# ereiss123/LDPCsimulation

Measured on AMD Instinct MI355X. Metric: decoded Mbit/s + FER match vs CPU, N=1944 rate-1/2 min-sum @ 1/2/4/8 MI355X, higher is better.
Workload: dtype f64

## Files before the change

include/ldpc_hip.h:

```cpp
#ifndef LDPC_HIP_H
#define LDPC_HIP_H

#include <stdint.h>

#ifdef __cplusplus
extern "C" {
#endif

#define LDPC_ABI_VERSION 11

typedef enum {
    LDPC_OK = 0,
    LDPC_ERR_INVALID = -1,
    LDPC_ERR_NOMEM = -2,
    LDPC_ERR_DEVICE = -3,
    LDPC_ERR_UNSUPPORTED = -4,
    LDPC_ERR_IO = -5,
    LDPC_ERR_GRAPH = -6
} ldpc_status;

typedef enum { LDPC_MS = 0, LDPC_NMS = 1, LDPC_OMS = 2, LDPC_BP = 3, LDPC_DDBMP = 4 } ldpc_variant;

typedef enum { LDPC_F32 = 0, LDPC_F64 = 1 } ldpc_precision;

typedef enum { LDPC_FLOODING = 0, LDPC_LAYERED = 1 } ldpc_schedule;

typedef struct ldpc_graph ldpc_graph;
typedef struct ldpc_ctx ldpc_ctx;

typedef struct {
    int64_t bit_err;
    int64_t frame_err;
    int64_t uncoded_bit_err;
    int64_t frames;
    int64_t iters;
    int64_t syndrome_fail;
} ldpc_counts;

typedef struct {
    int32_t bit_err;
    int32_t uncoded_bit_err;
    int32_t syndrome_fail;
    int32_t iters;
} ldpc_frame_result;

typedef struct {
    int32_t variant;
    int32_t precision;
    int32_t T;
    int32_t quantize;
    int32_t saturate;
    int32_t qbits;
    double  ymax;
    double  alpha;
    double  delta;
    int32_t schedule;
    int32_t early_stop;
    double  n0;
    double  max_llr;
} ldpc_decoder_cfg;

int         ldpc_abi_version(void);
const char *ldpc_last_error(void);
int         ldpc_f64_nms_fast_division(double alpha);
int         ldpc_bp_math_probe(int device, const double *x, int n, double *tanh_out, double *log_out);
int         ldpc_check_selftest(int device);

int  ldpc_graph_create(int N, int M, const int *num_nlist, const int *const *nlist,
                       const int *num_mlist, const int *const *mlist, ldpc_graph **out);
int  ldpc_graph_load_alist(const char *path, ldpc_graph **out);
int  ldpc_graph_info(const ldpc_graph *g, int *N, int *M, int *E, int *maxdv, int *maxdc);
void ldpc_graph_destroy(ldpc_graph *g);
int  ldpc_graph_layers(const ldpc_graph *g, int32_t *row_order, int32_t *layer_ptr, int *nlayers);

int  ldpc_device_count(int *n);
int  ldpc_ctx_create(int device, const ldpc_graph *g, int max_batch, ldpc_ctx **out);
int  ldpc_ctx_set_stream(ldpc_ctx *ctx, void *hip_stream);
int  ldpc_ctx_synchronize(ldpc_ctx *ctx);
void ldpc_ctx_destroy(ldpc_ctx *ctx);

int  ldpc_decode_batch(ldpc_ctx *ctx, const void *y, int batch, const ldpc_decoder_cfg *cfg,
                       const int8_t *c, int8_t *d_out, ldpc_frame_result *frames,
                       ldpc_counts *counts);

int  ldpc_sim_set_codewords(ldpc_ctx *ctx, const uint8_t *bits, int rows);

int  ldpc_sim_launch(ldpc_ctx *ctx, double ebn0_db, double R, const ldpc_decoder_cfg *cfg,
                     uint64_t seed, uint32_t stream_id, uint64_t first_cw, int batch,
                     ldpc_frame_result *frames_dev);
int  ldpc_ctx_read_counts(ldpc_ctx *ctx, ldpc_counts *out, int reset);
int  ldpc_ctx_read_histogram(ldpc_ctx *ctx, int64_t *out, int reset);
int  ldpc_sim_batch(ldpc_ctx *ctx, double ebn0_db, double R, const ldpc_decoder_cfg *cfg,
                    uint64_t seed, uint32_t stream_id, uint64_t first_cw, int batch,
                    ldpc_frame_result *frames, ldpc_counts *accum);

int  ldpc_sim_trace(ldpc_ctx *ctx, double ebn0_db, double R, const ldpc_decoder_cfg *cfg,
                    uint64_t seed, uint32_t stream_id, uint64_t first_cw, int batch,
                    void *y_out, int8_t *d_out, ldpc_frame_result *frames, ldpc_counts *accum);

int  ldpc_ctx_last_kernel_ms(ldpc_ctx *ctx, float *ms);
int  ldpc_ctx_kernel_info(ldpc_ctx *ctx, const ldpc_decoder_cfg *cfg, char *name, int name_len,
                          int *lds_bytes, int *blocks_per_cu);
int  ldpc_ctx_redo_count(ldpc_ctx *ctx, int64_t *n);
int  ldpc_ctx_redo_list(ldpc_ctx *ctx, uint32_t *list, int64_t cap, int64_t *n);
int  ldpc_ctx_row_sched_info(ldpc_ctx *ctx, const ldpc_decoder_cfg *cfg, int32_t *info);
int  ldpc_ctx_pp_inreg_info(ldpc_ctx *ctx, const ldpc_decoder_cfg *cfg, int32_t *info);
int  ldpc_ctx_pp_row_slots(ldpc_ctx *ctx, const ldpc_decoder_cfg *cfg, uint16_t *cols, uint8_t *deg, int cap,
                           int *nslots);

typedef enum {
    LDPC_OPT_ROWS64 = 1,
    LDPC_OPT_ROWS32 = 2,
    LDPC_OPT_PP_SLOTS = 3,
    LDPC_OPT_KERNEL = 4,
    LDPC_OPT_FLOOD_MODE = 5,
    LDPC_OPT_FLOOD_MSG = 6,
    LDPC_OPT_FLOOD_SPS_CHECK = 7,
    LDPC_OPT_FLOOD_SPS_BIT = 8,
    LDPC_OPT_FLOOD_RESIDENT = 9,
    LDPC_OPT_FLOOD_STREAMS = 10,
    LDPC_OPT_FLOOD_BPC = 11,
    LDPC_OPT_LAYERED_BPC = 12,
    LDPC_OPT_LAYERED_LDS_POS = 13,
    LDPC_OPT_LAYERED_ROWS64 = 14,
    LDPC_OPT_LAYERED_THREADS = 15,
    LDPC_OPT_ROWS_BPC = 16,
    LDPC_OPT_FAST_BPC = 17,
    LDPC_OPT_BP_KERNEL = 18,
    LDPC_OPT_GDBF_KERNEL = 19,
    LDPC_OPT_EMS_THREADS = 20,
    LDPC_OPT_EMS_SWIZZLE = 21,
    LDPC_OPT_DDBMP_KERNEL = 22
} ldpc_option;
#define LDPC_OPT_COUNT 23
int  ldpc_ctx_set_option(ldpc_ctx *ctx, int option, int value);
int  ldpc_ctx_get_option(const ldpc_ctx *ctx, int option, int *value);

typedef enum {
    LDPC_GDBF_NOISE = 1,
    LDPC_GDBF_ADAPT = 2,
    LDPC_GDBF_WEIGHT = 4,
    LDPC_GDBF_SMOOTH = 8,
    LDPC_GDBF_SATURATE = 16,
    LDPC_GDBF_QUANTIZE = 32,
    LDPC_GDBF_SEQUENTIAL = 64,
    LDPC_GDBF_MODESWITCH = 128,
    LDPC_GDBF_QPROB = 256
} ldpc_gdbf_flag;

typedef struct {
    int32_t flags;
    int32_t precision;
    int32_t T;
    int32_t windowsize;
    int32_t nq;
    int32_t tswitch;
    double  theta;
    double  lambda;
    double  alpha;
    double  noise_scale;
    double  ymax;
    double  qsigma;
} ldpc_gdbf_cfg;

int  ldpc_gdbf_decode_batch(ldpc_ctx *ctx, const void *y, const void *pert, int batch, const ldpc_gdbf_cfg *cfg,
                            const int8_t *c, int8_t *d_out, ldpc_frame_result *frames, ldpc_counts *counts);
int  ldpc_gdbf_sim_launch(ldpc_ctx *ctx, double ebn0_db, double R, const ldpc_gdbf_cfg *cfg, uint64_t seed,
                          uint32_t stream_id, uint64_t first_cw, int batch, ldpc_frame_result *frames_dev);
int  ldpc_gdbf_sim_batch(ldpc_ctx *ctx, double ebn0_db, double R, const ldpc_gdbf_cfg *cfg, uint64_t seed,
                         uint32_t stream_id, uint64_t first_cw, int batch, ldpc_frame_result *frames,
                         ldpc_counts *accum);
int  ldpc_gdbf_kernel_info(ldpc_ctx *ctx, const ldpc_gdbf_cfg *cfg, char *name, int name_len, int *lds_bytes);

typedef struct {
    int32_t flags;
    int32_t precision;
    int32_t T;
    int32_t maxphase;
    int32_t windowsize;
    int32_t reserved;
    double  theta;
    double  lambda;
    double  alpha;
    double  noise_scale;
    double  ymax;
} ldpc_rgdbf_cfg;

int  ldpc_rgdbf_decode_batch(ldpc_ctx *ctx, const void *y, const void *pert, int batch, const ldpc_rgdbf_cfg *cfg,
                             const int8_t *c, int8_t *d_out, ldpc_frame_result *frames, ldpc_counts *counts);
int  ldpc_rgdbf_sim_launch(ldpc_ctx *ctx, double ebn0_db, double R, const ldpc_rgdbf_cfg *cfg, uint64_t seed,
                           uint32_t stream_id, uint64_t first_cw, int batch, ldpc_frame_result *frames_dev);
int  ldpc_rgdbf_sim_batch(ldpc_ctx *ctx, double ebn0_db, double R, const ldpc_rgdbf_cfg *cfg, uint64_t seed,
                          uint32_t stream_id, uint64_t first_cw, int batch, ldpc_frame_result *frames,
                          ldpc_counts *accum);
int  ldpc_rgdbf_kernel_info(ldpc_ctx *ctx, const ldpc_rgdbf_cfg *cfg, char *name, int name_len, int *lds_bytes);

typedef struct {
    int32_t flags, precision, T, attempts, windowsize, first_attempt;
    double  theta, lambda, alpha, noise_scale, ymax;
} ldpc_rstat_cfg;
typedef struct { int32_t bit_err, iters, syndrome_fail, smoothing_used; } ldpc_attempt_result;
typedef struct {
    int32_t *err_trace;
    int32_t *unsat_trace;
    int8_t  *d_trace;
    int8_t  *s_trace;
} ldpc_rstat_trace;

int  ldpc_rstat_decode_batch(ldpc_ctx *ctx, const void *y, const void *pert, int batch, const ldpc_rstat_cfg *cfg,
                             const int8_t *c, ldpc_attempt_result *attempts_out, const ldpc_rstat_trace *trace,
                             int8_t *d_out, ldpc_frame_result *frames, ldpc_counts *counts);
int  ldpc_rstat_sim_launch(ldpc_ctx *ctx, double ebn0_db, double R, const ldpc_rstat_cfg *cfg, uint64_t seed,
                           uint32_t stream_id, uint64_t first_cw, int batch, ldpc_attempt_result *attempts_dev,
                           const ldpc_rstat_trace *trace_dev, ldpc_frame_result *frames_dev);
int  ldpc_rstat_sim_batch(ldpc_ctx *ctx, double ebn0_db, double R, const ldpc_rstat_cfg *cfg, uint64_t seed,
                          uint32_t stream_id, uint64_t first_cw, int batch, ldpc_attempt_result *attempts_out,
                          const ldpc_rstat_trace *trace, ldpc_frame_result *frames, ldpc_counts *accum);
int  ldpc_rstat_sim_trace(ldpc_ctx *ctx, double ebn0_db, double R, const ldpc_rstat_cfg *cfg, uint64_t seed,
                          uint32_t stream_id, uint64_t first_cw, int batch, void *y_out, void *pert_out,
                          ldpc_attempt_result *attempts_out, const ldpc_rstat_trace *trace, int8_t *d_out,
                          ldpc_frame_result *frames, ldpc_counts *accum);
int  ldpc_rstat_kernel_info(ldpc_ctx *ctx, const ldpc_rstat_cfg *cfg, int with_trace, char *name, int name_len,
                            int *lds_bytes);

typedef struct {
    int32_t precision;
    int32_t T;
    int32_t maxphase;
    int32_t nq;
    int32_t qlen;
    int32_t reserved;
    double  w, ymax, noise_scale, theta0;
} ldpc_hwgdbf_cfg;

int  ldpc_hwgdbf_decode_batch(ldpc_ctx *ctx, const void *y, const void *q, const int32_t *qptr0, int batch,
                              const ldpc_hwgdbf_cfg *cfg, const int8_t *c, int8_t *d_out, ldpc_frame_result *frames,
                              int32_t *iters_run, ldpc_counts *counts);
int  ldpc_hwgdbf_sim_launch(ldpc_ctx *ctx, double ebn0_db, double R, const ldpc_hwgdbf_cfg *cfg, uint64_t seed,
                            uint32_t stream_id, uint64_t first_cw, int batch, ldpc_frame_result *frames_dev);
int  ldpc_hwgdbf_sim_batch(ldpc_ctx *ctx, double ebn0_db, double R, const ldpc_hwgdbf_cfg *cfg, uint64_t seed,
                           uint32_t stream_id, uint64_t first_cw, int batch, ldpc_frame_result *frames,
                           ldpc_counts *accum);
int  ldpc_hwgdbf_sim_trace(ldpc_ctx *ctx, double ebn0_db, double R, const ldpc_hwgdbf_cfg *cfg, uint64_t seed,
                           uint32_t stream_id, uint64_t first_cw, int batch, void *y_out, void *q_out,
                           int8_t *d_out, ldpc_frame_result *frames, ldpc_counts *accum);
int  ldpc_hwgdbf_kernel_info(ldpc_ctx *ctx, const ldpc_hwgdbf_cfg *cfg, char *name, int name_len, int *lds_bytes);

typedef struct {
    int32_t variant;
    int32_t precision;
    int32_t T;
    int32_t qbits;
    int32_t msg_bits;
    int32_t nms_num;
    int32_t nms_shift;
    int32_t beta;
    int32_t early_stop;
    int32_t reserved;
    double  ymax;
} ldpc_fxms_cfg;

// ... 84 lines not shown
```

ldpcsimulation_amd/csrc/api.cpp:

```cpp
#include "ldpc_hip.h"
#include "gdbf.h"
#include "rgdbf.h"
#include "rstat.h"
#include "hwgdbf.h"
#include "fxms.h"
#include "fxlms.h"
#include "bp.h"
#include "ddbmp.h"
#include "nb.h"

#include <hip/hip_runtime.h>

#include <cmath>
#include <cstdlib>
#include <cstdio>
#include <cstring>
#include <algorithm>
#include <new>
#include <string>
#include <vector>

#include "graph.h"
#include "kernels.h"
#include "host_rt.h"

using namespace ldpc;

static thread_local std::string g_last_error;

#ifdef LDPC_CHECK
namespace ldpc {
static const char *check_site_name(unsigned s)
{
    static const char *const names[CHK_SITES] = {
        "?", "rows_pp gather (app entry)", "rows_pp scatter (c2v slot)", "rows_pp bit read (c2v slot)",
        "rows_pp app write", "rows_fast gather (app entry)", "rows_fast scatter (c2v slot)",
        "rows_fast bit read (c2v slot)", "rows_fast app write", "flood/layered bit position",
        "flood c2v / eref slot", "flood packed-state row", "gdbf_rows bit", "gdbf_rows check term slot",
        "EMS message slot", "bp_rows bit", "bp_rows message slot", "ddbmp edge flag slot", "ddbmp check parity",
        "rgdbf_rows bit flag", "rgdbf_rows check parity", "hwgdbf decision byte", "hwgdbf check parity",
        "hwgdbf noise sample", "rstat decision byte", "rstat check parity", "rows_es gather (app entry)",
        "rows_es scatter (c2v slot)", "rows_es bit read (c2v slot)", "rows_es app write", "fxms message slot",
        "fxms decision byte", "fxlms schedule entry", "fxlms APP", "fxlms row state"};
    return s < CHK_SITES ? names[s] : "?";
}
long check_collect(hipStream_t s, char *msg, size_t msg_len)
{
    hipError_t e = hipStreamSynchronize(s);
    if (e != hipSuccess) return -(long)e;
    hipError_t (*const take[])(CheckRec *) = {check_take_rows_pp, check_take_rows_fast, check_take_flood, check_take_layered,
                                              check_take_gdbf, check_take_nb, check_take_bp, check_take_ddbmp,
                                              check_take_rgdbf, check_take_hwgdbf, check_take_rstat, check_take_rows_es,
                                              check_take_fxms, check_take_fxlms};
    long total = 0;
    for (auto fn : take) {
        CheckRec r{};
        if ((e = fn(&r)) != hipSuccess) return -(long)e;
        if (r.count && !total)
            std::snprintf(msg, msg_len, "LDPC_CHECK: %s index %u >= bound %u (block %u, thread %u)",
                          check_site_name(r.site), r.idx, r.bound, r.block, r.thread);
        total += r.count;
    }
    return total;
}
}
#endif

struct ldpc_ctx : CtxCore {
    const ldpc_graph *g = nullptr;
    ldpc::DevGraph dg{};
    DevBuf graph, hist, y_stage, c_stage, d_stage, fw_stage, cw_table, gscratch, p_stage;
    DevBuf rs_att_stage, rs_unc, rs_tr_stage[4];
    DevBuf hw_ptr_stage, hw_it_stage;
    DevBuf fx_code_stage;
    bool has_fxl = false;
    ldpc::FxlmsSched fxl{};
    DevBuf fxl_sched;
    int cw_rows = 0;
    ldpc::AuxStream aux;
    bool has_rs = false;
    ldpc::RowSched rs{};
    DevBuf sched;
    bool has_rs_pp = false;
    ldpc::RowSched rs_pp{};
    DevBuf sched_pp;
    bool has_rs_ppi = false;
    ldpc::RowSched rs_ppi{};
    DevBuf sched_ppi;
    bool has_fs = false;
    ldpc::FloodSched fs{};
    DevBuf fsched;
    bool has_ls = false;
    ldpc::LayerSched ls{};
    DevBuf lsched;
    DevBuf divcheck;
    DevBuf redo;
    bool last_fast = false;
    std::vector<std::pair<float, bool>> div_ok;
};

namespace ldpc {
int set_last_error(int code, const std::string &msg)
{
    g_last_error = msg;
    return code;
}

static const Options kNoOptions{};
static thread_local const Options *t_opts = nullptr;
const Options &cur_opts() { return t_opts ? *t_opts : kNoOptions; }
OptScope::OptScope(const Options &o) : prev_(t_opts) { t_opts = &o; }
OptScope::~OptScope() { t_opts = prev_; }

bool option_value_ok(int option, int v)
{
    switch (option) {
    case LDPC_OPT_ROWS64:
    case LDPC_OPT_ROWS32: return v >= 0 && v <= 2;
    case LDPC_OPT_PP_SLOTS: return v >= 0 && v <= 2;
    case LDPC_OPT_FLOOD_MODE:
    case LDPC_OPT_FLOOD_MSG:
    case LDPC_OPT_BP_KERNEL:
    case LDPC_OPT_GDBF_KERNEL:
    case LDPC_OPT_DDBMP_KERNEL:
    case LDPC_OPT_EMS_SWIZZLE: return v == 0 || v == 1;
    case LDPC_OPT_KERNEL: return v >= 0 && v <= 3;
    case LDPC_OPT_FLOOD_SPS_CHECK:
    case LDPC_OPT_FLOOD_SPS_BIT: return v >= 0 && v <= 4;
    case LDPC_OPT_FLOOD_RESIDENT: return v >= 0 && v <= 4096;
    case LDPC_OPT_FLOOD_STREAMS: return v >= 0 && v <= 2;
    case LDPC_OPT_FLOOD_BPC:
    case LDPC_OPT_LAYERED_BPC:
    case LDPC_OPT_ROWS_BPC:
    case LDPC_OPT_FAST_BPC: return v >= 0 && v <= 64;
    case LDPC_OPT_LAYERED_LDS_POS: return v >= 0 && v <= 65536;
    case LDPC_OPT_LAYERED_ROWS64: return v >= 0 && v <= 2;
    case LDPC_OPT_LAYERED_THREADS:
    case LDPC_OPT_EMS_THREADS: return v == 0 || v == 512 || v == 1024;
    default: return false;
    }
}
}

template <class T> static const T *section(const DevBuf &buf, size_t off) { return (const T *)((const unsigned char *)buf.p + off); }

static hipError_t upload_graph(const ldpc_graph &g, DevBuf &buf, ldpc::DevGraph &dg)
{
    Blob b(256);
    const size_t o_rc = b.add(g.row_cols), o_rd = b.add(g.row_deg), o_cp = b.add(g.col_ptr),
                 o_cr = b.add(g.col_refs.data(), sizeof(uint32_t) * g.col_refs.size(), sizeof(uint32_t) * ((size_t)g.E + 1));
    const hipError_t e = upload(b, buf);
    if (e != hipSuccess) return e;
    dg = {g.N, g.M, g.maxdc > 0 ? g.maxdc : 1, section<int32_t>(buf, o_rc), section<uint8_t>(buf, o_rd),
          section<int32_t>(buf, o_cp), section<uint32_t>(buf, o_cr)};
    return hipSuccess;
}

static hipError_t upload_row_sched(const ldpc::RowSchedule &hs, DevBuf &buf, ldpc::RowSched &rs,
                                   const std::vector<uint8_t> *pair_flags = nullptr)
{
    Blob b(256);
    const size_t o_cc = b.add(hs.cn_cols), o_cp = b.add(hs.cn_pos), o_cd = b.add(hs.cn_deg), o_vc = b.add(hs.vn_col),
                 o_vi = b.add(hs.vn_info), o_pf = pair_flags ? b.add(*pair_flags) : 0;
    const hipError_t e = upload(b, buf);
    if (e != hipSuccess) return e;
    rs = {hs.threads, hs.cpt, hs.dc, hs.e_pad, hs.rpt, hs.dc_low, section<uint16_t>(buf, o_cc),
          section<uint16_t>(buf, o_cp), section<uint8_t>(buf, o_cd), section<uint16_t>(buf, o_vc),
          section<uint32_t>(buf, o_vi), pair_flags ? section<uint8_t>(buf, o_pf) : nullptr, hs.e_pad, 0, 0};
    return hipSuccess;
}

static hipError_t upload_flood_sched(const ldpc_graph &g, const ldpc::FloodSchedule &fh, DevBuf &buf, ldpc::FloodSched &fs)
{
    std::vector<uint32_t> eref((size_t)fh.e_pad + 64, 0);
    for (int i = 0; i < fh.M_pad; ++i)
        for (int k = 0; k < fh.rdeg[i]; ++k)
            eref[fh.sq[(size_t)k * fh.M_pad + i]] = ((uint32_t)i << 5) | (uint32_t)k;
    Blob b(256);
    const size_t o_sp = b.add(fh.sp), o_sq = b.add(fh.sq), o_rd = b.add(fh.rdeg), o_pb = b.add(fh.pos_of_bit),
                 o_ba = b.add(fh.bit_at), o_pd = b.add(fh.pdeg), o_gb = b.add(fh.gbase), o_er = b.add(eref);
    const hipError_t e = upload(b, buf);
    if (e != hipSuccess) return e;
    fs = {fh.M_pad, fh.dc, fh.ngroups, fh.e_pad, g.maxdv, section<int32_t>(buf, o_sp), section<int32_t>(buf, o_sq),
          section<uint8_t>(buf, o_rd), section<int32_t>(buf, o_pb), section<int32_t>(buf, o_ba),
          section<uint8_t>(buf, o_pd), section<int32_t>(buf, o_gb), section<uint32_t>(buf, o_er)};
    return hipSuccess;
}

static hipError_t upload_layer_sched(const ldpc::LayerSchedule &lh, DevBuf &buf, ldpc::LayerSched &ls)
{
    Blob b(256);
    const size_t o_lp = b.add(lh.lptr), o_sp = b.add(lh.sp), o_rd = b.add(lh.rdeg), o_pb = b.add(lh.pos_of_bit);
    const hipError_t e = upload(b, buf);
    if (e != hipSuccess) return e;
    ls = {(int)lh.lptr.size() - 1, 0, lh.M_pad, section<int32_t>(buf, o_lp), section<int32_t>(buf, o_sp),
          section<uint8_t>(buf, o_rd), section<int32_t>(buf, o_pb)};
    for (int L = 0; L < ls.nlayers; ++L) ls.max_layer = std::max(ls.max_layer, lh.lptr[L + 1] - lh.lptr[L]);
    return hipSuccess;
}

static hipError_t upload_fxlms_sched(const ldpc_graph &g, const ldpc::LayerSchedule &lh, DevBuf &buf, ldpc::FxlmsSched &sc)
{
    const int M = g.M, dcs = g.maxdc > 0 ? g.maxdc : 1;
    std::vector<int32_t> cols((size_t)dcs * M, 0);
    std::vector<uint8_t> deg(M, 0);
    for (int n = 0; n < M; ++n) {
        const int j = lh.row_order[n], d = g.row_deg[j];
        deg[n] = (uint8_t)d;
        for (int k = 0; k < dcs; ++k)
            cols[(size_t)k * M + n] = d ? g.row_cols[(size_t)j * dcs + std::min(k, d - 1)] : 0;
    }
    Blob b(256);
    const size_t o_lp = b.add(lh.lptr), o_c = b.add(cols), o_d = b.add(deg);
    const hipError_t e = upload(b, buf);
    if (e != hipSuccess) return e;
    sc = {g.N, M, dcs, (int)lh.lptr.size() - 1, section<int32_t>(buf, o_lp), section<int32_t>(buf, o_c),
          section<uint8_t>(buf, o_d)};
    return hipSuccess;
}

static const char kFramesDev[] = "frames_dev must be a device pointer";

template <class Args>
static int stage_given(SyncCall &s, ldpc_ctx *c, Args &a, bool f64, const void *y, const void *extra, size_t extra_elems,
                       const void **extra_dev, const int8_t *cw)
{
    const size_t fsz = f64 ? 8 : 4, nb = (size_t)a.batch * c->g->N;
    a.src = ldpc::SRC_GIVEN;
    RC_TRY(s.in(y, nb * fsz, c->y_stage, a.y));
    if (extra) RC_TRY(s.in(extra, extra_elems * fsz, c->p_stage, *extra_dev));
    return s.in(cw, nb, c->c_stage, a.c);
}

template <class Run>
static int sim_batch_frames(ldpc_ctx *c, int batch, ldpc_frame_result *frames, ldpc_counts *accum, Run run)
{
    RC_TRY(c->enter());
    SyncCall s(*c);
    RC_TRY(s.snapshot());
    ldpc_frame_result *w;
    RC_TRY(s.out(frames, c->fw_stage, sizeof(ldpc_frame_result) * (size_t)batch, w));
    RC_TRY(run(w));
    return s.finish(accum);
}

template <class Args>
static int bind_decisions(SyncCall &s, ldpc_ctx *c, Args &a, int8_t *d_out, ldpc_frame_result *frames)
{
    RC_TRY(s.out(d_out, c->d_stage, (size_t)a.batch * c->g->N, a.d_out));
    return s.out(frames, c->fw_stage, sizeof(ldpc_frame_result) * (size_t)a.batch, a.frame_res);
}

template <class Args, class Cfg> static void redecode_fill(Args &a, ldpc_ctx *c, const Cfg *cfg, int batch)
{
    std::memset((void *)&a, 0, sizeof a);
    a.batch = batch;
    a.T = cfg->T;
    a.flags = cfg->flags;
    a.windowsize = cfg->windowsize;
    a.theta0 = cfg->theta;
    a.lambda = cfg->lambda;
    a.w = cfg->alpha * cfg->ymax;
    a.ymax = cfg->ymax;
    a.qmax = 1.0;
    fill_accounting(a, *c);
}

template <class Cfg, class Own> static int fx_check_cfg(const Cfg *cfg, Own own)
{
    if (!cfg) return set_err(LDPC_ERR_INVALID, "cfg is null");
    if (cfg->variant != LDPC_MS && cfg->variant != LDPC_NMS && cfg->variant != LDPC_OMS)
        return set_err(cfg->variant == LDPC_BP || cfg->variant == LDPC_DDBMP ? LDPC_ERR_UNSUPPORTED : LDPC_ERR_INVALID,
// ... 471 lines not shown
    ldpc::DecodeArgs a;
    fill_common(a, c, cfg, batch);
    RC_TRY(nms_setup(c, cfg, a));
    SyncCall s(*c);
    RC_TRY(stage_given(s, c, a, f64, y, nullptr, 0, nullptr, cw));
    RC_TRY(bind_decisions(s, c, a, d_out, frame_weights));
    RC_TRY(s.snapshot());
    RC_TRY(run_kernel(c, a, f64, cfg->schedule));
    return s.finish(counts);
}

int ldpc_sim_set_codewords(ldpc_ctx *c, const uint8_t *bits, int rows)
{
    if (!c) return set_err(LDPC_ERR_INVALID, "ctx is null");
    if (rows < 0 || (rows > 0 && !bits)) return set_err(LDPC_ERR_INVALID, "bad codeword table");
    RC_TRY(c->enter());
    c->cw_rows = 0;
    if (rows == 0) return LDPC_OK;
    const size_t n = (size_t)rows * c->g->N;
    std::vector<int8_t> bip(n);
    for (size_t i = 0; i < n; ++i) {
        if (bits[i] > 1) return set_err(LDPC_ERR_INVALID, "codeword bit %zu is %d (want 0/1)", i, bits[i]);
        bip[i] = bits[i] ? -1 : +1;
    }
    HIP_TRY(c->cw_table.ensure(n));
    HIP_TRY(hipMemcpy(c->cw_table.p, bip.data(), n, hipMemcpyHostToDevice));
    c->cw_rows = rows;
    return LDPC_OK;
}

static int sim_run(ldpc_ctx *c, const SimCall &q, const ldpc_decoder_cfg *cfg, ldpc_frame_result *frames_dev,
                   void *y_out_dev, int8_t *d_out_dev)
{
    ldpc::DecodeArgs a;
    fill_common(a, c, cfg, q.batch);
    RC_TRY(nms_setup(c, cfg, a));
    const SimPoint pt = fill_sim(a, *c, q);
    fill_cw_table(a, *c);
    if (cfg->variant == LDPC_BP) a.n0 = pt.N0;
    a.frame_res = (int4 *)frames_dev;
    a.y_out = y_out_dev;
    a.d_out = d_out_dev;
    return run_kernel(c, a, cfg->precision == LDPC_F64, cfg->schedule);
}

int ldpc_sim_launch(ldpc_ctx *c, double ebn0_db, double R, const ldpc_decoder_cfg *cfg, uint64_t seed,
                    uint32_t stream_id, uint64_t first_cw, int batch, ldpc_frame_result *frames_dev)
{
    const SimCall q{ebn0_db, R, seed, stream_id, first_cw, batch};
    RC_TRY(check_sim(c, [&] { return check_cfg(c, cfg); }, q, false));
    RC_TRY(require_device(frames_dev, kFramesDev));
    RC_TRY(c->enter());
    return sim_run(c, q, cfg, frames_dev, nullptr, nullptr);
}

int ldpc_ctx_read_counts(ldpc_ctx *c, ldpc_counts *out, int reset)
{
    if (!c) return set_err(LDPC_ERR_INVALID, "ctx is null");
    RC_TRY(c->enter());
    return c->read_counts(out, reset);
}

int ldpc_ctx_read_histogram(ldpc_ctx *c, int64_t *out, int reset)
{
    if (!c || !out) return set_err(LDPC_ERR_INVALID, "null argument");
    RC_TRY(c->enter());
    HIP_TRY(hipMemcpyAsync(out, c->hist.p, c->hist.n, hipMemcpyDeviceToHost, c->stream));
    HIP_TRY(hipStreamSynchronize(c->stream));
    if (reset) HIP_TRY(hipMemsetAsync(c->hist.p, 0, c->hist.n, c->stream));
    return LDPC_OK;
}

int ldpc_sim_trace(ldpc_ctx *c, double ebn0_db, double R, const ldpc_decoder_cfg *cfg, uint64_t seed,
                   uint32_t stream_id, uint64_t first_cw, int batch, void *y_out, int8_t *d_out,
                   ldpc_frame_result *frames, ldpc_counts *accum)
{
    const SimCall q{ebn0_db, R, seed, stream_id, first_cw, batch};
    RC_TRY(check_sim(c, [&] { return check_cfg(c, cfg); }, q, false));
    RC_TRY(c->enter());
    const size_t nb = (size_t)batch * c->g->N;
    SyncCall s(*c);
    RC_TRY(s.snapshot());
    ldpc_frame_result *w;
    void *y;
    int8_t *d;
    RC_TRY(s.out(frames, c->fw_stage, sizeof(ldpc_frame_result) * (size_t)batch, w));
    RC_TRY(s.out(y_out, c->y_stage, nb * (cfg->precision == LDPC_F64 ? 8 : 4), y));
    RC_TRY(s.out(d_out, c->d_stage, nb, d));
    RC_TRY(sim_run(c, q, cfg, w, y, d));
    return s.finish(accum);
}

int ldpc_sim_batch(ldpc_ctx *c, double ebn0_db, double R, const ldpc_decoder_cfg *cfg, uint64_t seed,
                   uint32_t stream_id, uint64_t first_cw, int batch, ldpc_frame_result *frames, ldpc_counts *accum)
{
    return ldpc_sim_trace(c, ebn0_db, R, cfg, seed, stream_id, first_cw, batch, nullptr, nullptr, frames, accum);
}

int ldpc_ctx_last_kernel_ms(ldpc_ctx *c, float *ms)
{
    return c ? c->last_kernel_ms(ms) : set_err(LDPC_ERR_INVALID, "null argument");
}

static int info_plan(ldpc_ctx *c, const ldpc_decoder_cfg *cfg, ldpc::LaunchPlan &p)
{
    if (!c || !cfg) return set_err(LDPC_ERR_INVALID, "null argument");
    RC_TRY(check_cfg(c, cfg));
    RC_TRY(c->enter());
    ldpc::DecodeArgs a;
    fill_common(a, c, cfg, 1);
    RC_TRY(nms_setup(c, cfg, a));
    p = build_plan(c, a, cfg->precision == LDPC_F64, cfg->schedule);
    return LDPC_OK;
}

int ldpc_ctx_row_sched_info(ldpc_ctx *c, const ldpc_decoder_cfg *cfg, int32_t *info)
{
    if (!info) return set_err(LDPC_ERR_INVALID, "null argument");
    ldpc::LaunchPlan p;
    RC_TRY(info_plan(c, cfg, p));
    if (!p.rs) return set_err(LDPC_ERR_UNSUPPORTED, "the row kernel does not decode this cfg (kernel %s)", p.name);
    const ldpc::RowSched &rs = *p.rs;
    info[0] = rs.threads;
    info[1] = rs.rpt;
    info[2] = rs.cpt;
    info[3] = rs.dc;
    info[4] = rs.e_pad;
    info[5] = p.cw_per_block;
    info[6] = p.lds_bytes;
    info[7] = p.blocks_per_cu;
    info[8] = rs.dc_low;
    info[9] = rs.dc_low ? (rs.threads + rs.threads / 2) * rs.dc_low + (rs.threads / 2) * rs.dc
                        : rs.threads * rs.rpt * rs.dc;
    return LDPC_OK;
}

int ldpc_ctx_pp_inreg_info(ldpc_ctx *c, const ldpc_decoder_cfg *cfg, int32_t *info)
{
    if (!info) return set_err(LDPC_ERR_INVALID, "null argument");
    ldpc::LaunchPlan p;
    RC_TRY(info_plan(c, cfg, p));
    if (p.kernel != ldpc::Kernel::rows_pp || !p.rs)
        return set_err(LDPC_ERR_UNSUPPORTED, "the ping-pong kernel does not decode this cfg (kernel %s)", p.name);
    int32_t rsi[10];
    RC_TRY(ldpc_ctx_row_sched_info(c, cfg, rsi));
    const ldpc::RowSched *ri = p.rs_inreg;
    info[0] = ri ? ri->n_inreg : 0;
    info[1] = ri ? ri->lds_edge_slots : rsi[9];
    info[2] = ri ? ri->e_used : p.rs->e_pad;
    info[3] = ri ? ri->cpt : p.rs->cpt;
    return LDPC_OK;
}

int ldpc_ctx_pp_row_slots(ldpc_ctx *c, const ldpc_decoder_cfg *cfg, uint16_t *cols, uint8_t *deg, int cap, int *nslots)
{
    if (!cols || !deg || !nslots || cap < 0) return set_err(LDPC_ERR_INVALID, "null argument");
    ldpc::LaunchPlan p;
    RC_TRY(info_plan(c, cfg, p));
    if (p.kernel != ldpc::Kernel::rows_pp || !p.rs)
        return set_err(LDPC_ERR_UNSUPPORTED, "the ping-pong kernel does not decode this cfg (kernel %s)", p.name);
    const ldpc::RowSched *rs = p.rs_inreg ? p.rs_inreg : p.rs;
    *nslots = rs->threads * rs->rpt;
    if (cap < *nslots) return set_err(LDPC_ERR_INVALID, "%d row slots, room for %d", *nslots, cap);
    RC_TRY(c->enter());
    HIP_TRY(hipMemcpyAsync(cols, rs->cn_cols, sizeof(uint16_t) * (size_t)*nslots * rs->dc, hipMemcpyDeviceToHost, c->stream));
    HIP_TRY(hipMemcpyAsync(deg, rs->cn_deg, sizeof(uint8_t) * (size_t)*nslots, hipMemcpyDeviceToHost, c->stream));
    HIP_TRY(hipStreamSynchronize(c->stream));
    return LDPC_OK;
}

int ldpc_ctx_redo_count(ldpc_ctx *c, int64_t *n)
{
    if (!c || !n) return set_err(LDPC_ERR_INVALID, "null argument");
    *n = 0;
    if (!c->last_fast || !c->redo.p) return LDPC_OK;
    RC_TRY(c->enter());
    unsigned h = 0;
    HIP_TRY(hipMemcpyAsync(&h, c->redo.p, sizeof h, hipMemcpyDeviceToHost, c->stream));
    HIP_TRY(hipStreamSynchronize(c->stream));
    *n = (int64_t)h;
    return LDPC_OK;
}

int ldpc_ctx_redo_list(ldpc_ctx *c, uint32_t *list, int64_t cap, int64_t *n)
{
    if (!c || !n || cap < 0 || (cap > 0 && !list)) return set_err(LDPC_ERR_INVALID, "null argument");
    RC_TRY(ldpc_ctx_redo_count(c, n));
    const int64_t m = std::min(*n, cap);
    if (m > 0) {
        HIP_TRY(hipMemcpyAsync(list, (const unsigned *)c->redo.p + 1, sizeof(unsigned) * (size_t)m, hipMemcpyDeviceToHost,
                               c->stream));
        HIP_TRY(hipStreamSynchronize(c->stream));
    }
    return LDPC_OK;
}

int ldpc_ctx_kernel_info(ldpc_ctx *c, const ldpc_decoder_cfg *cfg, char *name, int name_len, int *lds_bytes,
                         int *bpc)
{
    ldpc::LaunchPlan p;
    RC_TRY(info_plan(c, cfg, p));
    if (bpc) *bpc = p.blocks_per_cu;
    return report_choice(p, name, name_len, lds_bytes);
}


static int gdbf_check_cfg(const ldpc_gdbf_cfg *cfg)
{
    if (!cfg) return set_err(LDPC_ERR_INVALID, "cfg is null");
    if (cfg->precision != LDPC_F32 && cfg->precision != LDPC_F64)
        return set_err(LDPC_ERR_INVALID, "bad precision %d", cfg->precision);
    if (cfg->T < 0 || cfg->T > 4094) return set_err(LDPC_ERR_INVALID, "T must be in 0..4094");
    if (cfg->flags & ~511) return set_err(LDPC_ERR_INVALID, "unknown GDBF flags 0x%x", cfg->flags);
    if ((cfg->flags & LDPC_GDBF_ADAPT) && (cfg->flags & (LDPC_GDBF_SEQUENTIAL | LDPC_GDBF_MODESWITCH)))
        return set_err(LDPC_ERR_UNSUPPORTED, "threshold adaptation with single-bit flips is not supported");
    if ((cfg->flags & LDPC_GDBF_QPROB) && (cfg->flags & LDPC_GDBF_NOISE))
        return set_err(LDPC_ERR_UNSUPPORTED, "QPROB with NOISE is not supported");
    if ((cfg->flags & LDPC_GDBF_MODESWITCH) && cfg->tswitch < 0) return set_err(LDPC_ERR_INVALID, "tswitch < 0");
    if ((cfg->flags & (LDPC_GDBF_SATURATE | LDPC_GDBF_QUANTIZE)) && !(cfg->ymax > 0))
        return set_err(LDPC_ERR_INVALID, "saturate/quantize need ymax > 0");
    if ((cfg->flags & LDPC_GDBF_QUANTIZE) && (cfg->nq < 1 || cfg->nq > 30))
        return set_err(LDPC_ERR_INVALID, "nq out of range");
    if ((cfg->flags & LDPC_GDBF_SMOOTH) && (cfg->windowsize < 0 || cfg->windowsize > 32767))
        return set_err(LDPC_ERR_INVALID, "windowsize out of range");
    return LDPC_OK;
}

static void gdbf_fill(ldpc::GdbfArgs &a, ldpc_ctx *c, const ldpc_gdbf_cfg *cfg, int batch)
{
    std::memset(&a, 0, sizeof a);
    a.batch = batch;
    a.T = cfg->T;
    a.flags = cfg->flags;
    a.windowsize = cfg->windowsize;
    a.theta0 = cfg->theta;
    a.lambda = cfg->lambda;
    a.w = (cfg->flags & LDPC_GDBF_WEIGHT) ? cfg->alpha : 1.0;
    a.ymax = cfg->ymax;
    a.qmax = std::pow(2, (cfg->nq - 1));
    a.tswitch = cfg->tswitch;
    a.qsigma = cfg->qsigma;
    fill_accounting(a, *c);
}

static int gdbf_run(ldpc_ctx *c, const ldpc::GdbfArgs &a, bool f64)
{
    const ldpc::OptScope os(c->opts);
    const ldpc::GdbfChoice ch = ldpc::gdbf_choose(c->dg, f64, a.flags, c->g->maxdv, c->g->maxdc);
    return run_with_slots(*c, c->gscratch, ch, a.batch, 2 * c->num_cus, [&](void *scratch, int slots) {
        return ldpc::gdbf_launch(c->dg, a, f64, ch, scratch, slots, c->num_cus, c->stream);
    });
}

int ldpc_gdbf_decode_batch(ldpc_ctx *c, const void *y, const void *pert, int batch, const ldpc_gdbf_cfg *cfg,
                           const int8_t *cw, int8_t *d_out, ldpc_frame_result *frames, ldpc_counts *counts)
{
    if (!c || !y) return set_err(LDPC_ERR_INVALID, "null argument");
    RC_TRY(gdbf_check_cfg(cfg));
    RC_TRY(check_batch(*c, batch));
    const bool with_pert = cfg->flags & (LDPC_GDBF_NOISE | LDPC_GDBF_QPROB);
    if (with_pert && !pert) return set_err(LDPC_ERR_INVALID, "NOISE / QPROB need pert");
    if ((cfg->flags & LDPC_GDBF_QPROB) && !(cfg->qsigma > 0)) return set_err(LDPC_ERR_INVALID, "QPROB needs qsigma > 0");
    RC_TRY(c->enter());
    const bool f64 = cfg->precision == LDPC_F64;
    ldpc::GdbfArgs a;
    gdbf_fill(a, c, cfg, batch);
    SyncCall s(*c);
    RC_TRY(stage_given(s, c, a, f64, y, with_pert ? pert : nullptr, (size_t)batch * c->g->N * (size_t)cfg->T, &a.pert, cw));
    RC_TRY(bind_decisions(s, c, a, d_out, frames));
    RC_TRY(s.snapshot());
    RC_TRY(gdbf_run(c, a, f64));
    return s.finish(counts);
}

static int gdbf_sim_run(ldpc_ctx *c, const SimCall &q, const ldpc_gdbf_cfg *cfg, ldpc_frame_result *frames_dev)
{
    ldpc::GdbfArgs a;
    gdbf_fill(a, c, cfg, q.batch);
    fill_sim(a, *c, q);
    fill_cw_table(a, *c);
    a.frame_res = (int4 *)frames_dev;
    a.noise_sigma = a.sigma * cfg->noise_scale;
    a.qsigma = a.noise_sigma;
    return gdbf_run(c, a, cfg->precision == LDPC_F64);
}

int ldpc_gdbf_sim_launch(ldpc_ctx *c, double ebn0_db, double R, const ldpc_gdbf_cfg *cfg, uint64_t seed,
                         uint32_t stream_id, uint64_t first_cw, int batch, ldpc_frame_result *frames_dev)
{
    const SimCall q{ebn0_db, R, seed, stream_id, first_cw, batch};
    RC_TRY(check_sim(c, [&] { return gdbf_check_cfg(cfg); }, q, true));
    RC_TRY(require_device(frames_dev, kFramesDev));
    RC_TRY(c->enter());
    return gdbf_sim_run(c, q, cfg, frames_dev);
}

int ldpc_gdbf_sim_batch(ldpc_ctx *c, double ebn0_db, double R, const ldpc_gdbf_cfg *cfg, uint64_t seed,
                        uint32_t stream_id, uint64_t first_cw, int batch, ldpc_frame_result *frames,
                        ldpc_counts *accum)
{
    const SimCall q{ebn0_db, R, seed, stream_id, first_cw, batch};
    RC_TRY(check_sim(c, [&] { return gdbf_check_cfg(cfg); }, q, true));
    return sim_batch_frames(c, batch, frames, accum, [&](ldpc_frame_result *w) { return gdbf_sim_run(c, q, cfg, w); });
}

int ldpc_gdbf_kernel_info(ldpc_ctx *c, const ldpc_gdbf_cfg *cfg, char *name, int name_len, int *lds_bytes)
// ... 667 lines not shown
```

ldpcsimulation_amd/csrc/kernels.h:

```cpp
#pragma once
#include "options.h"
#include <hip/hip_runtime.h>
#include <cstdint>

namespace ldpc {

struct DevGraph {
    int N, M, dcs;
    const int32_t *row_cols;
    const uint8_t *row_deg;
    const int32_t *col_ptr;
    const uint32_t *col_refs;
};

enum { SRC_GIVEN = 0, SRC_PHILOX = 1 };
enum { VARIANT_BP = 3, VARIANT_DDBMP = 4 };

struct DecodeArgs {
    int batch, T, variant, quantize, saturate;
    int early_stop;
    double ymax, nq, alpha, delta;
    double n0, max_llr;
    int nms_fast;
    float alpha_rcp;
    int src;
    const void *y;
    const int8_t *c;
    const int8_t *cw_table;
    int cw_rows;
    uint64_t seed, first_cw;
    uint32_t stream_id;
    double sigma;
    int8_t *d_out;
    void *y_out;
    int4 *frame_res;
    unsigned long long *counts;
    unsigned long long *hist;
    unsigned long long *stamps;
};

struct RowSched {
    int threads, cpt, dc, e_pad, rpt;
    int dc_low;
    const uint16_t *cn_cols;
    const uint16_t *cn_pos;
    const uint8_t *cn_deg;
    const uint16_t *vn_col;
    const uint32_t *vn_info;
    const uint8_t *pair;
    int e_used;
    int n_inreg;
    int lds_edge_slots;
};

struct FloodSched {
    int M_pad, dc, ngroups, e_pad;
    int dv;
    const int32_t *sp, *sq;
    const uint8_t *rdeg;
    const int32_t *pos_of_bit;
    const int32_t *bit_at;
    const uint8_t *pdeg;
    const int32_t *gbase;
    const uint32_t *eref;
};

struct LayerSched {
    int nlayers = 0, max_layer = 0, M_pad = 0;
    const int32_t *lptr = nullptr;
    const int32_t *sp = nullptr;
    const uint8_t *rdeg = nullptr;
    const int32_t *pos_of_bit = nullptr;
};

enum class Kernel {
    rows, rows_fast, rows_pp,
    rows_es,
    lds, global,
    flood_persistent, flood_phase,
    layered_lds, layered_global,
    bp_rows, bp_lds, bp_global,
    ddbmp_rows, ddbmp_lds, ddbmp_global
};

struct LaunchPlan {
    Kernel kernel = Kernel::global;
    const char *name = "";
    const void *fn = nullptr;
    int threads = 0;
    int lds_bytes = 0;
    int layered_pos = 0;
    int cache_lds_bytes = 0;
    int cw_per_block = 1;
    int blocks_per_cu = 0;
    int grid = 0;
    size_t scratch_per_block = 0;
    size_t scratch_bytes = 0;
    const RowSched *rs = nullptr;
    const RowSched *rs_inreg = nullptr;
    bool redo = false;
};

struct PlanInput {
    const DevGraph &g;
    int E;
    const RowSched *rs, *rs_pp;
    const FloodSched *fs;
    const LayerSched *ls;
    int num_cus;
    const DecodeArgs &a;
    bool f64;
    int maxdv = 0;
    const RowSched *rs_ppi = nullptr;
};

template <typename T> struct type_tag { using type = T; };
template <int V> struct src_tag { static constexpr int value = V; };
template <class Fn>
auto for_f_src(bool f64, int src, Fn &&fn)
{
    if (f64)
        return src == SRC_GIVEN ? fn(type_tag<double>{}, src_tag<SRC_GIVEN>{}) : fn(type_tag<double>{}, src_tag<SRC_PHILOX>{});
    return src == SRC_GIVEN ? fn(type_tag<float>{}, src_tag<SRC_GIVEN>{}) : fn(type_tag<float>{}, src_tag<SRC_PHILOX>{});
}

constexpr size_t kMaxLds = 160 * 1024;

int occupancy(const void *fn, int threads, int lds_bytes);
hipError_t launch_fn(const LaunchPlan &p, void **args, hipStream_t s);

bool plan_lds(const PlanInput &in, LaunchPlan &p);
void plan_global(const PlanInput &in, LaunchPlan &p);
hipError_t launch_generic(const LaunchPlan &p, const DevGraph &g, const DecodeArgs &a, void *gscratch, hipStream_t s);
bool plan_rows(const PlanInput &in, LaunchPlan &p);
hipError_t launch_rows(const LaunchPlan &p, const DevGraph &g, const DecodeArgs &a, hipStream_t s);
bool plan_rows_es(const PlanInput &in, LaunchPlan &p);
hipError_t launch_rows_es(const LaunchPlan &p, const DevGraph &g, const DecodeArgs &a, unsigned *ticket, hipStream_t s);
struct AuxStream {
    hipStream_t s = nullptr;
    hipEvent_t fork = nullptr, join = nullptr;
};
bool plan_flood(const PlanInput &in, LaunchPlan &p);
hipError_t launch_flood(const LaunchPlan &p, const DevGraph &g, const FloodSched &fs, const DecodeArgs &a, bool f64,
                        void *gscratch, hipStream_t s, const AuxStream *aux);
void plan_layered(const PlanInput &in, LaunchPlan &p);
hipError_t launch_layered(const LaunchPlan &p, const DevGraph &g, const FloodSched &fs, const LayerSched &ls,
                          const DecodeArgs &a, void *gscratch, hipStream_t s);
constexpr int kPackedMaxDc = 26;

hipError_t verify_div_by_reciprocal(float alpha, float rcp, unsigned long long *mismatches_dev, hipStream_t s);

bool plan_rows_fast(const PlanInput &in, LaunchPlan &p);
bool rows_fast_f32_ok(const DecodeArgs &a);
hipError_t launch_rows_fast(const LaunchPlan &p, const DevGraph &g, const DecodeArgs &a, unsigned *redo, hipStream_t s);
bool markstein_exact_alpha(double alpha);
size_t redo_lds_bytes(const DevGraph &g, bool f64);
hipError_t launch_redo(const DevGraph &g, const DecodeArgs &a, bool f64, const unsigned *redo, hipStream_t s,
                       int num_cus);

bool plan_rows_pp(const PlanInput &in, LaunchPlan &p);
#ifndef LDPC_PP_INREG_CPT
#define LDPC_PP_INREG_CPT 3
#endif
hipError_t launch_rows_pp(const LaunchPlan &p, const DevGraph &g, const DecodeArgs &a, unsigned *redo, hipStream_t s);

constexpr int kRowsMaxThreads = 1024;
constexpr int kRowsCpt[] = {2, 4, 8};
constexpr int kRowsMaxThreadsForRpt[] = {0, 1024, 512, 384};
constexpr int kRowsDc[] = {8, 16, 32};

}
```

ldpcsimulation_amd/csrc/kernels.hip:

```cpp
#include "minsum_kernels.h"
#include "frame.h"

namespace ldpc {

template <typename F, int SRC, bool ES>
__device__ __forceinline__ void decode_codeword(const DecodeArgs &a, const DevGraph &g, int b,
                                                RowState<F> *rows, F *app, F *yq, int *red)
{
    const int tid = threadIdx.x, nt = blockDim.x;
    const int N = g.N, M = g.M;

    const int8_t *cvec = frame_codeword<SRC>(a, b, N);
    int unc = 0;
    channel_bits<F, SRC, false>(a, b, N, cvec, a.y_out, [&](int v, F yv) {
        const F q = front_end<F>(yv, a);
        yq[v] = q;
        app[v] = q;
        const int cv = cvec ? cvec[v] : 1;
        unc += ((q > F(0) ? 1 : -1) * cv < 0);
    });
    for (int j = tid; j < M; j += nt) {
        RowState<F> z;
        z.m1 = F(0); z.m2 = F(0); z.meta = 0;
        rows[j] = z;
// ... 16 lines not shown
    for (; it < a.T; ++it) {
        if (ES && !__syncthreads_or(syndrome())) break;
        for (int j = tid; j < M; j += nt) {
            RowState<F> st = rows[j];
            const int deg = g.row_deg[j];
            const int32_t *rc = g.row_cols + (size_t)j * g.dcs;
            const int oidx = (int)(st.meta & 63u);
            const uint64_t osg = st.meta >> 6;
            F mn1 = dinf<F>(), mn2 = dinf<F>();
            int amin = 63;
            uint64_t sg = 0;
            for (int k = 0; k < deg; ++k) {
                F cold = (k == oidx) ? st.m2 : st.m1;
                if ((osg >> k) & 1u) cold = -cold;
                const F x = app[rc[k]] - cold;
                sg |= (uint64_t)(!(x >= F(0))) << k;
                const F ax = dabs(x);
                if (ax <= mn1) { mn2 = mn1; mn1 = ax; amin = k; }
                else if (ax < mn2) { mn2 = ax; }
            }
            const uint64_t degmask = (deg >= 64) ? ~0ull : ((1ull << deg) - 1ull);
            uint64_t eff = (__popcll(sg) & 1) ? (sg ^ degmask) : sg;
            F M1 = mn1, M2 = mn2;
            if (a.variant == V_NMS) {
                M1 = mn1 / alpha;
                M2 = mn2 / alpha;
            } else if (a.variant == V_OMS) {
                const F t1 = mn1 - delta, t2 = mn2 - delta;
                const bool p1 = t1 > F(0), p2 = t2 > F(0);
                M1 = p1 ? t1 : F(0);
                M2 = p2 ? t2 : F(0);
                const uint64_t abit = (amin < 64) ? (1ull << amin) : 0ull;
                if (!p1 || mn1 == F(0)) eff &= abit;
                if (!p2 || mn2 == F(0)) eff &= ~abit;
            }
            st.m1 = M1;
            st.m2 = M2;
            st.meta = (uint64_t)amin | (eff << 6);
            rows[j] = st;
        }
        __syncthreads();
        for (int v = tid; v < N; v += nt) {
            F sum = yq[v];
            const int e1 = g.col_ptr[v + 1];
            for (int e = g.col_ptr[v]; e < e1; ++e) {
                const uint32_t ref = g.col_refs[e];
                const int k = (int)(ref & 63u);
                const RowState<F> st = rows[ref >> 6];
                const F mag = (k == (int)(st.meta & 63u)) ? st.m2 : st.m1;
                sum += ((st.meta >> (6 + k)) & 1u) ? -mag : mag;
            }
            app[v] = sum;
        }
        __syncthreads();
    }

    int w = 0;
    for (int v = tid; v < N; v += nt) {
        const int d = app[v] > F(0) ? 1 : -1;
        const int cv = cvec ? cvec[v] : 1;
        w += (d != cv);
        if (a.d_out) a.d_out[(size_t)b * N + v] = (int8_t)d;
    }
    int sums[3] = {w, unc, syndrome()};
    block_sum_n_t0<3>(sums, red);
    if (tid == 0)
        frame_account(a.counts, a.hist, a.frame_res, b, sums[0], sums[1], sums[2] > 0, ES ? it : a.T, ES ? it : 0);
    __syncthreads();
}

template <typename F, int SRC, bool ES>
__global__ __launch_bounds__(256) void k_decode_lds(DecodeArgs a, DevGraph g)
{
    extern __shared__ __attribute__((aligned(16))) unsigned char smem[];
    RowState<F> *rows = reinterpret_cast<RowState<F> *>(smem);
    F *app = reinterpret_cast<F *>(smem + sizeof(RowState<F>) * (size_t)g.M);
    F *yq = app + g.N;
    int *red = reinterpret_cast<int *>(yq + g.N);
    decode_codeword<F, SRC, ES>(a, g, blockIdx.x, rows, app, yq, red);
}

template <typename F, int SRC>
__global__ __launch_bounds__(256) void k_redo(DecodeArgs a, DevGraph g, const unsigned *redo)
{
    extern __shared__ __attribute__((aligned(16))) unsigned char smem[];
    RowState<F> *rows = reinterpret_cast<RowState<F> *>(smem);
    F *app = reinterpret_cast<F *>(smem + sizeof(RowState<F>) * (size_t)g.M);
    F *yq = app + g.N;
    int *red = reinterpret_cast<int *>(yq + g.N);
    const unsigned n = redo[0];
    for (unsigned i = blockIdx.x; i < n; i += gridDim.x) decode_codeword<F, SRC, false>(a, g, (int)redo[1 + i], rows, app, yq, red);
}

template <typename F, int SRC, bool ES>
__global__ __launch_bounds__(256) void k_decode_global(DecodeArgs a, DevGraph g, unsigned char *scratch,
                                                       size_t slot_bytes)
{
    __shared__ int red[16];
    unsigned char *base = scratch + slot_bytes * blockIdx.x;
    RowState<F> *rows = reinterpret_cast<RowState<F> *>(base);
    F *app = reinterpret_cast<F *>(base + sizeof(RowState<F>) * (size_t)g.M);
    F *yq = app + g.N;
    for (int b = blockIdx.x; b < a.batch; b += gridDim.x)
        decode_codeword<F, SRC, ES>(a, g, b, rows, app, yq, red);
}


__global__ __launch_bounds__(256) void k_verify_div(float alpha, float rcp, unsigned long long *bad)
{
    const uint32_t total = 0x7f800000u;
    unsigned long long nbad = 0;
    for (uint32_t u = blockIdx.x * blockDim.x + threadIdx.x; u < total; u += gridDim.x * blockDim.x) {
        const float x = __uint_as_float(u);
        const float q = x * rcp;
        const float f = __builtin_fmaf(__builtin_fmaf(-q, alpha, x), rcp, q);
        const float d = x / alpha;
        nbad += (__float_as_uint(f) != __float_as_uint(d));
    }
    for (int o = 32; o > 0; o >>= 1) nbad += __shfl_xor(nbad, o, 64);
    if ((threadIdx.x & 63) == 0 && nbad) atomicAdd(bad, nbad);
}


hipError_t verify_div_by_reciprocal(float alpha, float rcp, unsigned long long *bad, hipStream_t s)
{
    hipError_t e = hipMemsetAsync(bad, 0, sizeof(unsigned long long), s);
    if (e != hipSuccess) return e;
    hipLaunchKernelGGL(k_verify_div, dim3(8192), dim3(256), 0, s, alpha, rcp, bad);
    return hipGetLastError();
}

static size_t state_bytes(const DevGraph &g, bool f64)
{
    const size_t rs = f64 ? sizeof(RowState<double>) : sizeof(RowState<float>);
    const size_t fs = f64 ? 8 : 4;
    return rs * (size_t)g.M + 2 * fs * (size_t)g.N;
}

constexpr int kThreads = 256;

int occupancy(const void *fn, int threads, int lds_bytes)
{
    int nb = 0;
    if (lds_bytes > 0) (void)hipFuncSetAttribute(fn, hipFuncAttributeMaxDynamicSharedMemorySize, lds_bytes);
    if (hipOccupancyMaxActiveBlocksPerMultiprocessor(&nb, fn, threads, lds_bytes) != hipSuccess) {
        (void)hipGetLastError();
        return 0;
    }
    return nb;
}

hipError_t launch_fn(const LaunchPlan &p, void **args, hipStream_t s)
{
    const int lds = p.lds_bytes + p.cache_lds_bytes;
    if (!p.fn || p.grid <= 0) return hipErrorInvalidValue;
    if (lds > 0) {
        const hipError_t e = hipFuncSetAttribute(p.fn, hipFuncAttributeMaxDynamicSharedMemorySize, lds);
        if (e != hipSuccess) return e;
    }
    return hipLaunchKernel(p.fn, dim3(p.grid), dim3(p.threads), args, (size_t)lds, s);
}

bool plan_lds(const PlanInput &in, LaunchPlan &p)
{
    const size_t lds = (state_bytes(in.g, in.f64) + 64 + 15) & ~(size_t)15;
    if (lds > kMaxLds) return false;
    const bool es = in.a.early_stop != 0;
    const auto fn = [es](auto f, auto s) {
        using F = typename decltype(f)::type;
        constexpr int SRC = decltype(s)::value;
        return es ? (const void *)k_decode_lds<F, SRC, true> : (const void *)k_decode_lds<F, SRC, false>;
    };
    p = LaunchPlan{};
    p.kernel = Kernel::lds;
    p.name = "lds";
    p.fn = for_f_src(in.f64, in.a.src, fn);
    p.threads = kThreads;
    p.lds_bytes = (int)lds;
    p.blocks_per_cu = occupancy(for_f_src(in.f64, SRC_PHILOX, fn), p.threads, p.lds_bytes);
    p.grid = in.a.batch;
    return true;
}

void plan_global(const PlanInput &in, LaunchPlan &p)
{
    const bool es = in.a.early_stop != 0;
    const auto fn = [es](auto f, auto s) {
        using F = typename decltype(f)::type;
        constexpr int SRC = decltype(s)::value;
        return es ? (const void *)k_decode_global<F, SRC, true> : (const void *)k_decode_global<F, SRC, false>;
    };
    p = LaunchPlan{};
    p.kernel = Kernel::global;
    p.name = "global";
    p.fn = for_f_src(in.f64, in.a.src, fn);
    p.threads = kThreads;
    p.scratch_per_block = (state_bytes(in.g, in.f64) + 255) & ~(size_t)255;
    p.blocks_per_cu = occupancy(for_f_src(in.f64, SRC_PHILOX, fn), p.threads, 0);
    int per_cu = p.blocks_per_cu;
    if (const int cap = opt(LDPC_OPT_FLOOD_BPC)) per_cu = std::min(per_cu, cap);
    if (per_cu <= 0) per_cu = 1;
    p.grid = std::min(per_cu * in.num_cus, in.a.batch);
    p.scratch_bytes = p.scratch_per_block * (size_t)p.grid;
}

hipError_t launch_generic(const LaunchPlan &p, const DevGraph &g, const DecodeArgs &a, void *gscratch, hipStream_t s)
{
    unsigned char *gs = (unsigned char *)gscratch;
    size_t spb = p.scratch_per_block;
    void *args[] = {(void *)&a, (void *)&g, &gs, &spb};
    return launch_fn(p, args, s);
}

size_t redo_lds_bytes(const DevGraph &g, bool f64) { return (state_bytes(g, f64) + 64 + 15) & ~(size_t)15; }

hipError_t launch_redo(const DevGraph &g, const DecodeArgs &a, bool f64, const unsigned *redo, hipStream_t s,
                       int num_cus)
{
    const size_t lds = redo_lds_bytes(g, f64);
    return for_f_src(f64, a.src, [&](auto f, auto src) -> hipError_t {
        auto fn = k_redo<typename decltype(f)::type, decltype(src)::value>;
        hipError_t e = hipFuncSetAttribute((const void *)fn, hipFuncAttributeMaxDynamicSharedMemorySize, (int)lds);
        if (e != hipSuccess) return e;
        hipLaunchKernelGGL(fn, dim3(num_cus), dim3(kThreads), lds, s, a, g, redo);
        return hipGetLastError();
    });
}

}
```

ldpcsimulation_amd/csrc/rows_pp.hip:

```cpp
#ifndef LDPC_VN_U3_F64
#ifdef LDPC_VN_U3
#define LDPC_VN_U3_F64 LDPC_VN_U3
#else
#define LDPC_VN_U3_F64 4
#endif
#endif
#ifndef LDPC_VN_U1_F64
#ifdef LDPC_VN_U1
#define LDPC_VN_U1_F64 LDPC_VN_U1
#else
#define LDPC_VN_U1_F64 8
#endif
#endif
#include "kernels.h"
#include "device_common.h"
#include "minsum_common.h"
#include "fast64.h"

#include <hip/hip_runtime.h>
#include <algorithm>
#include <cstdint>
#include <cstdlib>
#include <type_traits>

namespace ldpc {

namespace {

#ifndef LDPC_PP_STICKY
#define LDPC_PP_STICKY 0
#endif
#ifndef LDPC_PP_TAILFUSE
#define LDPC_PP_TAILFUSE 1
#endif
#ifndef LDPC_PP_TAILEXP
#define LDPC_PP_TAILEXP 0
#endif
#ifndef LDPC_PP_CHAN_ALL
#define LDPC_PP_CHAN_ALL 0
#endif
#ifndef LDPC_PP_NOB2
#define LDPC_PP_NOB2 1
#endif
#ifndef LDPC_PP_CHAN_SPLIT
#define LDPC_PP_CHAN_SPLIT 0
#endif
#ifndef LDPC_PP_EXP
#define LDPC_PP_EXP 0
#endif
#if LDPC_PP_EXP != 0 && !defined(LDPC_AB_BUILD)
#error "LDPC_PP_EXP != 0 gives wrong results by design: make ppvariant only"
#endif
#if LDPC_PP_TAILEXP != 0 && !defined(LDPC_AB_BUILD)
#error "LDPC_PP_TAILEXP != 0 gives wrong results by design: make ppvariant only"
#endif
#ifndef LDPC_PP_BITDELAY
#define LDPC_PP_BITDELAY 0
#endif
#ifndef LDPC_PP_ROWFENCE
#define LDPC_PP_ROWFENCE 1
#endif

#ifndef LDPC_PP_PRIO
#define LDPC_PP_PRIO 0
#endif
#ifndef LDPC_PP_PREFETCH
#define LDPC_PP_PREFETCH 1
#endif
#ifndef LDPC_PP_STORE_ORDER
#define LDPC_PP_STORE_ORDER 1
#endif
#ifndef LDPC_PP_GATHER_FIRST
#define LDPC_PP_GATHER_FIRST 0
#endif
#ifndef LDPC_PP_INREG_Y
#define LDPC_PP_INREG_Y 1
#endif
#ifndef LDPC_PP_ILV
#define LDPC_PP_ILV 2
#endif
#ifndef LDPC_PP_ILV_SKIP
#define LDPC_PP_ILV_SKIP 0
#endif
#ifndef LDPC_PP_SBASE
#define LDPC_PP_SBASE 0
#endif
#ifndef LDPC_PP_ONEPREM
#define LDPC_PP_ONEPREM 1
#endif
#if LDPC_PP_SBASE && !defined(LDPC_CHECK)
#define PP_ADDR8(DC, w, k, base, n, site) addr8<DC, true>(w, k, base)
#else
#define PP_ADDR8(DC, w, k, base, n, site) LDPC_ADDR8(DC, w, k, base, n, site)
#endif

#ifdef LDPC_STAMPS
#define PP_STAMP_DECL unsigned long long st_work = 0, st_wait = 0, st_step[6] = {}, st_t0 = __builtin_amdgcn_s_memtime()
#define PP_BARRIER()                                                        \
    do {                                                                    \
        const unsigned long long te_ = __builtin_amdgcn_s_memtime();        \
        __syncthreads();                                                    \
        const unsigned long long tb_ = __builtin_amdgcn_s_memtime();        \
        st_work += te_ - st_t0;                                             \
        st_wait += tb_ - te_;                                               \
        st_t0 = tb_;                                                        \
    } while (0)
#define PP_STAMP_ACC(k)                                                     \
    do {                                                                    \
        const unsigned long long t_ = __builtin_amdgcn_s_memtime();         \
        st_step[k] += t_ - st_t0;                                           \
        st_t0 = t_;                                                         \
    } while (0)
#define PP_STAMP_TOP() PP_STAMP_ACC(0)
#define PP_SYNC_STAMPED(k0)                                                 \
    do {                                                                    \
        PP_STAMP_ACC(k0);                                                   \
        __syncthreads();                                                    \
        PP_STAMP_ACC(k0 + 1);                                               \
    } while (0)
#define PP_STAMP_OUT()                                                                              \
    if (a.stamps && (threadIdx.x & 63) == 0 && blockIdx.x < 256) {                                  \
        a.stamps[(blockIdx.x * 16 + (threadIdx.x >> 6)) * 2] = st_work;                             \
        a.stamps[(blockIdx.x * 16 + (threadIdx.x >> 6)) * 2 + 1] = st_wait;                         \
        for (int k_ = 0; k_ < 6; ++k_)                                                              \
            a.stamps[8192 + (blockIdx.x * 16 + (threadIdx.x >> 6)) * 6 + k_] = st_step[k_];         \
    }
#else
#define PP_STAMP_DECL
#define PP_BARRIER() __syncthreads()
#define PP_STAMP_TOP()
#define PP_STAMP_ACC(k)
#define PP_SYNC_STAMPED(k0) __syncthreads()
#define PP_STAMP_OUT()
#endif

constexpr int kPPRole = 512;
constexpr int kPPWaves = 2 * kPPRole / 64;
constexpr int kPPMaxCw = 4;
constexpr int kPPRedSums = 32;
constexpr int kPPRedAcc = kPPRedSums + kPPWaves * 3 * kPPMaxCw;
constexpr int kPPRedInts = kPPRedAcc + 2 * 6 + 4;
static_assert(kPPRedAcc % 2 == 0 && kPPRedAcc + 2 * 6 <= kPPRedInts, "acc (6 x u64) outside red[]");

template <int B, int E, typename Fn>
__device__ __forceinline__ void static_for(Fn &&f)
{
    if constexpr (B < E) {
        f(std::integral_constant<int, B>());
        static_for<B + 1, E>(f);
    }
}

template <typename F> struct PPCw { static constexpr int C = sizeof(F) == 8 ? 1 : 2; };

template <typename P>
struct PPSlots {
    P *app[2], *c2v[2];
    uint32_t app_base[2], c2v_base[2];
    int *red;
};

__host__ __device__ constexpr int pp_slot_words(int N, int EA) { return (N + 3 + EA + 1) & ~1; }

template <typename P>
__device__ __forceinline__ PPSlots<P> pp_slots(unsigned char *smem, int N, int EA)
{
    static_assert(sizeof(P) == 8, "one 8-byte LDS word per slot element");
    PPSlots<P> s;
    const int SL = pp_slot_words(N, EA);
    P *b = reinterpret_cast<P *>(smem);
#pragma unroll
    for (int X = 0; X < 2; ++X) {
        s.app[X] = b + X * SL;
        s.c2v[X] = s.app[X] + (N + 3);
        s.app_base[X] = lds_addr_of(s.app[X]);
        s.c2v_base[X] = lds_addr_of(s.c2v[X]);
    }
    s.red = reinterpret_cast<int *>(b + 2 * SL);
    return s;
}

__device__ __forceinline__ bool pp_plain_step(const DecodeArgs &a, int N, int grp, int C)
{
    return !a.cw_table && !a.y_out && !a.quantize && !a.saturate && (N & 3) == 0 && (grp + 1) * 2 * C <= a.batch;
}

template <typename F>
__device__ __forceinline__ void pp_channel_plain(const DecodeArgs &a, const PPSlots<Pack<F, PPCw<F>::C>> &s, int N,
                                                 int grp, int (&unc)[2 * PPCw<F>::C], int t0, int nt, unsigned *bad)
{
    constexpr int C = PPCw<F>::C;
    const F kMax = sizeof(F) == 8 ? (F)kFast64Max : (F)1e30f;
    const int ng4 = N / 4;
    const F sigma = (F)a.sigma;
    for (int t = t0; t < 2 * C * ng4; t += nt) {
        int q = 0;
#pragma unroll
        for (int k = 1; k < 2 * C; ++k) q += t >= k * ng4 ? 1 : 0;
        const int g4 = t - q * ng4, X = q >= C ? 1 : 0, c = q - X * C;
        const uint64_t cw = a.first_cw + (uint64_t)(grp * 2 * C + q);
        uint32_t u[4];
        philox4x32_10<true>((uint32_t)g4, (uint32_t)cw, (uint32_t)(cw >> 32), a.stream_id, (uint32_t)a.seed,
                            (uint32_t)(a.seed >> 32), u);
        F n[4];
        box_muller(u[0], u[1], n[0], n[1]);
        box_muller(u[2], u[3], n[2], n[3]);
        F qv[4];
        int e = 0;
        bool ok = true;
#pragma unroll
        for (int q4 = 0; q4 < 4; ++q4) {
            qv[q4] = (F(1) + sigma * n[q4]) + F(0);
            e += (qv[q4] > F(0) ? 1 : -1) < 0;
            ok &= dabs(qv[q4]) < kMax;
        }
        if (!ok) *bad |= 1u << X;
        if constexpr (C == 1) {
            struct alignas(16) D2 { F d[2]; };
            const uint32_t at = (X ? s.app_base[1] : s.app_base[0]) + 32u * (uint32_t)g4;
            lds_put<D2>(at, D2{{qv[0], qv[1]}});
            lds_put<D2>(at + 16u, D2{{qv[2], qv[3]}});
        } else {
            auto *ap = X ? s.app[1] : s.app[0];
#pragma unroll
            for (int q4 = 0; q4 < 4; ++q4) ap[4 * g4 + q4].v[c] = qv[q4];
        }
#pragma unroll
        for (int qq = 0; qq < 2 * C; ++qq) unc[qq] += qq == q ? e : 0;
    }
}

template <typename F, int SRC>
__device__ __forceinline__ void pp_channel(const DecodeArgs &a, const PPSlots<Pack<F, PPCw<F>::C>> &s, int N, int grp,
                                           int (&unc)[2 * PPCw<F>::C], int t0, int nt, unsigned *bad = nullptr)
{
    constexpr int C = PPCw<F>::C;
    const F kMax = sizeof(F) == 8 ? (F)kFast64Max : (F)1e30f;
#pragma unroll
    for (int q = 0; q < 2 * C; ++q) unc[q] = 0;
    const int ng4 = (N + 3) / 4;
    if constexpr (SRC == SRC_PHILOX && LDPC_PP_NOB2) {
        if (pp_plain_step(a, N, grp, C)) {
            pp_channel_plain<F>(a, s, N, grp, unc, t0, nt, bad);
            return;
        }
    }
    for (int t = t0; t < 2 * C * ng4; t += nt) {
        int q = 0;
#pragma unroll
        for (int k = 1; k < 2 * C; ++k) q += t >= k * ng4 ? 1 : 0;
        const int g4 = t - q * ng4, X = q >= C ? 1 : 0, c = q - X * C;
        const int b = grp * 2 * C + q;
        auto *ap = X ? s.app[1] : s.app[0];
        if (b >= a.batch) {
#pragma unroll
            for (int q4 = 0; q4 < 4; ++q4)
                if (4 * g4 + q4 < N) ap[4 * g4 + q4].v[c] = F(1);
            continue;
        }
        const uint64_t cw = a.first_cw + (uint64_t)b;
        F yv[4];
        const int8_t *cvec;
        if (SRC == SRC_GIVEN) {
            cvec = a.c ? a.c + (size_t)b * N : nullptr;
            const F *y = reinterpret_cast<const F *>(a.y) + (size_t)b * N;
#pragma unroll
            for (int q4 = 0; q4 < 4; ++q4) yv[q4] = 4 * g4 + q4 < N ? y[4 * g4 + q4] : F(0);
        } else {
            cvec = a.cw_table ? a.cw_table + (size_t)(cw % (uint64_t)a.cw_rows) * N : nullptr;
            uint32_t u[4];
            philox4x32_10<true>((uint32_t)g4, (uint32_t)cw, (uint32_t)(cw >> 32), a.stream_id, (uint32_t)a.seed,
                          (uint32_t)(a.seed >> 32), u);
            F n[4];
            box_muller(u[0], u[1], n[0], n[1]);
            box_muller(u[2], u[3], n[2], n[3]);
            const F sigma = (F)a.sigma;
#pragma unroll
            for (int q4 = 0; q4 < 4; ++q4) {
                const int v = 4 * g4 + q4;
                const int cv = (cvec && v < N) ? cvec[v] : 1;
                yv[q4] = (F)cv * (F(1) + sigma * n[q4]);
                if (a.y_out && v < N) reinterpret_cast<F *>(a.y_out)[(size_t)b * N + v] = yv[q4];
            }
        }
        int e = 0;
#pragma unroll
        for (int q4 = 0; q4 < 4; ++q4) {
            const int v = 4 * g4 + q4;
            if (v < N) {
                const int cv = cvec ? cvec[v] : 1;
                F qv = front_end<F>(yv[q4], a);
                if (LDPC_PP_NOB2) {
                    qv = qv + F(0);
                    if (!(dabs(qv) < kMax)) *bad |= 1u << X;
                }
                ap[v].v[c] = qv;
                e += ((qv > F(0) ? 1 : -1) * cv < 0);
            }
        }
#pragma unroll
        for (int qq = 0; qq < 2 * C; ++qq) unc[qq] += qq == q ? e : 0;
    }
}

__device__ __forceinline__ int wave_sum3(int x)
{
    return __builtin_popcountll(__builtin_amdgcn_ballot_w64((x & 1) != 0)) +
           2 * __builtin_popcountll(__builtin_amdgcn_ballot_w64((x & 2) != 0)) +
           4 * __builtin_popcountll(__builtin_amdgcn_ballot_w64((x & 4) != 0));
}

template <int C, bool HB, bool WCHK = false>
__device__ __forceinline__ void pp_account(const DecodeArgs &a, int *red, int grp, int (&sums)[6 * C], unsigned *redo,
                                           unsigned long long *acc)
{
    int *tot = red + kPPRedSums;
    const bool lane0 = (threadIdx.x & 63) == 0;
    if (!(LDPC_PP_TAILEXP & 4)) {
#pragma unroll
        for (int q = 0; q < 2 * C; ++q) {
            if constexpr (HB) {
                const int w = wave_sum3(sums[3 * q]), u = wave_sum3(sums[3 * q + 1]);
                if (lane0 && w) atomicAdd(&tot[3 * q], w);
                if (lane0 && u) atomicAdd(&tot[3 * q + 1], u);
            } else {
                if (__builtin_amdgcn_ballot_w64(sums[3 * q + 2] != 0) && lane0) atomicAdd(&tot[3 * q + 2], 1);
                if constexpr (WCHK) {
                    const int w = wave_sum3(sums[3 * q]);
                    if (lane0 && w) atomicAdd(&tot[3 * q], w);
                }
                if constexpr (LDPC_PP_CHAN_ALL || LDPC_PP_CHAN_SPLIT) {
                    const int u = wave_sum3(sums[3 * q + 1]);
                    if (lane0 && u) atomicAdd(&tot[3 * q + 1], u);
                }
            }
        }
    }
    __syncthreads();
    if (threadIdx.x == 0) {
#pragma unroll
        for (int v = 0; v < 6 * C; ++v) {
            sums[v] = tot[v];
            tot[v] = 0;
        }
        const int fl[2] = {red[0], red[1]};
        red[0] = red[1] = 0;
#pragma unroll
        for (int q = 0; q < 2 * C; ++q) {
            const int b = grp * 2 * C + q;
            if (b >= a.batch) continue;
            if (fl[q / C]) {
                const unsigned at = atomicAdd(&redo[0], 1u);
                redo[1 + at] = (unsigned)b;
                continue;
            }
            const int w = sums[3 * q], uc = sums[3 * q + 1], sf = sums[3 * q + 2] > 0;
            acc[0] += (unsigned long long)w;
            acc[1] += (unsigned long long)(w > 0);
            acc[2] += (unsigned long long)uc;
            acc[3] += 1ull;
            acc[5] += (unsigned long long)sf;
            if (w > 0 && a.hist) atomicAdd(&a.hist[w - 1], 1ull);
            if (a.frame_res) a.frame_res[b] = make_int4(w, uc, sf, 0);
        }
    }
}

template <typename F, int DC, int VAR, bool FDIV, int C, int DCA, typename Store>
__device__ __forceinline__ bool pp_check_node(const Pack<F, C> (&xin)[DCA], Pack<F, C> (&pv)[DCA], F alpha, F rcp,
                                              F delta, Store store, uint32_t *pacc)
{
    if constexpr (sizeof(F) == 8) {
        return cn_fast64<DC, VAR, FDIV, DCA, Store, LDPC_PP_STORE_ORDER != 0, true>(xin, pv, alpha, rcp, delta, store,
                                                                                     pacc);
    } else {
        return cn_fast_pair<DC, DCA, Store, LDPC_PP_STORE_ORDER != 0>(xin, pv, VAR == V_NMS, alpha, rcp, store);
    }
}

template <typename F, int SRC, int DC0, int DC1, int CPT, int VAR, bool FDIV, int R, bool HB, int IR = 0>
__device__ __forceinline__ void pp_role(const DecodeArgs &a, const DevGraph &g, const RowSched &rs,
                                        const PPSlots<Pack<F, PPCw<F>::C>> &s, unsigned *redo,
                                        unsigned long long *acc)
{
    constexpr int C = PPCw<F>::C;
    using P = Pack<F, C>;
    constexpr int DCX = 8;
    constexpr int RR = R > 0 ? R : 1;
    static_assert(DC0 <= DCX && DC1 <= DCX && (R == 0) == HB, "pp_role shape");
    static_assert(IR == 0 || R == 2, "in-register bits: two rows per check thread");
    constexpr int L0 = DC0 - 1, L1 = DC1 - 1;
    constexpr bool F64 = sizeof(F) == 8;
    const F kMax = F64 ? (F)kFast64Max : (F)1e30f;
    const int tid = threadIdx.x, N = g.N, lane = tid & 63;
    [[maybe_unused]] const int EA = rs.e_pad + 64;
    [[maybe_unused]] int deg[RR];
    [[maybe_unused]] uint32_t colw[RR][DCX / 2], posw[RR][DCX / 2];
    [[maybe_unused]] P prev[2][RR][DCX];
    if constexpr (R > 0) {
#pragma unroll
        for (int r = 0; r < R; ++r) {
            const int j = tid + r * kPPRole;
            deg[r] = rs.cn_deg[j];
            const uint4 xc = reinterpret_cast<const uint4 *>(rs.cn_cols + (size_t)j * DCX)[0];
            const uint4 xp = reinterpret_cast<const uint4 *>(rs.cn_pos + (size_t)j * DCX)[0];
            colw[r][0] = xc.x; colw[r][1] = xc.y; colw[r][2] = xc.z; colw[r][3] = xc.w;
            posw[r][0] = xp.x; posw[r][1] = xp.y; posw[r][2] = xp.z; posw[r][3] = xp.w;
            if (deg[r] == 0)
#pragma unroll
                for (int q = 0; q < DCX / 2; ++q) colw[r][q] = (uint32_t)(N + 2) * 0x10001u;
        }
    }
    [[maybe_unused]] bool has = IR == 1, fr1 = false;
    if constexpr (IR != 0) {
        const uint32_t pf = rs.pair[LDPC_CHK(tid, kPPRole, CHK_PP_GATHER)];
        if (IR == 2) has = (pf & 1u) != 0;
        fr1 = DC0 != DC1 && (pf & 2u) != 0;
        if (IR == 1 && deg[0] == 0)
            colw[0][L0 / 2] = (L0 & 1) ? (colw[0][L0 / 2] & 0xffffu) | ((uint32_t)N << 16)
                                       : (colw[0][L0 / 2] & 0xffff0000u) | (uint32_t)N;
    }
    [[maybe_unused]] auto inreg_sum = [&](auto Xc, const P &y) -> P {
        constexpr int X = decltype(Xc)::value;
        P sum;
#pragma unroll
        for (int c = 0; c < C; ++c) {
            const F p0 = prev[X][0][L0].v[c], p1 = prev[X][RR - 1][L1].v[c];
            sum.v[c] = (y.v[c] + (fr1 ? p1 : p0)) + (fr1 ? p0 : p1);
        }
        return sum;
    };
    const int bt = tid - kPPRole;
    [[maybe_unused]] int vgb[CPT], vgd[CPT];
    [[maybe_unused]] uint32_t vdst2[(CPT + 1) / 2] = {};
    if constexpr (HB) {
#pragma unroll
        for (int i = 0; i < CPT; ++i) {
            const int c = rs.vn_col[bt * CPT + i];
            vdst2[i / 2] |= (uint32_t)(c == 0xffff ? N + 1 : c) << (16 * (i & 1));
            const uint32_t info = rs.vn_info[bt * CPT + i];
            vgb[i] = __builtin_amdgcn_readfirstlane((int)(info & 0xffffu) - lane);
            vgd[i] = __builtin_amdgcn_readfirstlane((int)(info >> 24));
        }
        P z;
#pragma unroll
        for (int c = 0; c < C; ++c) z.v[c] = F(0);
#pragma unroll
        for (int i = 0; i < CPT; ++i) {
            const int dg = (int)((rs.vn_info[bt * CPT + i] >> 16) & 0xffu);
            const int base = vgb[i] + lane, gd = vgd[i];
            for (int k = dg; k < gd; ++k) {
                const int e = LDPC_CHK(base + k * 64, EA, CHK_PP_BIT_READ);
                s.c2v[0][e] = s.c2v[1][e] = z;
            }
        }
    }
    auto vdst = [&](int i) -> int { return (int)((vdst2[i / 2] >> (16 * (i & 1))) & 0xffffu); };
    const F alpha = (F)a.alpha, delta = (F)a.delta;
    F rcp = F64 ? (F)(1.0 / a.alpha) : (F)a.alpha_rcp;
    if constexpr (F64 && LDPC_PP_SBASE && R > 0)
        rcp = mkd((uint32_t)__builtin_amdgcn_readfirstlane((int)lo32(rcp)), (uint32_t)__builtin_amdgcn_readfirstlane((int)hi32(rcp)));
    const int nsteps = (a.batch + 2 * C - 1) / (2 * C);
    if constexpr (HB && LDPC_PP_NOB2) {
        P inf, zero;
#pragma unroll
        for (int c = 0; c < C; ++c) {
            inf.v[c] = dinf<F>();
            zero.v[c] = F(0);
        }
        if (tid == kPPRole) s.app[0][N] = s.app[1][N] = inf;
        if (tid == kPPRole + 1) s.app[0][N + 2] = s.app[1][N + 2] = zero;
    }
    PP_STAMP_DECL;
    for (int grp = blockIdx.x; grp < nsteps; grp += gridDim.x) {
        PP_STAMP_TOP();
        [[maybe_unused]] uint32_t pacc[2] = {0u, 0u};
        constexpr bool TF = (LDPC_PP_TAILFUSE & (F64 ? 2 : 1)) != 0;
        int unc[2 * C];
        [[maybe_unused]] int wdec[2 * C];
        [[maybe_unused]] int synd0[C];
#pragma unroll
        for (int q = 0; q < 2 * C; ++q) unc[q] = wdec[q] = 0;
        [[maybe_unused]] unsigned chan_bad = 0;
        if constexpr (LDPC_PP_CHAN_ALL && !HB) {
            if (!(LDPC_PP_TAILEXP & 1)) pp_channel<F, SRC>(a, s, N, grp, unc, tid, 2 * kPPRole, &chan_bad);
        }
        [[maybe_unused]] const bool split = LDPC_PP_CHAN_SPLIT && SRC == SRC_PHILOX && LDPC_PP_NOB2 &&
                                            !(LDPC_PP_TAILEXP & 1) && pp_plain_step(a, N, grp, C);
        if constexpr (LDPC_PP_CHAN_SPLIT && !HB) {
            if (split) pp_channel_plain<F>(a, s, N, grp, unc, tid, 2 * kPPRole, &chan_bad);
        }
        if constexpr (HB) {
            if (LDPC_PP_CHAN_SPLIT && split) {
                pp_channel_plain<F>(a, s, N, grp, unc, tid, 2 * kPPRole, &chan_bad);
            } else if (!(LDPC_PP_TAILEXP & 1)) {
                pp_channel<F, SRC>(a, s, N, grp, unc, LDPC_PP_CHAN_ALL ? tid : bt, LDPC_PP_CHAN_ALL ? 2 * kPPRole : kPPRole,
                                   &chan_bad);
            } else {
                for (int q = 0; q < 2 * C; ++q) unc[q] = 0;
                for (int v = bt; v < N; v += kPPRole)
                    for (int c = 0; c < C; ++c) s.app[0][v].v[c] = s.app[1][v].v[c] = F(1);
            }
        }
        PP_SYNC_STAMPED(1);
        [[maybe_unused]] P yq[2][CPT];
        if constexpr (R > 0) {
#pragma unroll
            for (int X = 0; X < 2; ++X)
#pragma unroll
                for (int r = 0; r < R; ++r)
#pragma unroll
                    for (int k = 0; k < DCX; ++k)
#pragma unroll
                        for (int c = 0; c < C; ++c) prev[X][r][k].v[c] = F(0);
        }
        if constexpr ((LDPC_PP_CHAN_SPLIT || (LDPC_PP_CHAN_ALL && LDPC_PP_NOB2)) && !HB) {
            if (__builtin_amdgcn_ballot_w64(chan_bad != 0)) {
                if (chan_bad & 1u) s.red[0] = 1;
                if (chan_bad & 2u) s.red[1] = 1;
            }
        }
        if constexpr (HB && LDPC_PP_NOB2) {
            if (__builtin_amdgcn_ballot_w64(chan_bad != 0)) {
                if (chan_bad & 1u) s.red[0] = 1;
                if (chan_bad & 2u) s.red[1] = 1;
            }
#pragma unroll
            for (int X = 0; X < 2; ++X)
#pragma unroll
                for (int i = 0; i < CPT; ++i)
                    yq[X][i] = s.app[X][LDPC_CHK(vdst(i) < N ? vdst(i) : N + 2, N + 3, CHK_PP_APP_WRITE)];
        } else if constexpr (HB) {
#pragma unroll
            for (int X = 0; X < 2; ++X) {
                bool in_ok = true;
#pragma unroll
                for (int i = 0; i < CPT; ++i) {
                    const P st = s.app[X][LDPC_CHK(vdst(i) <= N ? vdst(i) : 0, N + 3, CHK_PP_APP_WRITE)];
#pragma unroll
                    for (int c = 0; c < C; ++c) {
                        yq[X][i].v[c] = st.v[c] + F(0);
                        in_ok &= dabs(yq[X][i].v[c]) < kMax;
                    }
                }
#pragma unroll
                for (int i = 0; i < CPT; ++i) s.app[X][LDPC_CHK(vdst(i), N + 3, CHK_PP_APP_WRITE)] = yq[X][i];
                if (!in_ok) s.red[X] = 1;
            }
            P inf, zero;
#pragma unroll
            for (int c = 0; c < C; ++c) {
                inf.v[c] = dinf<F>();
                zero.v[c] = F(0);
            }
            if (tid == kPPRole) s.app[0][N] = s.app[1][N] = inf;
            if (tid == kPPRole + 1) s.app[0][N + 2] = s.app[1][N + 2] = zero;
        }
        if constexpr (!LDPC_PP_NOB2) PP_SYNC_STAMPED(3);

        auto decide = [&](int Y, const P *post, int *w) {
            const bool plain = (SRC == SRC_GIVEN ? !a.c : !a.cw_table) && !a.d_out;
            if (plain) {
#pragma unroll
                for (int c = 0; c < C; ++c) {
                    const int q = Y * C + c;
                    int e = 0;
#pragma unroll
                    for (int i = 0; i < CPT; ++i) e += (vdst(i) < N && !(post[i].v[c] > F(0))) ? 1 : 0;
                    w[q] = grp * 2 * C + q < a.batch ? e : 0;
                }
                return;
            }
#pragma unroll
            for (int c = 0; c < C; ++c) {
                const int q = Y * C + c, b = grp * 2 * C + q;
                if (b >= a.batch) continue;
                const int8_t *cvec =
                    SRC == SRC_GIVEN ? (a.c ? a.c + (size_t)b * N : nullptr)
                                     : (a.cw_table ? a.cw_table + (size_t)((a.first_cw + (uint64_t)b) % (uint64_t)a.cw_rows) * N
                                                   : nullptr);
                int e = 0;
#pragma unroll
                for (int i = 0; i < CPT; ++i) {
                    const int v = vdst(i);
                    if (v < N) {
                        const int d = post[i].v[c] > F(0) ? 1 : -1;
                        const int cv = cvec ? cvec[v] : 1;
                        e += (d != cv);
                        if (a.d_out) a.d_out[(size_t)b * N + v] = (int8_t)d;
                    }
                }
                w[q] = e;
            }
        };
        constexpr bool YREG = IR == 1 && LDPC_PP_INREG_Y;
        [[maybe_unused]] P yreg[2];
        if constexpr (YREG) {
#pragma unroll
            for (int X = 0; X < 2; ++X) yreg[X] = s.app[X][LDPC_CHK(u16_at<DCX>(colw[0], L0), N + 3, CHK_PP_GATHER)];
        }
        [[maybe_unused]] P ipost[2];
        [[maybe_unused]] auto inreg_final = [&](auto Xc) {
            constexpr int X = decltype(Xc)::value;
            ipost[X] = inreg_sum(Xc, YREG ? yreg[X] : s.app[X][LDPC_CHK(u16_at<DCX>(colw[0], L0), N + 3, CHK_PP_GATHER)]);
        };
        auto syndrome = [&](int X, int c) -> int {
            int synd = 0;
            if constexpr (R > 0) {
                static_for<0, R>([&](auto rc) {
                    constexpr int r = decltype(rc)::value, DCr = r == 0 ? DC0 : DC1;
                    int par = 0;
#pragma unroll
                    for (int k = 0; k < DCr; ++k) {
                        if (IR == 1 && k == DCr - 1) continue;
                        const int neg = (s.app[X][LDPC_CHK(u16_at<DCX>(colw[r], k), N + 3, CHK_PP_GATHER)].v[c] > F(0)) ? 0 : 1;
                        par ^= (IR == 2 && k == DCr - 1 && has) ? 0 : neg;
                    }
                    if constexpr (IR != 0) par ^= (has && !(ipost[X].v[c] > F(0))) ? 1 : 0;
                    synd |= deg[r] > 0 ? par : 0;
                });
            }
            return synd;
        };

        auto interval = [&](auto Xc, bool rows, bool bits, bool last) {
            constexpr int X = decltype(Xc)::value, Y = 1 - X;
            [[maybe_unused]] P xin[RR][DCX];
            if constexpr (R > 0) {
                if (rows && LDPC_PP_EXP != 2) {
#pragma unroll
                    for (int r = 0; r < R; ++r)
#pragma unroll
                        for (int q = 0; q < DCX / 2; ++q) asm volatile("" : "+v"(colw[r][q]), "+v"(posw[r][q]));
                    const uint32_t ab = s.app_base[X];
                    static_for<0, (LDPC_PP_PREFETCH ? R : 1)>([&](auto rc) {
                        constexpr int r = decltype(rc)::value, DCr = r == 0 ? DC0 : DC1;
#pragma unroll
                        for (int k = 0; k < DCr - (IR == 1 && (r == 1 || YREG) ? 1 : 0); ++k)
                            xin[r][k] = lds_at<P>((LDPC_PP_EXP == 5 || LDPC_PP_EXP == 7) ? ab + 8u * (uint32_t)(lane + 64 * (k + 8 * r))
                                                                                         : PP_ADDR8(DCX, colw[r], k, ab, N + 3, CHK_PP_GATHER));
                    });
                    if constexpr (LDPC_PP_GATHER_FIRST && LDPC_PP_PREFETCH) {
                        constexpr int NG = DC0 + (R > 1 ? DC1 : 0);
                        __builtin_amdgcn_sched_group_barrier(0x2, NG, 1);
                        __builtin_amdgcn_sched_group_barrier(0x100, NG, 1);
                    }
                }
            }
            if constexpr (HB) {
                if (LDPC_PP_BITDELAY > 0) __builtin_amdgcn_s_sleep(LDPC_PP_BITDELAY);
                if (bits && LDPC_PP_EXP != 1) {
#pragma unroll
                    for (int q = 0; q < (CPT + 1) / 2; ++q) asm volatile("" : "+v"(vdst2[q]));
                    P sum[CPT];
#pragma unroll
                    for (int i = 0; i < CPT; ++i) sum[i] = yq[Y][i];
                    int k = 0;
                    const int ln = (int)__builtin_amdgcn_mbcnt_hi(~0u, __builtin_amdgcn_mbcnt_lo(~0u, 0u));
                    vn_phases<F, C, CPT, CPT>(s.c2v[Y] + ln, vgb, vgd, k, sum, LDPC_CHK_LIM(EA - ln), CHK_PP_BIT_READ);
#pragma unroll
                    for (int i = 0; i < CPT; ++i) s.app[Y][LDPC_CHK(vdst(i), N + 3, CHK_PP_APP_WRITE)] = sum[i];
                    if (TF && last) decide(Y, sum, wdec);
                }
            }
            if constexpr (R > 0) {
                if (rows && LDPC_PP_EXP != 2) {
                    const uint32_t ab = s.app_base[X], cb = s.c2v_base[X];
                    if constexpr (IR != 0) {
                        if constexpr (YREG) xin[0][L0] = yreg[X];
                        const P sum = inreg_sum(Xc, xin[0][L0]);
#pragma unroll
                        for (int c = 0; c < C; ++c) {
                            xin[0][L0].v[c] = has ? sum.v[c] : xin[0][L0].v[c];
                            xin[RR - 1][L1].v[c] = has ? sum.v[c] : xin[RR - 1][L1].v[c];
                        }
                    }
                    constexpr int ILV = (F64 && R == 2 && LDPC_PP_PREFETCH && LDPC_PP_STORE_ORDER && LDPC_PP_EXP == 0) ? LDPC_PP_ILV : 0;
                    using Front = std::conditional_t<(ILV > 0), CnFront64<DC1>, int>;
                    [[maybe_unused]] Front fr;
                    [[maybe_unused]] uint32_t pa1 = 0;
                    static_for<0, R>([&](auto rc) {
                        constexpr int r = decltype(rc)::value, DCr = r == 0 ? DC0 : DC1;
                        if (!LDPC_PP_PREFETCH && r > 0) {
#pragma unroll
                            for (int k = 0; k < DCr; ++k) xin[r][k] = lds_at<P>(LDPC_ADDR8(DCX, colw[r], k, ab, N + 3, CHK_PP_GATHER));
                        }
                        bool ok = true;
                        auto store = [&](int k, const P &m) {
                            if (IR == 1 && k == DCr - 1) return;
                            if constexpr (LDPC_PP_EXP != 4)
                                lds_put<P>((LDPC_PP_EXP == 6 || LDPC_PP_EXP == 7)
                                               ? cb + 8u * (uint32_t)(lane + 64 * ((k + 8 * r + 16 * (tid >> 6)) % 112))
                                               : PP_ADDR8(DCX, posw[r], k, cb, EA, CHK_PP_SCATTER),
                                           m);
                        };
                        if constexpr (LDPC_PP_EXP == 3) {
#pragma unroll
                            for (int k = 0; k < DCr; ++k) {
#pragma unroll
                                for (int c = 0; c < C; ++c) prev[X][r][k].v[c] = xin[r][k].v[c] - prev[X][r][k].v[c];
                                store(k, prev[X][r][k]);
                            }
                        } else {
                            constexpr bool ONE = F64 && !LDPC_PP_STICKY && LDPC_PP_ONEPREM && R == 2;
                            [[maybe_unused]] uint32_t pa0 = 0;
                            uint32_t &pa = ONE ? pa1 : pa0;
                            if constexpr (ILV > 0) {
                                constexpr int NF = Front::N, SK = LDPC_PP_ILV_SKIP, CUT = ILV * (DC0 - SK) < NF ? ILV * (DC0 - SK) : NF;
                                if constexpr (r == 0) {
                                    auto fill = [&](int k) {
                                        static_for<0, CUT>([&](auto ic) {
                                            constexpr int I = decltype(ic)::value;
                                            if (I / ILV + SK == k) fr.template step<I>(xin[1], prev[X][1]);
                                        });
                                    };
                                    ok = cn_fast64<DCr, VAR, FDIV, DCX, decltype(store), true, true, decltype(fill), ILV>(
                                        xin[r], prev[X][r], alpha, rcp, delta, store, LDPC_PP_STICKY ? &pacc[X] : &pa, fill);
                                } else {
                                    static_for<CUT, NF>([&](auto ic) { fr.template step<decltype(ic)::value>(xin[1], prev[X][1]); });
                                    ok = cn_fast64_back<DCr, VAR, FDIV, DCX, decltype(store), true, true>(
                                        fr.x, fr.mn1, fr.mn2, fr.par, prev[X][r], alpha, rcp, delta, store,
                                        LDPC_PP_STICKY ? &pacc[X] : &pa);
                                }
                            } else {
                                ok = pp_check_node<F, DCr, VAR, FDIV>(xin[r], prev[X][r], alpha, rcp, delta, store,
                                                                      LDPC_PP_STICKY ? &pacc[X] : &pa);
                            }
                            if constexpr (F64 && !LDPC_PP_STICKY && (!ONE || r == R - 1)) {
                                if (__builtin_amdgcn_ballot_w64(pa >= kFast64MaxHi)) {
                                    asm volatile(";");
                                    if (pa >= kFast64MaxHi && LDPC_PP_EXP == 0) s.red[X] = 1;
                                }
                            }
                        }
                        if (!ok && deg[r] > 0 && LDPC_PP_EXP == 0) s.red[X] = 1;
                        if (R > 1 && LDPC_PP_ROWFENCE) __builtin_amdgcn_sched_barrier(0);
                    });
                }
            }
        };
        for (int it = 0; it < a.T; ++it) {
            interval(std::integral_constant<int, 0>(), true, it > 0, false);
            PP_BARRIER();
            interval(std::integral_constant<int, 1>(), true, true, it == a.T - 1);
            PP_BARRIER();
        }
        if (a.T > 0) {
            interval(std::integral_constant<int, 0>(), false, true, true);
            if (TF && !(LDPC_PP_TAILEXP & 2)) {
                if constexpr (IR != 0) inreg_final(std::integral_constant<int, 0>());
#pragma unroll
                for (int c = 0; c < C; ++c) synd0[c] = syndrome(0, c);
            }
            PP_BARRIER();
        }
        if constexpr (F64 && R > 0 && LDPC_PP_STICKY) {
            if (pacc[0] >= kFast64MaxHi && LDPC_PP_EXP == 0) s.red[0] = 1;
            if (pacc[1] >= kFast64MaxHi && LDPC_PP_EXP == 0) s.red[1] = 1;
        }

        if (LDPC_PP_TAILEXP & 2) {
            int sums[6 * C] = {};
            pp_account<C, HB, IR != 0>(a, s.red, grp, sums, redo, acc);
            continue;
        }
        const bool fused = TF && a.T > 0;
        if constexpr (HB) {
            if (!fused) {
#pragma unroll
                for (int X = 0; X < 2; ++X) {
                    P post[CPT];
#pragma unroll
                    for (int i = 0; i < CPT; ++i) post[i] = s.app[X][LDPC_CHK(vdst(i) <= N ? vdst(i) : 0, N + 3, CHK_PP_APP_WRITE)];
                    decide(X, post, wdec);
                }
            }
        }
        if constexpr (IR != 0) {
            inreg_final(std::integral_constant<int, 0>());
            inreg_final(std::integral_constant<int, 1>());
            const int v = u16_at<DCX>(colw[0], L0);
            if (has && v < N) {
#pragma unroll
                for (int q = 0; q < 2 * C; ++q) {
                    const int b = grp * 2 * C + q;
                    if (b >= a.batch) continue;
                    const int8_t *cvec =
                        SRC == SRC_GIVEN ? (a.c ? a.c + (size_t)b * N : nullptr)
                                         : (a.cw_table ? a.cw_table + (size_t)((a.first_cw + (uint64_t)b) % (uint64_t)a.cw_rows) * N
                                                       : nullptr);
                    const int d = ipost[q / C].v[q % C] > F(0) ? 1 : -1;
                    wdec[q] += d != (cvec ? cvec[v] : 1);
                    if (a.d_out) a.d_out[(size_t)b * N + v] = (int8_t)d;
                }
            }
        }
        int sums[6 * C];
#pragma unroll
        for (int X = 0; X < 2; ++X) {
#pragma unroll
            for (int c = 0; c < C; ++c) {
                const int q = X * C + c;
                sums[3 * q] = wdec[q];
                sums[3 * q + 1] = unc[q];
                sums[3 * q + 2] = (X == 0 && fused) ? synd0[c] : syndrome(X, c);
            }
        }
        PP_STAMP_ACC(5);
        pp_account<C, HB, IR != 0>(a, s.red, grp, sums, redo, acc);
    }
    PP_STAMP_OUT()
}

}

LDPC_CHECK_TU(rows_pp)

#ifndef LDPC_PP_ENTRY_NOPS
#define LDPC_PP_ENTRY_NOPS 0
#endif

template <typename F, int SRC, int CPT, int VAR, bool FDIV, bool SPLIT, bool INREG>
__device__ __forceinline__ void pp_kernel(const DecodeArgs &a, const DevGraph &g, const RowSched &rs, unsigned *redo)
{
    static_assert(!INREG || SPLIT, "in-register bits come with the degree-aware row slots");
    using P = Pack<F, PPCw<F>::C>;
    extern __shared__ __attribute__((aligned(16))) unsigned char smem[];
#pragma unroll
    for (int i = 0; i < LDPC_PP_ENTRY_NOPS; ++i) asm volatile("s_nop 0");
    const PPSlots<P> s = pp_slots<P>(smem, g.N, rs.e_pad + 64);
    unsigned long long *acc = reinterpret_cast<unsigned long long *>(s.red + kPPRedAcc);
    if (threadIdx.x == 0) {
        s.red[0] = s.red[1] = 0;
#pragma unroll
        for (int q = 0; q < 6; ++q) acc[q] = 0;
#pragma unroll
        for (int v = 0; v < 3 * kPPMaxCw; ++v) s.red[kPPRedSums + v] = 0;
    }
    const int wave = __builtin_amdgcn_readfirstlane(threadIdx.x >> 6);
    const bool low = wave < kPPRole / 64;
    if (LDPC_PP_PRIO == 1 && low) __builtin_amdgcn_s_setprio(1);
    if (LDPC_PP_PRIO == 2 && !low) __builtin_amdgcn_s_setprio(1);
    if (LDPC_PP_PRIO == 3 && ((threadIdx.x >> 8) & 1)) __builtin_amdgcn_s_setprio(1);
    if (LDPC_PP_PRIO == 4 && low && wave >= kPPRole / 128) __builtin_amdgcn_s_setprio(1);
    if (LDPC_PP_PRIO == 5 && low) {
        if (wave >= kPPRole / 128) __builtin_amdgcn_s_setprio(2);
        else __builtin_amdgcn_s_setprio(1);
    }
    if constexpr (INREG) {
        const bool pure = low && __builtin_amdgcn_readfirstlane((int)rs.pair[kPPRole + (low ? wave : 0)]) != 0;
        if (!low)
            pp_role<F, SRC, 8, 8, CPT, VAR, FDIV, 0, true>(a, g, rs, s, redo, acc);
        else if (wave >= kPPRole / 128) {
            if (pure) pp_role<F, SRC, 7, 7, CPT, VAR, FDIV, 2, false, 1>(a, g, rs, s, redo, acc);
            else pp_role<F, SRC, 7, 7, CPT, VAR, FDIV, 2, false, 2>(a, g, rs, s, redo, acc);
        } else {
            if (pure) pp_role<F, SRC, 7, 8, CPT, VAR, FDIV, 2, false, 1>(a, g, rs, s, redo, acc);
            else pp_role<F, SRC, 7, 8, CPT, VAR, FDIV, 2, false, 2>(a, g, rs, s, redo, acc);
        }
    } else if (!low)
        pp_role<F, SRC, 8, 8, CPT, VAR, FDIV, 0, true>(a, g, rs, s, redo, acc);
    else if (!SPLIT)
        pp_role<F, SRC, 8, 8, CPT, VAR, FDIV, 2, false>(a, g, rs, s, redo, acc);
    else if (wave >= kPPRole / 128)
        pp_role<F, SRC, 7, 7, CPT, VAR, FDIV, 2, false>(a, g, rs, s, redo, acc);
    else
        pp_role<F, SRC, 7, 8, CPT, VAR, FDIV, 2, false>(a, g, rs, s, redo, acc);
    if (threadIdx.x == 0 && acc[3] > 0) {
        acc[4] = acc[3] * (unsigned long long)a.T;
#pragma unroll
        for (int q = 0; q < 6; ++q) atomicAdd(&a.counts[q], acc[q]);
    }
}

template <typename F, int SRC, int CPT, int VAR, bool FDIV, bool SPLIT>
__global__ __launch_bounds__(2 * kPPRole) void k_rows_pp(DecodeArgs a, DevGraph g, RowSched rs, unsigned *redo)
{
    pp_kernel<F, SRC, CPT, VAR, FDIV, SPLIT, false>(a, g, rs, redo);
}

template <typename F, int SRC, int CPT, int VAR, bool FDIV>
__global__ __launch_bounds__(2 * kPPRole) void k_rows_ppi(DecodeArgs a, DevGraph g, RowSched rs, unsigned *redo)
{
    pp_kernel<F, SRC, CPT, VAR, FDIV, true, true>(a, g, rs, redo);
}

static int rows_pp_lds_bytes(const DevGraph &g, const RowSched &rs)
{
    return (int)(2 * (size_t)pp_slot_words(g.N, rs.e_pad + 64) * 8 + kPPRedInts * sizeof(int));
}

static bool rows_pp_supported(const DevGraph &g, const RowSched &rs)
{
    return rs.threads == kPPRole && rs.rpt == 2 && (rs.cpt == 4 || (rs.pair && rs.cpt == 3)) && rs.dc == 8 && (rs.dc_low == 0 || rs.dc_low == 7) &&
           g.N <= 4 * kPPRole && g.N + 3 <= 0xffff && rows_pp_lds_bytes(g, rs) <= 160 * 1024;
}

template <typename F, int SRC, int VAR, bool FDIV>
static const void *pp_fn_t(const RowSched &rs)
{
    if constexpr (sizeof(F) == 8)
        if (rs.pair)
            return rs.cpt == 3 ? (const void *)k_rows_ppi<F, SRC, 3, VAR, FDIV> : (const void *)k_rows_ppi<F, SRC, 4, VAR, FDIV>;
    return rs.dc_low == 7 ? (const void *)k_rows_pp<F, SRC, 4, VAR, FDIV, true>
                          : (const void *)k_rows_pp<F, SRC, 4, VAR, FDIV, false>;
}

static const void *pp_fn(const RowSched &rs, const DecodeArgs &a, bool f64)
{
    const bool given = a.src == SRC_GIVEN;
#define LDPC_PP_SRC(FT, VARV, FD) \
    return given ? pp_fn_t<FT, SRC_GIVEN, VARV, FD>(rs) : pp_fn_t<FT, SRC_PHILOX, VARV, FD>(rs);
    if (!f64) {
        if (a.variant == V_MS) { LDPC_PP_SRC(float, V_MS, false) }
        if (a.variant == V_NMS && a.nms_fast) { LDPC_PP_SRC(float, V_NMS, false) }
        return nullptr;
    }
    if (a.variant == V_MS) { LDPC_PP_SRC(double, V_MS, false) }
    if (a.variant == V_OMS) { LDPC_PP_SRC(double, V_OMS, false) }
    if (markstein_exact_alpha(a.alpha)) { LDPC_PP_SRC(double, V_NMS, true) }
    LDPC_PP_SRC(double, V_NMS, false)
#undef LDPC_PP_SRC
}

bool plan_rows_pp(const PlanInput &in, LaunchPlan &p)
{
    const RowSched *rs = in.rs_pp && opt(LDPC_OPT_PP_SLOTS) != 1 ? in.rs_pp : in.rs;
    if (!rows_pp_supported(in.g, *rs)) return false;
    const RowSched *ri = nullptr;
    if (in.f64 && LDPC_PP_NOB2 && LDPC_PP_PREFETCH && rs == in.rs_pp && in.rs_ppi && opt(LDPC_OPT_PP_SLOTS) == 0 &&
        rs->dc_low == 7 && in.rs_ppi->pair && in.rs_ppi->e_pad == rs->e_pad && rows_pp_supported(in.g, *in.rs_ppi))
        ri = in.rs_ppi;
    p.kernel = Kernel::rows_pp;
    p.name = "rows_pp";
    p.redo = true;
    p.rs = rs;
    p.rs_inreg = ri;
    p.fn = pp_fn(ri ? *ri : *rs, in.a, in.f64);
    p.threads = 2 * kPPRole;
    p.lds_bytes = rows_pp_lds_bytes(in.g, *rs);
    p.blocks_per_cu = 1;
    const int CW = 2 * (in.f64 ? PPCw<double>::C : PPCw<float>::C);
    p.grid = std::min(in.num_cus, (in.a.batch + CW - 1) / CW);
    return true;
}

hipError_t launch_rows_pp(const LaunchPlan &p, const DevGraph &g, const DecodeArgs &a, unsigned *redo, hipStream_t s)
{
    void *args[] = {(void *)&a, (void *)&g, (void *)(p.rs_inreg ? p.rs_inreg : p.rs), &redo};
    return launch_fn(p, args, s);
}

}
```

ldpcsimulation_amd/native.py:

```python
from __future__ import annotations

import ctypes as C
import os
from dataclasses import dataclass, field
from typing import Optional

import numpy as np

_PKG = os.path.dirname(os.path.abspath(__file__))
LIB_PATH = os.path.join(_PKG, "lib", "libldpc_hip.so")

LDPC_OK = 0
MS, NMS, OMS, BP, DDBMP = 0, 1, 2, 3, 4
F32, F64 = 0, 1
FLOODING, LAYERED = 0, 1
ABI_VERSION = 11
OPTIONS = {"rows64": 1, "rows32": 2, "pp_slots": 3, "kernel": 4, "flood_mode": 5, "flood_msg": 6,
           "flood_sps_check": 7, "flood_sps_bit": 8, "flood_resident": 9, "flood_streams": 10, "flood_bpc": 11,
           "layered_bpc": 12, "layered_lds_pos": 13, "layered_rows64": 14, "layered_threads": 15,
           "rows_bpc": 16, "fast_bpc": 17, "bp_kernel": 18, "gdbf_kernel": 19, "ems_threads": 20,
           "ems_swizzle": 21, "ddbmp_kernel": 22}
EMS_OPTIONS = ("ems_threads", "ems_swizzle")
OPTION_VALUES = {"rows64": {"pp": 0, "fast": 1, "rows": 2}, "rows32": {"pp": 0, "fast": 1, "rows": 2},
                 "pp_slots": {"split": 0, "plain": 1, "split_lds": 2}, "kernel": {"auto": 0, "lds": 1, "flood": 2, "global": 3},
                 "flood_mode": {"phase": 0, "persistent": 1}, "flood_msg": {"packed": 0, "c2v": 1},
                 "bp_kernel": {"rows": 0, "generic": 1}, "gdbf_kernel": {"rows": 0, "generic": 1},
                 "ddbmp_kernel": {"rows": 0, "generic": 1},
                 "ems_swizzle": {"on": 0, "off": 1}}


def option_id(name) -> int:
    return name if isinstance(name, int) else OPTIONS[name]


def option_value(name, value) -> int:
    if isinstance(value, str) and not isinstance(name, int):
        return OPTION_VALUES[name][value]
    return int(value)


def use_library(path: str):
    global LIB_PATH
    if _lib is not None and os.path.abspath(path) != os.path.abspath(LIB_PATH):
        raise RuntimeError("the decoder library is already loaded")
    LIB_PATH = path
_STATUS = {0: "OK", -1: "INVALID", -2: "NOMEM", -3: "DEVICE", -4: "UNSUPPORTED", -5: "IO", -6: "GRAPH"}


class LdpcError(RuntimeError):
    def __init__(self, code: int, msg: str):
        super().__init__(f"ldpc error {code} ({_STATUS.get(code, '?')}): {msg}")
        self.code = code


class Counts(C.Structure):
    _fields_ = [("bit_err", C.c_int64), ("frame_err", C.c_int64), ("uncoded_bit_err", C.c_int64),
                ("frames", C.c_int64), ("iters", C.c_int64), ("syndrome_fail", C.c_int64)]

    def as_dict(self) -> dict:
        return {k: int(getattr(self, k)) for k, _ in self._fields_}

    def as_array(self) -> np.ndarray:
        return np.array([getattr(self, k) for k, _ in self._fields_], dtype=np.int64)


FRAME_DTYPE = np.dtype([("bit_err", np.int32), ("uncoded_bit_err", np.int32),
                        ("syndrome_fail", np.int32), ("iters", np.int32)])


class _Cfg(C.Structure):
    _fields_ = [("variant", C.c_int32), ("precision", C.c_int32), ("T", C.c_int32),
                ("quantize", C.c_int32), ("saturate", C.c_int32), ("qbits", C.c_int32),
                ("ymax", C.c_double), ("alpha", C.c_double), ("delta", C.c_double),
                ("schedule", C.c_int32), ("early_stop", C.c_int32), ("n0", C.c_double), ("max_llr", C.c_double)]


GDBF_NOISE, GDBF_ADAPT, GDBF_WEIGHT, GDBF_SMOOTH, GDBF_SATURATE, GDBF_QUANTIZE = 1, 2, 4, 8, 16, 32
GDBF_SEQUENTIAL, GDBF_MODESWITCH, GDBF_QPROB = 64, 128, 256
GDBF_VARIANTS = {
    "MNGDBF": GDBF_NOISE | GDBF_ADAPT | GDBF_WEIGHT | GDBF_SATURATE,
    "SMNGDBF": GDBF_NOISE | GDBF_ADAPT | GDBF_WEIGHT | GDBF_SMOOTH | GDBF_SATURATE,
    "ATGDBF": GDBF_ADAPT,
    "SATGDBF": GDBF_ADAPT | GDBF_SMOOTH,
    "SMGDBF": GDBF_SMOOTH,
    "SGDBF": GDBF_SEQUENTIAL,
    "MGDBF": GDBF_MODESWITCH,
    "StochasticNGDBF": GDBF_QUANTIZE | GDBF_QPROB | GDBF_WEIGHT | GDBF_SATURATE,
}


class _GdbfCfg(C.Structure):
    _fields_ = [("flags", C.c_int32), ("precision", C.c_int32), ("T", C.c_int32), ("windowsize", C.c_int32),
                ("nq", C.c_int32), ("tswitch", C.c_int32), ("theta", C.c_double), ("lambda_", C.c_double),
                ("alpha", C.c_double), ("noise_scale", C.c_double), ("ymax", C.c_double), ("qsigma", C.c_double)]


@dataclass
class GdbfConfig:
    flags: int = GDBF_VARIANTS["SMNGDBF"]
    T: int = 100
    theta: float = -0.6
    lambda_: float = 0.99
    alpha: float = 0.8
    noise_scale: float = 0.75
    ymax: float = 2.5
    windowsize: int = 16
    nq: int = 16
    precision: int = 1
    tswitch: int = 0
    qsigma: float = 0.0

    def _c(self) -> _GdbfCfg:
        return _GdbfCfg(self.flags, self.precision, self.T, self.windowsize, self.nq, self.tswitch, self.theta,
                        self.lambda_, self.alpha, self.noise_scale, self.ymax, self.qsigma)


RGDBF_FLAGS = GDBF_NOISE | GDBF_ADAPT | GDBF_WEIGHT | GDBF_SMOOTH | GDBF_SATURATE


class _RgdbfCfg(C.Structure):
    _fields_ = [("flags", C.c_int32), ("precision", C.c_int32), ("T", C.c_int32), ("maxphase", C.c_int32),
                ("windowsize", C.c_int32), ("reserved", C.c_int32), ("theta", C.c_double), ("lambda_", C.c_double),
                ("alpha", C.c_double), ("noise_scale", C.c_double), ("ymax", C.c_double)]


@dataclass
class RgdbfConfig:
    flags: int = RGDBF_FLAGS
    T: int = 100
    maxphase: int = 3
    theta: float = -0.6
    lambda_: float = 0.99
    alpha: float = 0.96
    noise_scale: float = 0.75
    ymax: float = 2.5
    windowsize: int = 16
    precision: int = 1

    def _c(self) -> _RgdbfCfg:
        return _RgdbfCfg(self.flags, self.precision, self.T, self.maxphase, self.windowsize, 0, self.theta,
                         self.lambda_, self.alpha, self.noise_scale, self.ymax)


class _RstatCfg(C.Structure):
    _fields_ = [("flags", C.c_int32), ("precision", C.c_int32), ("T", C.c_int32), ("attempts", C.c_int32),
                ("windowsize", C.c_int32), ("first_attempt", C.c_int32), ("theta", C.c_double),
                ("lambda_", C.c_double), ("alpha", C.c_double), ("noise_scale", C.c_double), ("ymax", C.c_double)]


class _RstatTrace(C.Structure):
    _fields_ = [("err_trace", C.c_void_p), ("unsat_trace", C.c_void_p), ("d_trace", C.c_void_p),
                ("s_trace", C.c_void_p)]


ATTEMPT_DTYPE = np.dtype([("bit_err", np.int32), ("iters", np.int32), ("syndrome_fail", np.int32),
                          ("smoothing_used", np.int32)])


@dataclass
class RstatConfig:
    flags: int = RGDBF_FLAGS
    T: int = 100
    attempts: int = 5
    first_attempt: int = 0
    theta: float = -0.6
    lambda_: float = 0.99
    alpha: float = 0.96
    noise_scale: float = 0.75
    ymax: float = 2.5
    windowsize: int = 16
    precision: int = 1

    def _c(self) -> _RstatCfg:
        return _RstatCfg(self.flags, self.precision, self.T, self.attempts, self.windowsize, self.first_attempt,
                         self.theta, self.lambda_, self.alpha, self.noise_scale, self.ymax)


# ... 22 lines not shown

class _FxmsCfg(C.Structure):
    _fields_ = [("variant", C.c_int32), ("precision", C.c_int32), ("T", C.c_int32), ("qbits", C.c_int32),
                ("msg_bits", C.c_int32), ("nms_num", C.c_int32), ("nms_shift", C.c_int32), ("beta", C.c_int32),
                ("early_stop", C.c_int32), ("reserved", C.c_int32), ("ymax", C.c_double)]


@dataclass
class FxmsConfig:
    variant: int = MS
    T: int = 10
    qbits: int = 5
    msg_bits: int = 6
    nms_num: int = 3
    nms_shift: int = 2
    beta: int = 1
    early_stop: bool = False
    ymax: float = 31 / 16
    precision: int = F64

    def _c(self) -> _FxmsCfg:
        return _FxmsCfg(self.variant, self.precision, self.T, self.qbits, self.msg_bits, self.nms_num, self.nms_shift,
                        self.beta, int(self.early_stop), 0, self.ymax)


class _FxlmsCfg(C.Structure):
    _fields_ = [("variant", C.c_int32), ("precision", C.c_int32), ("T", C.c_int32), ("qbits", C.c_int32),
                ("msg_bits", C.c_int32), ("app_bits", C.c_int32), ("nms_num", C.c_int32), ("nms_shift", C.c_int32),
                ("beta", C.c_int32), ("early_stop", C.c_int32), ("ymax", C.c_double)]


@dataclass
class FxlmsConfig:
    variant: int = MS
    T: int = 10
    qbits: int = 5
    msg_bits: int = 6
    app_bits: Optional[int] = None
    nms_num: int = 3
    nms_shift: int = 2
    beta: int = 1
    early_stop: bool = False
    ymax: float = 31 / 16
    precision: int = F64

    def __post_init__(self):
        if self.app_bits is None:
            self.app_bits = min(self.msg_bits + 1, 16)

    def _c(self) -> _FxlmsCfg:
        return _FxlmsCfg(self.variant, self.precision, self.T, self.qbits, self.msg_bits, self.app_bits, self.nms_num,
                         self.nms_shift, self.beta, int(self.early_stop), self.ymax)


def rgdbf_phases(iters, T: int, maxphase: int):
    return np.minimum(maxphase, np.asarray(iters) // T + 1)


def rgdbf_smoothing_used(iters, T: int, maxphase: int, windowsize: int):
    iters = np.asarray(iters)
    p = rgdbf_phases(iters, T, maxphase)
    last = iters - (p - 1) * T
    return (p - 1) * int(windowsize > 0) + (last > T - windowsize)


@dataclass
class DecoderConfig:
    variant: int = MS
    T: int = 10
    precision: int = F64
    alpha: float = 1.0
    delta: float = 0.0
    quantize: bool = False
    saturate: bool = False
    ymax: float = 0.0
    qbits: int = 0
    schedule: int = FLOODING
    n0: float = 0.0
    max_llr: float = 0.0
    early_stop: bool = False

    def _c(self) -> _Cfg:
        return _Cfg(self.variant, self.precision, self.T, int(self.quantize), int(self.saturate),
                    self.qbits, self.ymax, self.alpha, self.delta, self.schedule, int(self.early_stop), self.n0,
                    self.max_llr)


class _EmsCfg(C.Structure):
    _fields_ = [("T", C.c_int32), ("nm", C.c_int32), ("early_stop", C.c_int32), ("reserved", C.c_int32),
                ("offset", C.c_double)]


class NbCounts(C.Structure):
    _fields_ = [(k, C.c_int64) for k in ("bit_err", "frame_err", "uncoded_bit_err", "frames", "iters",
                                         "syndrome_fail", "symbol_err")]

    def as_dict(self) -> dict:
        return {k: getattr(self, k) for k, _ in self._fields_}


@dataclass
class EmsConfig:
    T: int = 20
    nm: int = 16
    offset: float = 0.0
    early_stop: bool = True

    def _c(self) -> _EmsCfg:
        return _EmsCfg(self.T, self.nm, int(self.early_stop), 0, self.offset)


_vp, _i32, _u32, _u64, _dbl = C.c_void_p, C.c_int, C.c_uint32, C.c_uint64, C.c_double
_pi32 = C.POINTER(C.c_int)


def _sim(cfg, *outs):
    return [_vp, _dbl, _dbl, C.POINTER(cfg), _u64, _u32, _u64, _i32, *outs]


def _info(cfg, *more):
    return [_vp, C.POINTER(cfg), *more, C.c_char_p, _i32, _pi32]


_SIG = {
    "ldpc_abi_version": ([], _i32),
    "ldpc_f64_nms_fast_division": ([_dbl], _i32),
    "ldpc_bp_math_probe": ([_i32, _vp, _i32, _vp, _vp], _i32),
    "ldpc_check_selftest": ([_i32], _i32),
    "ldpc_last_error": ([], C.c_char_p),
    "ldpc_graph_create": ([_i32, _i32, _vp, _vp, _vp, _vp, C.POINTER(_vp)], _i32),
    "ldpc_graph_load_alist": ([C.c_char_p, C.POINTER(_vp)], _i32),
    "ldpc_graph_info": ([_vp] + [_pi32] * 5, _i32),
    "ldpc_graph_destroy": ([_vp], None),
    "ldpc_graph_layers": ([_vp, _vp, _vp, _pi32], _i32),
    "ldpc_device_count": ([_pi32], _i32),
    "ldpc_ctx_create": ([_i32, _vp, _i32, C.POINTER(_vp)], _i32),
    "ldpc_ctx_set_stream": ([_vp, _vp], _i32),
    "ldpc_ctx_synchronize": ([_vp], _i32),
    "ldpc_ctx_destroy": ([_vp], None),
    "ldpc_decode_batch": ([_vp, _vp, _i32, C.POINTER(_Cfg), _vp, _vp, _vp, C.POINTER(Counts)], _i32),
    "ldpc_sim_set_codewords": ([_vp, _vp, _i32], _i32),
    "ldpc_sim_launch": (_sim(_Cfg, _vp), _i32),
    "ldpc_ctx_read_counts": ([_vp, C.POINTER(Counts), _i32], _i32),
    "ldpc_ctx_read_histogram": ([_vp, _vp, _i32], _i32),
    "ldpc_sim_batch": (_sim(_Cfg, _vp, C.POINTER(Counts)), _i32),
    "ldpc_sim_trace": (_sim(_Cfg, _vp, _vp, _vp, C.POINTER(Counts)), _i32),
    "ldpc_ctx_last_kernel_ms": ([_vp, C.POINTER(C.c_float)], _i32),
    "ldpc_ctx_kernel_info": (_info(_Cfg) + [_pi32], _i32),
    "ldpc_ctx_redo_count": ([_vp, C.POINTER(C.c_int64)], _i32),
    "ldpc_ctx_redo_list": ([_vp, _vp, C.c_int64, C.POINTER(C.c_int64)], _i32),
    "ldpc_ctx_pp_row_slots": ([_vp, _vp, _vp, _vp, C.c_int, C.POINTER(C.c_int)], _i32),
    "ldpc_ctx_row_sched_info": ([_vp, C.POINTER(_Cfg), _vp], _i32),
    "ldpc_ctx_pp_inreg_info": ([_vp, C.POINTER(_Cfg), _vp], _i32),
    "ldpc_ctx_set_option": ([_vp, _i32, _i32], _i32),
    "ldpc_ctx_get_option": ([_vp, _i32, _pi32], _i32),
    "ldpc_nb_ctx_set_option": ([_vp, _i32, _i32], _i32),
    "ldpc_gdbf_decode_batch": ([_vp, _vp, _vp, _i32, C.POINTER(_GdbfCfg), _vp, _vp, _vp, C.POINTER(Counts)], _i32),
    "ldpc_gdbf_sim_launch": (_sim(_GdbfCfg, _vp), _i32),
    "ldpc_gdbf_sim_batch": (_sim(_GdbfCfg, _vp, C.POINTER(Counts)), _i32),
    "ldpc_gdbf_kernel_info": (_info(_GdbfCfg), _i32),
    "ldpc_rgdbf_decode_batch": ([_vp, _vp, _vp, _i32, C.POINTER(_RgdbfCfg), _vp, _vp, _vp, C.POINTER(Counts)], _i32),
    "ldpc_rgdbf_sim_launch": (_sim(_RgdbfCfg, _vp), _i32),
    "ldpc_rgdbf_sim_batch": (_sim(_RgdbfCfg, _vp, C.POINTER(Counts)), _i32),
    "ldpc_rgdbf_kernel_info": (_info(_RgdbfCfg), _i32),
    "ldpc_rstat_decode_batch": ([_vp, _vp, _vp, _i32, C.POINTER(_RstatCfg), _vp, _vp, C.POINTER(_RstatTrace), _vp,
                                 _vp, C.POINTER(Counts)], _i32),
    "ldpc_rstat_sim_launch": (_sim(_RstatCfg, _vp, C.POINTER(_RstatTrace), _vp), _i32),
    "ldpc_rstat_sim_batch": (_sim(_RstatCfg, _vp, C.POINTER(_RstatTrace), _vp, C.POINTER(Counts)), _i32),
    "ldpc_rstat_sim_trace": (_sim(_RstatCfg, _vp, _vp, _vp, C.POINTER(_RstatTrace), _vp, _vp, C.POINTER(Counts)),
                              _i32),
    "ldpc_rstat_kernel_info": (_info(_RstatCfg, _i32), _i32),
    "ldpc_hwgdbf_decode_batch": ([_vp, _vp, _vp, _vp, _i32, C.POINTER(_HwGdbfCfg), _vp, _vp, _vp, _vp,
                                  C.POINTER(Counts)], _i32),
    "ldpc_hwgdbf_sim_launch": (_sim(_HwGdbfCfg, _vp), _i32),
    "ldpc_hwgdbf_sim_batch": (_sim(_HwGdbfCfg, _vp, C.POINTER(Counts)), _i32),
    "ldpc_hwgdbf_sim_trace": (_sim(_HwGdbfCfg, _vp, _vp, _vp, _vp, C.POINTER(Counts)), _i32),
    "ldpc_hwgdbf_kernel_info": (_info(_HwGdbfCfg), _i32),
    "ldpc_fxms_decode_batch": ([_vp, _vp, _i32, C.POINTER(_FxmsCfg), _vp, _vp, _vp, C.POINTER(Counts)], _i32),
    "ldpc_fxms_sim_launch": (_sim(_FxmsCfg, _vp), _i32),
    "ldpc_fxms_sim_batch": (_sim(_FxmsCfg, _vp, C.POINTER(Counts)), _i32),
    "ldpc_fxms_sim_trace": (_sim(_FxmsCfg, _vp, _vp, _vp, _vp, C.POINTER(Counts)), _i32),
    "ldpc_fxms_kernel_info": (_info(_FxmsCfg), _i32),
    "ldpc_fxlms_decode_batch": ([_vp, _vp, _i32, C.POINTER(_FxlmsCfg), _vp, _vp, _vp, C.POINTER(Counts)], _i32),
    "ldpc_fxlms_sim_launch": (_sim(_FxlmsCfg, _vp), _i32),
    "ldpc_fxlms_sim_batch": (_sim(_FxlmsCfg, _vp, C.POINTER(Counts)), _i32),
    "ldpc_fxlms_sim_trace": (_sim(_FxlmsCfg, _vp, _vp, _vp, _vp, C.POINTER(Counts)), _i32),
    "ldpc_fxlms_kernel_info": (_info(_FxlmsCfg), _i32),
    "ldpc_nb_graph_create": ([_i32, _i32, _i32, _vp, _vp, _vp, _vp, _vp, _vp, C.POINTER(_vp)], _i32),
    "ldpc_nb_graph_load_alist": ([C.c_char_p, C.POINTER(_vp)], _i32),
    "ldpc_nb_graph_info": ([_vp] + [_pi32] * 6, _i32),
    "ldpc_nb_graph_destroy": ([_vp], None),
    "ldpc_nb_ctx_create": ([_i32, _vp, _i32, C.POINTER(_vp)], _i32),
    "ldpc_nb_ctx_set_stream": ([_vp, _vp], _i32),
    "ldpc_nb_ctx_destroy": ([_vp], None),
    "ldpc_nb_ctx_read_counts": ([_vp, C.POINTER(NbCounts), _i32], _i32),
    "ldpc_nb_ctx_last_kernel_ms": ([_vp, C.POINTER(C.c_float)], _i32),
    "ldpc_ems_kernel_info": ([_vp, C.c_char_p, _i32, _pi32], _i32),
    "ldpc_ems_decode_batch": ([_vp, _vp, _i32, _dbl, C.POINTER(_EmsCfg), _vp, _vp, _vp, C.POINTER(NbCounts)], _i32),
    "ldpc_ems_sim_launch": (_sim(_EmsCfg, _vp), _i32),
    "ldpc_ems_sim_batch": (_sim(_EmsCfg, _vp, C.POINTER(NbCounts)), _i32),
    "ldpc_ems_sim_trace": (_sim(_EmsCfg, _vp, _vp, _vp, C.POINTER(NbCounts)), _i32),
}
EXPORTED = list(_SIG)

_lib = None


_ADDED_IN_ABI = {"ldpc_ctx_pp_inreg_info", "ldpc_ctx_redo_list", "ldpc_ctx_pp_row_slots", "ldpc_fxms_decode_batch",
                 "ldpc_fxms_sim_launch", "ldpc_fxms_sim_batch", "ldpc_fxms_sim_trace", "ldpc_fxms_kernel_info",
                 "ldpc_fxlms_decode_batch", "ldpc_fxlms_sim_launch", "ldpc_fxlms_sim_batch", "ldpc_fxlms_sim_trace",
                 "ldpc_fxlms_kernel_info"}


def lib():
    global _lib
    if _lib is not None:
        return _lib
    if not os.path.exists(LIB_PATH):
        raise ImportError(f"HIP decoder library not built: {LIB_PATH} (run __graft_entry__.build() or `make`)")
    try:
        import torch
    except ImportError:
        pass
    L = C.CDLL(LIB_PATH)
    for name, (argt, rest) in _SIG.items():
        if name in _ADDED_IN_ABI and not hasattr(L, name):
            continue
        fn = getattr(L, name)
        fn.argtypes = argt
        fn.restype = rest
    if L.ldpc_abi_version() != ABI_VERSION:
        raise ImportError(f"{LIB_PATH}: ABI version {L.ldpc_abi_version()}, this binding needs {ABI_VERSION}")
    _lib = L
    return L


def _check(rc: int):
    if rc != LDPC_OK:
        raise LdpcError(rc, lib().ldpc_last_error().decode(errors="replace"))


def device_count() -> int:
    n = C.c_int(0)
    rc = lib().ldpc_device_count(C.byref(n))
    return n.value if rc == LDPC_OK else 0


class Graph:

    def __init__(self, handle):
        self._h = handle
        N, M, E, dv, dc = (C.c_int() for _ in range(5))
        _check(lib().ldpc_graph_info(self._h, C.byref(N), C.byref(M), C.byref(E), C.byref(dv), C.byref(dc)))
        self.N, self.M, self.E, self.maxdv, self.maxdc = N.value, M.value, E.value, dv.value, dc.value

    @classmethod
    def from_alist(cls, path: str) -> "Graph":
        h = C.c_void_p()
        _check(lib().ldpc_graph_load_alist(os.fspath(path).encode(), C.byref(h)))
        return cls(h)

    @classmethod
    def from_lists(cls, N: int, M: int, nlist, mlist) -> "Graph":
        num_n = (C.c_int * N)(*[len(x) for x in nlist])
        num_m = (C.c_int * M)(*[len(x) for x in mlist])
        keep = [(C.c_int * max(len(x), 1))(*x) for x in nlist] + [(C.c_int * max(len(x), 1))(*x) for x in mlist]
        np_ = (C.c_void_p * N)(*[C.cast(a, C.c_void_p) for a in keep[:N]])
        mp_ = (C.c_void_p * M)(*[C.cast(a, C.c_void_p) for a in keep[N:]])
        h = C.c_void_p()
        _check(lib().ldpc_graph_create(N, M, num_n, np_, num_m, mp_, C.byref(h)))
        return cls(h)

    def layers(self):
        n = C.c_int()
        _check(lib().ldpc_graph_layers(self._h, None, None, C.byref(n)))
        order = np.empty(self.M, dtype=np.int32)
        ptr = np.empty(n.value + 1, dtype=np.int32)
        _check(lib().ldpc_graph_layers(self._h, order.ctypes.data, ptr.ctypes.data, C.byref(n)))
        return order, ptr

    def __del__(self):
        h = getattr(self, "_h", None)
        if h and _lib is not None:
            _lib.ldpc_graph_destroy(h)
            self._h = None


def _ptr(a) -> Optional[int]:
    if a is None:
        return None
    if isinstance(a, np.ndarray):
        if not a.flags["C_CONTIGUOUS"]:
            raise ValueError("array must be C-contiguous")
        return a.ctypes.data
    if hasattr(a, "data_ptr"):
        if not a.is_contiguous():
            raise ValueError("tensor must be contiguous")
        return a.data_ptr()
    raise TypeError(type(a))


def _given(N: int, cfg, y, c=None):
    want = np.float64 if cfg.precision == F64 else np.float32
    y = np.ascontiguousarray(y, dtype=want).reshape(-1, N)
    if c is not None:
        c = np.ascontiguousarray(c, dtype=np.int8)
    return y, y.shape[0], c, want


def _sim_launch(fn, h, ebn0_db, R, cfg, seed, stream_id, first_cw, batch, *outs_dev):
    _check(fn(h, ebn0_db, R, C.byref(cfg._c()), seed, stream_id, first_cw, batch, *(_ptr(o) for o in outs_dev)))


def _sim_batch(fn, h, ebn0_db, R, cfg, seed, stream_id, first_cw, batch, *outs, want_frames=True, counts=None):
    fr = np.empty(batch, dtype=FRAME_DTYPE) if want_frames else None
    cnt = (counts or Counts)()
    outs = [_ptr(o) if isinstance(o, np.ndarray) else o for o in outs]
    _check(fn(h, ebn0_db, R, C.byref(cfg._c()), seed, stream_id, first_cw, batch, *outs, _ptr(fr), C.byref(cnt)))
    return fr, cnt


def _kernel_info(fn, *args) -> dict:
    name = C.create_string_buffer(32)
    lds = C.c_int()
    _check(fn(*args, name, 32, C.byref(lds)))
    return {"kernel": name.value.decode(), "lds_bytes": lds.value}


class Context:

    def __init__(self, graph: Graph, device: int = 0, max_batch: int = 65536):
        self.graph = graph
        self.device = device
        self.max_batch = max_batch
        h = C.c_void_p()
        _check(lib().ldpc_ctx_create(device, graph._h, max_batch, C.byref(h)))
        self._h = h

    def __del__(self):
        h = getattr(self, "_h", None)
        if h and _lib is not None:
            _lib.ldpc_ctx_destroy(h)
            self._h = None

    def set_stream(self, stream_handle: Optional[int]):
        _check(lib().ldpc_ctx_set_stream(self._h, stream_handle))

    def set_option(self, name, value):
        _check(lib().ldpc_ctx_set_option(self._h, option_id(name), option_value(name, value)))

    def get_option(self, name) -> int:
        v = C.c_int()
        _check(lib().ldpc_ctx_get_option(self._h, option_id(name), C.byref(v)))
        return int(v.value)

    def set_options(self, opts: Optional[dict]):
        for k, v in (opts or {}).items():
            self.set_option(k, v)

    def reset_options(self):
        for name, k in OPTIONS.items():
            if name not in EMS_OPTIONS:
                _check(lib().ldpc_ctx_set_option(self._h, k, 0))

    def synchronize(self):
        _check(lib().ldpc_ctx_synchronize(self._h))

    def decode(self, y, cfg: DecoderConfig, c=None, want_decisions: bool = True, want_frames: bool = True):
        N = self.graph.N
        if isinstance(y, np.ndarray):
            want = np.float64 if cfg.precision == F64 else np.float32
            if y.dtype != want:
                raise TypeError(f"y must be {np.dtype(want)} for this precision, got {y.dtype}")
            y = np.ascontiguousarray(y)
            size = y.size
        else:
            want = "torch.float64" if cfg.precision == F64 else "torch.float32"
            if str(y.dtype) != want:
                raise TypeError(f"y must be {want} for this precision, got {y.dtype}")
            size = y.numel()
        if size % N:
            raise ValueError(f"y has {size} elements, not a multiple of N={N}")
        batch = size // N
        if c is not None:
            if isinstance(c, np.ndarray):
                c = np.ascontiguousarray(c, dtype=np.int8)
            elif str(c.dtype) != "torch.int8":
                raise TypeError(f"c must be torch.int8 (bipolar +1/-1), got {c.dtype}")
            csize = c.size if isinstance(c, np.ndarray) else c.numel()
            if csize != batch * N:
                raise ValueError(f"c has {csize} elements, y {batch * N}")
        d = np.empty((batch, N), dtype=np.int8) if want_decisions else None
        fr = np.empty(batch, dtype=FRAME_DTYPE) if want_frames else None
        cnt = Counts()
        _check(lib().ldpc_decode_batch(self._h, _ptr(y), batch, C.byref(cfg._c()), _ptr(c), _ptr(d), _ptr(fr),
                                       C.byref(cnt)))
        return d, fr, cnt

    def set_codewords(self, bits: Optional[np.ndarray]):
        if bits is None:
            _check(lib().ldpc_sim_set_codewords(self._h, None, 0))
            return
        bits = np.ascontiguousarray(bits, dtype=np.uint8).reshape(-1, self.graph.N)
        _check(lib().ldpc_sim_set_codewords(self._h, bits.ctypes.data, bits.shape[0]))

    def sim_launch(self, ebn0_db: float, R: float, cfg: DecoderConfig, seed: int, stream_id: int, first_cw: int,
                   batch: int, frames_dev=None):
        _sim_launch(lib().ldpc_sim_launch, self._h, ebn0_db, R, cfg, seed, stream_id, first_cw, batch, frames_dev)

    def sim_batch(self, ebn0_db: float, R: float, cfg: DecoderConfig, seed: int, stream_id: int, first_cw: int,
                  batch: int, want_frames: bool = True):
        return _sim_batch(lib().ldpc_sim_batch, self._h, ebn0_db, R, cfg, seed, stream_id, first_cw, batch,
                          want_frames=want_frames)

    def sim_trace(self, ebn0_db: float, R: float, cfg: DecoderConfig, seed: int, stream_id: int, first_cw: int,
                  batch: int):
        N = self.graph.N
        y = np.empty((batch, N), dtype=np.float64 if cfg.precision == F64 else np.float32)
        d = np.empty((batch, N), dtype=np.int8)
        fr, cnt = _sim_batch(lib().ldpc_sim_trace, self._h, ebn0_db, R, cfg, seed, stream_id, first_cw, batch, y, d)
        return y, d, fr, cnt

    def read_counts(self, reset: bool = False) -> Counts:
        cnt = Counts()
        _check(lib().ldpc_ctx_read_counts(self._h, C.byref(cnt), int(reset)))
        return cnt

    def read_histogram(self, reset: bool = False) -> np.ndarray:
        h = np.zeros(self.graph.N, dtype=np.int64)
        _check(lib().ldpc_ctx_read_histogram(self._h, h.ctypes.data, int(reset)))
        return h

    def last_kernel_ms(self) -> float:
        ms = C.c_float()
        _check(lib().ldpc_ctx_last_kernel_ms(self._h, C.byref(ms)))
        return float(ms.value)

    def redo_count(self) -> int:
        n = C.c_int64()
        _check(lib().ldpc_ctx_redo_count(self._h, C.byref(n)))
        return int(n.value)

    def redo_list(self) -> np.ndarray:
        n = C.c_int64()
        out = np.zeros(max(self.redo_count(), 1), dtype=np.uint32)
        _check(lib().ldpc_ctx_redo_list(self._h, out.ctypes.data, out.size, C.byref(n)))
        return np.sort(out[:int(n.value)])

    def row_sched_info(self, cfg: DecoderConfig) -> dict:
        info = np.zeros(10, dtype=np.int32)
        _check(lib().ldpc_ctx_row_sched_info(self._h, C.byref(cfg._c()), info.ctypes.data))
        keys = ("threads", "rows_per_thread", "slots_per_thread", "dc", "e_pad", "cw_per_block", "lds_bytes",
                "blocks_per_cu", "dc_low", "issued_check_edges")
        return {k: int(v) for k, v in zip(keys, info)}

    def pp_inreg_info(self, cfg: DecoderConfig) -> dict:
        info = np.zeros(4, dtype=np.int32)
        _check(lib().ldpc_ctx_pp_inreg_info(self._h, C.byref(cfg._c()), info.ctypes.data))
        keys = ("inreg_bits", "lds_check_edges", "bit_slot_edges", "slots_per_thread")
        return {k: int(v) for k, v in zip(keys, info)}

    def pp_row_slots(self, cfg: DecoderConfig):
        cols = np.zeros((2048, 8), dtype=np.uint16)
        deg = np.zeros(2048, dtype=np.uint8)
        n = C.c_int()
        _check(lib().ldpc_ctx_pp_row_slots(self._h, C.byref(cfg._c()), cols.ctypes.data, deg.ctypes.data, 2048, C.byref(n)))
        return cols[:n.value], deg[:n.value]

    def kernel_info(self, cfg: DecoderConfig) -> dict:
        name = C.create_string_buffer(32)
        lds, bpc = C.c_int(), C.c_int()
        _check(lib().ldpc_ctx_kernel_info(self._h, C.byref(cfg._c()), name, 32, C.byref(lds), C.byref(bpc)))
        return {"kernel": name.value.decode(), "lds_bytes": lds.value, "blocks_per_cu": bpc.value}

    def _decode(self, fn, y, cfg, c, want_decisions, *ins):
        batch = y.shape[0]
        d = np.empty((batch, self.graph.N), dtype=np.int8) if want_decisions else None
        fr = np.empty(batch, dtype=FRAME_DTYPE)
        cnt = Counts()
        _check(fn(self._h, _ptr(y), *(_ptr(a) for a in ins), batch, C.byref(cfg._c()), _ptr(c), _ptr(d), _ptr(fr),
                  C.byref(cnt)))
        return d, fr, cnt

    def gdbf_decode(self, y, pert, cfg: GdbfConfig, c=None, want_decisions: bool = True):
        y, batch, c, want = _given(self.graph.N, cfg, y, c)
        if pert is not None:
            pert = np.ascontiguousarray(pert, dtype=want).reshape(batch, cfg.T, self.graph.N)
        return self._decode(lib().ldpc_gdbf_decode_batch, y, cfg, c, want_decisions, pert)

    def gdbf_sim_launch(self, ebn0_db: float, R: float, cfg: GdbfConfig, seed: int, stream_id: int, first_cw: int,
                        batch: int, frames_dev=None):
        _sim_launch(lib().ldpc_gdbf_sim_launch, self._h, ebn0_db, R, cfg, seed, stream_id, first_cw, batch, frames_dev)

    def gdbf_sim_batch(self, ebn0_db: float, R: float, cfg: GdbfConfig, seed: int, stream_id: int, first_cw: int,
                       batch: int, want_frames: bool = True):
        return _sim_batch(lib().ldpc_gdbf_sim_batch, self._h, ebn0_db, R, cfg, seed, stream_id, first_cw, batch,
                          want_frames=want_frames)

    def gdbf_kernel_info(self, cfg: GdbfConfig) -> dict:
        return _kernel_info(lib().ldpc_gdbf_kernel_info, self._h, C.byref(cfg._c()))

    def rgdbf_decode(self, y, pert, cfg: RgdbfConfig, c=None, want_decisions: bool = True):
        y, batch, c, want = _given(self.graph.N, cfg, y, c)
        if pert is not None:
            pert = np.ascontiguousarray(pert, dtype=want).reshape(batch, cfg.maxphase * cfg.T, self.graph.N)
        return self._decode(lib().ldpc_rgdbf_decode_batch, y, cfg, c, want_decisions, pert)

    def rgdbf_sim_launch(self, ebn0_db: float, R: float, cfg: RgdbfConfig, seed: int, stream_id: int, first_cw: int,
                         batch: int, frames_dev=None):
        _sim_launch(lib().ldpc_rgdbf_sim_launch, self._h, ebn0_db, R, cfg, seed, stream_id, first_cw, batch, frames_dev)

    def rgdbf_sim_batch(self, ebn0_db: float, R: float, cfg: RgdbfConfig, seed: int, stream_id: int, first_cw: int,
                        batch: int, want_frames: bool = True):
        return _sim_batch(lib().ldpc_rgdbf_sim_batch, self._h, ebn0_db, R, cfg, seed, stream_id, first_cw, batch,
                          want_frames=want_frames)

    def rgdbf_kernel_info(self, cfg: RgdbfConfig) -> dict:
        return _kernel_info(lib().ldpc_rgdbf_kernel_info, self._h, C.byref(cfg._c()))

    def _rstat_trace(self, batch: int, cfg: RstatConfig, want: bool):
        if not want:
            return None, None
        shape = (batch, cfg.attempts, cfg.T)
        tr = {"err_trace": np.empty(shape, dtype=np.int32), "unsat_trace": np.empty(shape, dtype=np.int32),
              "d_trace": np.empty(shape + (self.graph.N,), dtype=np.int8),
              "s_trace": np.empty(shape + (self.graph.M,), dtype=np.int8)}
        return C.byref(_RstatTrace(*(tr[k].ctypes.data for k, _ in _RstatTrace._fields_))), tr

    def rstat_decode(self, y, pert, cfg: RstatConfig, c=None, want_trace: bool = False):
        N = self.graph.N
        y, batch, c, want = _given(N, cfg, y, c)
        if pert is not None:
            pert = np.ascontiguousarray(pert, dtype=want).reshape(batch, cfg.attempts, cfg.T, N)
        att = np.empty((batch, cfg.attempts), dtype=ATTEMPT_DTYPE)
        d = np.empty((batch, N), dtype=np.int8)
        fr = np.empty(batch, dtype=FRAME_DTYPE)
        cnt = Counts()
        targ, tr = self._rstat_trace(batch, cfg, want_trace)
        _check(lib().ldpc_rstat_decode_batch(self._h, _ptr(y), _ptr(pert), batch, C.byref(cfg._c()), _ptr(c),
                                             _ptr(att), targ, _ptr(d), _ptr(fr), C.byref(cnt)))
        return att, d, fr, cnt, tr

    def rstat_sim_launch(self, ebn0_db: float, R: float, cfg: RstatConfig, seed: int, stream_id: int, first_cw: int,
                         batch: int, attempts_dev=None, frames_dev=None, trace_dev: Optional[dict] = None):
        targ = None
        if trace_dev:
            unknown = set(trace_dev) - {k for k, _ in _RstatTrace._fields_}
            if unknown:
                raise KeyError(f"unknown trace {sorted(unknown)}")
            targ = _RstatTrace(*(_ptr(trace_dev.get(k)) for k, _ in _RstatTrace._fields_))
        _check(lib().ldpc_rstat_sim_launch(self._h, ebn0_db, R, C.byref(cfg._c()), seed, stream_id, first_cw, batch,
                                           _ptr(attempts_dev), targ and C.byref(targ), _ptr(frames_dev)))

    def rstat_sim(self, ebn0_db: float, R: float, cfg: RstatConfig, seed: int, stream_id: int, first_cw: int,
                  batch: int, want_trace: bool = False):
        att = np.empty((batch, cfg.attempts), dtype=ATTEMPT_DTYPE)
        targ, tr = self._rstat_trace(batch, cfg, want_trace)
        fr, cnt = _sim_batch(lib().ldpc_rstat_sim_batch, self._h, ebn0_db, R, cfg, seed, stream_id, first_cw, batch,
                             att, targ)
        return att, fr, cnt, tr

    def rstat_sim_trace(self, ebn0_db: float, R: float, cfg: RstatConfig, seed: int, stream_id: int, first_cw: int,
                        batch: int, want_trace: bool = False):
        N = self.graph.N
        want = np.float64 if cfg.precision == F64 else np.float32
        y = np.empty((batch, N), dtype=want)
        pert = np.empty((batch, cfg.attempts, cfg.T, N), dtype=want)
        att = np.empty((batch, cfg.attempts), dtype=ATTEMPT_DTYPE)
        d = np.empty((batch, N), dtype=np.int8)
        targ, tr = self._rstat_trace(batch, cfg, want_trace)
        fr, cnt = _sim_batch(lib().ldpc_rstat_sim_trace, self._h, ebn0_db, R, cfg, seed, stream_id, first_cw, batch,
                             y, pert, att, targ, d)
        return y, pert, att, d, fr, cnt, tr

    def rstat_kernel_info(self, cfg: RstatConfig, with_trace: bool = False) -> dict:
        return _kernel_info(lib().ldpc_rstat_kernel_info, self._h, C.byref(cfg._c()), int(with_trace))

    def hwgdbf_decode(self, y, q, cfg: HwGdbfConfig, qptr0=None, c=None, want_decisions: bool = True):
        N = self.graph.N
        y, batch, c, want = _given(N, cfg, y, c)
        q = np.ascontiguousarray(q, dtype=want).reshape(batch, cfg.qlen)
        if qptr0 is not None:
            qptr0 = np.ascontiguousarray(qptr0, dtype=np.int32).reshape(batch)
        d = np.empty((batch, N), dtype=np.int8) if want_decisions else None
        fr = np.empty(batch, dtype=FRAME_DTYPE)
        run = np.empty(batch, dtype=np.int32)
        cnt = Counts()
        _check(lib().ldpc_hwgdbf_decode_batch(self._h, _ptr(y), _ptr(q), _ptr(qptr0), batch, C.byref(cfg._c()),
                                              _ptr(c), _ptr(d), _ptr(fr), _ptr(run), C.byref(cnt)))
        return d, fr, run, cnt

    def hwgdbf_sim_launch(self, ebn0_db: float, R: float, cfg: HwGdbfConfig, seed: int, stream_id: int,
                          first_cw: int, batch: int, frames_dev=None):
        _sim_launch(lib().ldpc_hwgdbf_sim_launch, self._h, ebn0_db, R, cfg, seed, stream_id, first_cw, batch, frames_dev)

    def hwgdbf_sim_batch(self, ebn0_db: float, R: float, cfg: HwGdbfConfig, seed: int, stream_id: int, first_cw: int,
                         batch: int, want_frames: bool = True):
        return _sim_batch(lib().ldpc_hwgdbf_sim_batch, self._h, ebn0_db, R, cfg, seed, stream_id, first_cw, batch,
                          want_frames=want_frames)

    def hwgdbf_sim_trace(self, ebn0_db: float, R: float, cfg: HwGdbfConfig, seed: int, stream_id: int, first_cw: int,
                         batch: int):
        N = self.graph.N
        want = np.float64 if cfg.precision == F64 else np.float32
        y = np.empty((batch, N), dtype=want)
        q = np.empty((batch, cfg.qlen), dtype=want)
        d = np.empty((batch, N), dtype=np.int8)
        fr, cnt = _sim_batch(lib().ldpc_hwgdbf_sim_trace, self._h, ebn0_db, R, cfg, seed, stream_id, first_cw, batch,
                             y, q, d)
        return y, q, d, fr, cnt

    def hwgdbf_kernel_info(self, cfg: HwGdbfConfig) -> dict:
        return _kernel_info(lib().ldpc_hwgdbf_kernel_info, self._h, C.byref(cfg._c()))

# ... 161 lines not shown
```

Before: 11460.

## Add 12-wave ping-pong f64 kernel with merged bit threads and fixed LDS layout

Adds a new default variant of the f64 in-register ping-pong row kernel that launches 1.5x kPPRole threads instead of 2x. The bit-update side has fewer threads, each interleaving two former threads' columns ordered by degree. It uses a fixed-stride LDS layout so gather and scatter addresses can be precomputed and held unpacked in registers. The intent is to cut idle bit-role waves and per-iteration address arithmetic. In exchange it raises register pressure per bit thread, pads LDS and serialises more bit work per thread.

Result: faster. 12130, median of 6 (+5.8%).

```diff
diff --git a/include/ldpc_hip.h b/include/ldpc_hip.h
--- a/include/ldpc_hip.h
+++ b/include/ldpc_hip.h
@@ -107,6 +107,8 @@
 int  ldpc_ctx_pp_inreg_info(ldpc_ctx *ctx, const ldpc_decoder_cfg *cfg, int32_t *info);
 int  ldpc_ctx_pp_row_slots(ldpc_ctx *ctx, const ldpc_decoder_cfg *cfg, uint16_t *cols, uint8_t *deg, int cap,
                            int *nslots);
+int  ldpc_ctx_pp_block_info(ldpc_ctx *ctx, const ldpc_decoder_cfg *cfg, int32_t *info);
+int  ldpc_pp_block_layout(int n_bits, int e_pad, int32_t *info);
 
 typedef enum {
     LDPC_OPT_ROWS64 = 1,
diff --git a/ldpcsimulation_amd/csrc/api.cpp b/ldpcsimulation_amd/csrc/api.cpp
--- a/ldpcsimulation_amd/csrc/api.cpp
+++ b/ldpcsimulation_amd/csrc/api.cpp
@@ -117,7 +117,7 @@
     switch (option) {
     case LDPC_OPT_ROWS64:
     case LDPC_OPT_ROWS32: return v >= 0 && v <= 2;
-    case LDPC_OPT_PP_SLOTS: return v >= 0 && v <= 2;
+    case LDPC_OPT_PP_SLOTS: return v >= 0 && v <= 3;
     case LDPC_OPT_FLOOD_MODE:
     case LDPC_OPT_FLOOD_MSG:
     case LDPC_OPT_BP_KERNEL:
@@ -895,6 +895,27 @@
     return LDPC_OK;
 }
 
+int ldpc_pp_block_layout(int n_bits, int e_pad, int32_t *info)
+{
+    if (!info) return set_err(LDPC_ERR_INVALID, "null argument");
+    int bytes = 0;
+    info[0] = ldpc::pp_w12_layout(n_bits, e_pad, &bytes) ? 1 : 0;
+    info[1] = bytes;
+    return LDPC_OK;
+}
+
+int ldpc_ctx_pp_block_info(ldpc_ctx *c, const ldpc_decoder_cfg *cfg, int32_t *info)
+{
+    if (!info) return set_err(LDPC_ERR_INVALID, "null argument");
+    ldpc::LaunchPlan p;
+    RC_TRY(info_plan(c, cfg, p));
+    if (p.kernel != ldpc::Kernel::rows_pp || !p.rs)
+        return set_err(LDPC_ERR_UNSUPPORTED, "the ping-pong kernel does not decode this cfg (kernel %s)", p.name);
+    info[0] = p.threads;
+    info[1] = p.lds_bytes + p.cache_lds_bytes + p.pad_lds_bytes;
+    return LDPC_OK;
+}
+
 int ldpc_ctx_pp_row_slots(ldpc_ctx *c, const ldpc_decoder_cfg *cfg, uint16_t *cols, uint8_t *deg, int cap, int *nslots)
 {
     if (!cols || !deg || !nslots || cap < 0) return set_err(LDPC_ERR_INVALID, "null argument");
diff --git a/ldpcsimulation_amd/csrc/kernels.h b/ldpcsimulation_amd/csrc/kernels.h
--- a/ldpcsimulation_amd/csrc/kernels.h
+++ b/ldpcsimulation_amd/csrc/kernels.h
@@ -91,6 +91,7 @@
     int lds_bytes = 0;
     int layered_pos = 0;
     int cache_lds_bytes = 0;
+    int pad_lds_bytes = 0;
     int cw_per_block = 1;
     int blocks_per_cu = 0;
     int grid = 0;
@@ -159,6 +160,7 @@
                        int num_cus);
 
 bool plan_rows_pp(const PlanInput &in, LaunchPlan &p);
+bool pp_w12_layout(int N, int e_pad, int *lds_bytes);
 #ifndef LDPC_PP_INREG_CPT
 #define LDPC_PP_INREG_CPT 3
 #endif
diff --git a/ldpcsimulation_amd/csrc/kernels.hip b/ldpcsimulation_amd/csrc/kernels.hip
--- a/ldpcsimulation_amd/csrc/kernels.hip
+++ b/ldpcsimulation_amd/csrc/kernels.hip
@@ -192,7 +192,7 @@
 
 hipError_t launch_fn(const LaunchPlan &p, void **args, hipStream_t s)
 {
-    const int lds = p.lds_bytes + p.cache_lds_bytes;
+    const int lds = p.lds_bytes + p.cache_lds_bytes + p.pad_lds_bytes;
     if (!p.fn || p.grid <= 0) return hipErrorInvalidValue;
     if (lds > 0) {
         const hipError_t e = hipFuncSetAttribute(p.fn, hipFuncAttributeMaxDynamicSharedMemorySize, lds);
diff --git a/ldpcsimulation_amd/csrc/rows_pp.hip b/ldpcsimulation_amd/csrc/rows_pp.hip
--- a/ldpcsimulation_amd/csrc/rows_pp.hip
+++ b/ldpcsimulation_amd/csrc/rows_pp.hip
@@ -87,6 +87,15 @@
 #endif
 #ifndef LDPC_PP_ONEPREM
 #define LDPC_PP_ONEPREM 1
+#endif
+#ifndef LDPC_PP_W12_UNP
+#define LDPC_PP_W12_UNP 1
+#endif
+#ifndef LDPC_PP_W12_K0
+#define LDPC_PP_W12_K0 12
+#endif
+#ifndef LDPC_PP_W12_K1
+#define LDPC_PP_W12_K1 4
 #endif
 #if LDPC_PP_SBASE && !defined(LDPC_CHECK)
 #define PP_ADDR8(DC, w, k, base, n, site) addr8<DC, true>(w, k, base)
@@ -162,13 +171,26 @@
 
 __host__ __device__ constexpr int pp_slot_words(int N, int EA) { return (N + 3 + EA + 1) & ~1; }
 
-template <typename P>
+constexpr uint32_t kPPAppStride = 16384, kPPC2vStride = 65520, kPPC2vDist = kPPC2vStride + 8;
+
+template <typename P, bool FIX = false>
 __device__ __forceinline__ PPSlots<P> pp_slots(unsigned char *smem, int N, int EA)
 {
     static_assert(sizeof(P) == 8, "one 8-byte LDS word per slot element");
     PPSlots<P> s;
+    P *b = reinterpret_cast<P *>(smem);
+    if constexpr (FIX) {
+#pragma unroll
+        for (int X = 0; X < 2; ++X) {
+            s.app[X] = b + X * (kPPAppStride / 8);
+            s.c2v[X] = b + (2 * kPPAppStride + 8 + X * kPPC2vDist) / 8;
+            s.app_base[X] = lds_addr_of(s.app[X]);
+            s.c2v_base[X] = lds_addr_of(s.c2v[X]);
+        }
+        s.red = reinterpret_cast<int *>(s.c2v[1] + EA);
+        return s;
+    }
     const int SL = pp_slot_words(N, EA);
-    P *b = reinterpret_cast<P *>(smem);
 #pragma unroll
     for (int X = 0; X < 2; ++X) {
         s.app[X] = b + X * SL;
@@ -303,14 +325,16 @@
     }
 }
 
-__device__ __forceinline__ int wave_sum3(int x)
-{
-    return __builtin_popcountll(__builtin_amdgcn_ballot_w64((x & 1) != 0)) +
-           2 * __builtin_popcountll(__builtin_amdgcn_ballot_w64((x & 2) != 0)) +
-           4 * __builtin_popcountll(__builtin_amdgcn_ballot_w64((x & 4) != 0));
-}
-
-template <int C, bool HB, bool WCHK = false>
+template <int NB>
+__device__ __forceinline__ int wave_sum(int x)
+{
+    int t = 0;
+#pragma unroll
+    for (int b = 0; b < NB; ++b) t += (1 << b) * __builtin_popcountll(__builtin_amdgcn_ballot_w64((x & (1 << b)) != 0));
+    return t;
+}
+
+template <int C, bool HB, bool WCHK = false, bool CHU = (LDPC_PP_CHAN_ALL || LDPC_PP_CHAN_SPLIT), int NB = 3>
 __device__ __forceinline__ void pp_account(const DecodeArgs &a, int *red, int grp, int (&sums)[6 * C], unsigned *redo,
                                            unsigned long long *acc)
 {
@@ -320,17 +344,17 @@
 #pragma unroll
         for (int q = 0; q < 2 * C; ++q) {
             if constexpr (HB) {
-                const int w = wave_sum3(sums[3 * q]), u = wave_sum3(sums[3 * q + 1]);
+                const int w = wave_sum<NB>(sums[3 * q]), u = wave_sum<NB>(sums[3 * q + 1]);
                 if (lane0 && w) atomicAdd(&tot[3 * q], w);
                 if (lane0 && u) atomicAdd(&tot[3 * q + 1], u);
             } else {
                 if (__builtin_amdgcn_ballot_w64(sums[3 * q + 2] != 0) && lane0) atomicAdd(&tot[3 * q + 2], 1);
                 if constexpr (WCHK) {
-                    const int w = wave_sum3(sums[3 * q]);
+                    const int w = wave_sum<NB>(sums[3 * q]);
                     if (lane0 && w) atomicAdd(&tot[3 * q], w);
                 }
-                if constexpr (LDPC_PP_CHAN_ALL || LDPC_PP_CHAN_SPLIT) {
-                    const int u = wave_sum3(sums[3 * q + 1]);
+                if constexpr (CHU) {
+                    const int u = wave_sum<NB>(sums[3 * q + 1]);
                     if (lane0 && u) atomicAdd(&tot[3 * q + 1], u);
                 }
             }
@@ -378,7 +402,7 @@
     }
 }
 
-template <typename F, int SRC, int DC0, int DC1, int CPT, int VAR, bool FDIV, int R, bool HB, int IR = 0>
+template <typename F, int SRC, int DC0, int DC1, int CPT, int VAR, bool FDIV, int R, bool HB, int IR = 0, int W = 16>
 __device__ __forceinline__ void pp_role(const DecodeArgs &a, const DevGraph &g, const RowSched &rs,
                                         const PPSlots<Pack<F, PPCw<F>::C>> &s, unsigned *redo,
                                         unsigned long long *acc)
@@ -388,6 +412,14 @@
     constexpr int DCX = 8;
     constexpr int RR = R > 0 ? R : 1;
     static_assert(DC0 <= DCX && DC1 <= DCX && (R == 0) == HB, "pp_role shape");
+    static_assert(W == 16 || W == 12, "pp_role block shape");
+    constexpr bool W12 = W == 12;
+    constexpr int NT = 64 * W, NBT = NT - kPPRole;
+    constexpr int CPL = HB ? CPT * (kPPRole / NBT) : CPT;
+    constexpr bool FIXL = W12;
+    constexpr bool UNP = FIXL && LDPC_PP_W12_UNP && R > 0 && sizeof(F) == 8 && LDPC_PP_EXP == 0;
+    constexpr bool SPLITCH = LDPC_PP_CHAN_SPLIT || W12;
+    static_assert(!UNP || LDPC_PP_PREFETCH, "unpacked addresses: both rows' gathers ahead of row 0");
     static_assert(IR == 0 || R == 2, "in-register bits: two rows per check thread");
     constexpr int L0 = DC0 - 1, L1 = DC1 - 1;
     constexpr bool F64 = sizeof(F) == 8;
@@ -420,6 +452,23 @@
             colw[0][L0 / 2] = (L0 & 1) ? (colw[0][L0 / 2] & 0xffffu) | ((uint32_t)N << 16)
                                        : (colw[0][L0 / 2] & 0xffff0000u) | (uint32_t)N;
     }
+    [[maybe_unused]] uint32_t ga[RR][DCX], sa[RR][DCX], vin = 0;
+    if constexpr (UNP) {
+        static_for<0, R>([&](auto rc) {
+            constexpr int r = decltype(rc)::value, DCr = r == 0 ? DC0 : DC1;
+#pragma unroll
+            for (int k = 0; k < DCr - (IR == 1 ? 1 : 0); ++k) {
+                ga[r][k] = s.app_base[0] + 8u * (uint32_t)LDPC_CHK(u16_at<DCX>(colw[r], k), N + 3, CHK_PP_GATHER);
+                sa[r][k] = s.c2v_base[0] + 8u * (uint32_t)LDPC_CHK(u16_at<DCX>(posw[r], k), EA, CHK_PP_SCATTER);
+                asm("" : "+v"(ga[r][k]), "+v"(sa[r][k]));
+            }
+        });
+        if constexpr (IR != 0) vin = (uint32_t)LDPC_CHK(u16_at<DCX>(colw[0], L0), N + 3, CHK_PP_GATHER);
+    }
+    [[maybe_unused]] auto inreg_col = [&]() -> int {
+        if constexpr (UNP) return (int)vin;
+        else return u16_at<DCX>(colw[0], L0);
+    };
     [[maybe_unused]] auto inreg_sum = [&](auto Xc, const P &y) -> P {
         constexpr int X = decltype(Xc)::value;
         P sum;
@@ -431,23 +480,54 @@
         return sum;
     };
     const int bt = tid - kPPRole;
-    [[maybe_unused]] int vgb[CPT], vgd[CPT];
-    [[maybe_unused]] uint32_t vdst2[(CPT + 1) / 2] = {};
+    static_assert(!UNP || IR != 1 || LDPC_PP_INREG_Y, "unpacked addresses: the in-register bit's sample in registers");
+    [[maybe_unused]] int vgb[CPL], vgd[CPL];
+    [[maybe_unused]] uint32_t vdst2[(CPL + 1) / 2] = {};
+    [[maybe_unused]] uint32_t ra[CPL][LDPC_PP_W12_K0 > LDPC_PP_W12_K1 ? LDPC_PP_W12_K0 : LDPC_PP_W12_K1];
     if constexpr (HB) {
-#pragma unroll
-        for (int i = 0; i < CPT; ++i) {
-            const int c = rs.vn_col[bt * CPT + i];
+        int si[CPL];
+        if constexpr (W12) {
+            int pa = 0, pb = 0;
+#pragma unroll
+            for (int i = 0; i < CPL; ++i) {
+                const int ia = bt * CPT + (pa < CPT ? pa : CPT - 1), ib = (bt + NBT) * CPT + (pb < CPT ? pb : CPT - 1);
+                const int da = pa < CPT ? __builtin_amdgcn_readfirstlane((int)(rs.vn_info[ia] >> 24)) : -1;
+                const int db = pb < CPT ? __builtin_amdgcn_readfirstlane((int)(rs.vn_info[ib] >> 24)) : -1;
+                const bool ta = da >= db;
+                si[i] = ta ? ia : ib;
+                pa += ta ? 1 : 0;
+                pb += ta ? 0 : 1;
+            }
+        } else {
+#pragma unroll
+            for (int i = 0; i < CPL; ++i) si[i] = bt * CPT + i;
+        }
+#pragma unroll
+        for (int i = 0; i < CPL; ++i) {
+            const int c = rs.vn_col[si[i]];
             vdst2[i / 2] |= (uint32_t)(c == 0xffff ? N + 1 : c) << (16 * (i & 1));
-            const uint32_t info = rs.vn_info[bt * CPT + i];
+            const uint32_t info = rs.vn_info[si[i]];
             vgb[i] = __builtin_amdgcn_readfirstlane((int)(info & 0xffffu) - lane);
             vgd[i] = __builtin_amdgcn_readfirstlane((int)(info >> 24));
         }
         P z;
 #pragma unroll
         for (int c = 0; c < C; ++c) z.v[c] = F(0);
-#pragma unroll
-        for (int i = 0; i < CPT; ++i) {
-            const int dg = (int)((rs.vn_info[bt * CPT + i] >> 16) & 0xffu);
+        if constexpr (W12) {
+            if (tid == kPPRole + 2) s.c2v[0][-1] = s.c2v[1][-1] = z;
+            const int ln0 = lane;
+#pragma unroll
+            for (int i = 0; i < CPL; ++i)
+#pragma unroll
+                for (int k = 0; k < (i == 0 ? LDPC_PP_W12_K0 : LDPC_PP_W12_K1); ++k) {
+                    const uint32_t e = (uint32_t)LDPC_CHK(k < vgd[i] ? vgb[i] + ln0 + k * 64 : 0, EA, CHK_PP_BIT_READ);
+                    ra[i][k] = k < vgd[i] ? s.c2v_base[0] + 8u * e : s.c2v_base[0] - 8u;
+                    asm("" : "+v"(ra[i][k]));
+                }
+        }
+#pragma unroll
+        for (int i = 0; i < CPL; ++i) {
+            const int dg = (int)((rs.vn_info[si[i]] >> 16) & 0xffu);
             const int base = vgb[i] + lane, gd = vgd[i];
             for (int k = dg; k < gd; ++k) {
                 const int e = LDPC_CHK(base + k * 64, EA, CHK_PP_BIT_READ);
@@ -483,27 +563,26 @@
         for (int q = 0; q < 2 * C; ++q) unc[q] = wdec[q] = 0;
         [[maybe_unused]] unsigned chan_bad = 0;
         if constexpr (LDPC_PP_CHAN_ALL && !HB) {
-            if (!(LDPC_PP_TAILEXP & 1)) pp_channel<F, SRC>(a, s, N, grp, unc, tid, 2 * kPPRole, &chan_bad);
-        }
-        [[maybe_unused]] const bool split = LDPC_PP_CHAN_SPLIT && SRC == SRC_PHILOX && LDPC_PP_NOB2 &&
+            if (!(LDPC_PP_TAILEXP & 1)) pp_channel<F, SRC>(a, s, N, grp, unc, tid, NT, &chan_bad);
+        }
+        [[maybe_unused]] const bool split = SPLITCH && SRC == SRC_PHILOX && LDPC_PP_NOB2 &&
                                             !(LDPC_PP_TAILEXP & 1) && pp_plain_step(a, N, grp, C);
-        if constexpr (LDPC_PP_CHAN_SPLIT && !HB) {
-            if (split) pp_channel_plain<F>(a, s, N, grp, unc, tid, 2 * kPPRole, &chan_bad);
+        if constexpr (SPLITCH && !HB) {
+            if (split) pp_channel_plain<F>(a, s, N, grp, unc, tid, NT, &chan_bad);
         }
         if constexpr (HB) {
-            if (LDPC_PP_CHAN_SPLIT && split) {
-                pp_channel_plain<F>(a, s, N, grp, unc, tid, 2 * kPPRole, &chan_bad);
+            if (SPLITCH && split) {
+                pp_channel_plain<F>(a, s, N, grp, unc, tid, NT, &chan_bad);
             } else if (!(LDPC_PP_TAILEXP & 1)) {
-                pp_channel<F, SRC>(a, s, N, grp, unc, LDPC_PP_CHAN_ALL ? tid : bt, LDPC_PP_CHAN_ALL ? 2 * kPPRole : kPPRole,
-                                   &chan_bad);
+                pp_channel<F, SRC>(a, s, N, grp, unc, LDPC_PP_CHAN_ALL ? tid : bt, LDPC_PP_CHAN_ALL ? NT : NBT, &chan_bad);
             } else {
                 for (int q = 0; q < 2 * C; ++q) unc[q] = 0;
-                for (int v = bt; v < N; v += kPPRole)
+                for (int v = bt; v < N; v += NBT)
                     for (int c = 0; c < C; ++c) s.app[0][v].v[c] = s.app[1][v].v[c] = F(1);
             }
         }
         PP_SYNC_STAMPED(1);
-        [[maybe_unused]] P yq[2][CPT];
+        [[maybe_unused]] P yq[2][CPL];
         if constexpr (R > 0) {
 #pragma unroll
             for (int X = 0; X < 2; ++X)
@@ -514,7 +593,7 @@
 #pragma unroll
                         for (int c = 0; c < C; ++c) prev[X][r][k].v[c] = F(0);
         }
-        if constexpr ((LDPC_PP_CHAN_SPLIT || (LDPC_PP_CHAN_ALL && LDPC_PP_NOB2)) && !HB) {
+        if constexpr ((SPLITCH || (LDPC_PP_CHAN_ALL && LDPC_PP_NOB2)) && !HB) {
             if (__builtin_amdgcn_ballot_w64(chan_bad != 0)) {
                 if (chan_bad & 1u) s.red[0] = 1;
                 if (chan_bad & 2u) s.red[1] = 1;
@@ -528,14 +607,14 @@
 #pragma unroll
             for (int X = 0; X < 2; ++X)
 #pragma unroll
-                for (int i = 0; i < CPT; ++i)
+                for (int i = 0; i < CPL; ++i)
                     yq[X][i] = s.app[X][LDPC_CHK(vdst(i) < N ? vdst(i) : N + 2, N + 3, CHK_PP_APP_WRITE)];
         } else if constexpr (HB) {
 #pragma unroll
             for (int X = 0; X < 2; ++X) {
                 bool in_ok = true;
 #pragma unroll
-                for (int i = 0; i < CPT; ++i) {
+                for (int i = 0; i < CPL; ++i) {
                     const P st = s.app[X][LDPC_CHK(vdst(i) <= N ? vdst(i) : 0, N + 3, CHK_PP_APP_WRITE)];
 #pragma unroll
                     for (int c = 0; c < C; ++c) {
@@ -544,7 +623,7 @@
                     }
                 }
 #pragma unroll
-                for (int i = 0; i < CPT; ++i) s.app[X][LDPC_CHK(vdst(i), N + 3, CHK_PP_APP_WRITE)] = yq[X][i];
+                for (int i = 0; i < CPL; ++i) s.app[X][LDPC_CHK(vdst(i), N + 3, CHK_PP_APP_WRITE)] = yq[X][i];
                 if (!in_ok) s.red[X] = 1;
             }
             P inf, zero;
@@ -566,7 +645,7 @@
                     const int q = Y * C + c;
                     int e = 0;
 #pragma unroll
-                    for (int i = 0; i < CPT; ++i) e += (vdst(i) < N && !(post[i].v[c] > F(0))) ? 1 : 0;
+                    for (int i = 0; i < CPL; ++i) e += (vdst(i) < N && !(post[i].v[c] > F(0))) ? 1 : 0;
                     w[q] = grp * 2 * C + q < a.batch ? e : 0;
                 }
                 return;
@@ -581,7 +660,7 @@
                                                    : nullptr);
                 int e = 0;
 #pragma unroll
-                for (int i = 0; i < CPT; ++i) {
+                for (int i = 0; i < CPL; ++i) {
                     const int v = vdst(i);
                     if (v < N) {
                         const int d = post[i].v[c] > F(0) ? 1 : -1;
@@ -597,12 +676,12 @@
         [[maybe_unused]] P yreg[2];
         if constexpr (YREG) {
 #pragma unroll
-            for (int X = 0; X < 2; ++X) yreg[X] = s.app[X][LDPC_CHK(u16_at<DCX>(colw[0], L0), N + 3, CHK_PP_GATHER)];
+            for (int X = 0; X < 2; ++X) yreg[X] = s.app[X][LDPC_CHK(inreg_col(), N + 3, CHK_PP_GATHER)];
         }
         [[maybe_unused]] P ipost[2];
         [[maybe_unused]] auto inreg_final = [&](auto Xc) {
             constexpr int X = decltype(Xc)::value;
-            ipost[X] = inreg_sum(Xc, YREG ? yreg[X] : s.app[X][LDPC_CHK(u16_at<DCX>(colw[0], L0), N + 3, CHK_PP_GATHER)]);
+            ipost[X] = inreg_sum(Xc, YREG ? yreg[X] : s.app[X][LDPC_CHK(inreg_col(), N + 3, CHK_PP_GATHER)]);
         };
         auto syndrome = [&](int X, int c) -> int {
             int synd = 0;
@@ -613,7 +692,9 @@
 #pragma unroll
                     for (int k = 0; k < DCr; ++k) {
                         if (IR == 1 && k == DCr - 1) continue;
-                        const int neg = (s.app[X][LDPC_CHK(u16_at<DCX>(colw[r], k), N + 3, CHK_PP_GATHER)].v[c] > F(0)) ? 0 : 1;
+                        int neg;
+                        if constexpr (UNP) neg = (lds_at<P>(ga[r][k] + (X ? kPPAppStride : 0u)).v[c] > F(0)) ? 0 : 1;
+                        else neg = (s.app[X][LDPC_CHK(u16_at<DCX>(colw[r], k), N + 3, CHK_PP_GATHER)].v[c] > F(0)) ? 0 : 1;
                         par ^= (IR == 2 && k == DCr - 1 && has) ? 0 : neg;
                     }
                     if constexpr (IR != 0) par ^= (has && !(ipost[X].v[c] > F(0))) ? 1 : 0;
@@ -628,17 +709,24 @@
             [[maybe_unused]] P xin[RR][DCX];
             if constexpr (R > 0) {
                 if (rows && LDPC_PP_EXP != 2) {
-#pragma unroll
-                    for (int r = 0; r < R; ++r)
-#pragma unroll
-                        for (int q = 0; q < DCX / 2; ++q) asm volatile("" : "+v"(colw[r][q]), "+v"(posw[r][q]));
-                    const uint32_t ab = s.app_base[X];
+                    if constexpr (!UNP) {
+#pragma unroll
+                        for (int r = 0; r < R; ++r)
+#pragma unroll
+                            for (int q = 0; q < DCX / 2; ++q) asm volatile("" : "+v"(colw[r][q]), "+v"(posw[r][q]));
+                    }
+                    [[maybe_unused]] const uint32_t ab = s.app_base[FIXL ? 0 : X];
+                    constexpr uint32_t aoff = FIXL ? X * kPPAppStride : 0u;
                     static_for<0, (LDPC_PP_PREFETCH ? R : 1)>([&](auto rc) {
                         constexpr int r = decltype(rc)::value, DCr = r == 0 ? DC0 : DC1;
 #pragma unroll
-                        for (int k = 0; k < DCr - (IR == 1 && (r == 1 || YREG) ? 1 : 0); ++k)
-                            xin[r][k] = lds_at<P>((LDPC_PP_EXP == 5 || LDPC_PP_EXP == 7) ? ab + 8u * (uint32_t)(lane + 64 * (k + 8 * r))
-                                                                                         : PP_ADDR8(DCX, colw[r], k, ab, N + 3, CHK_PP_GATHER));
+                        for (int k = 0; k < DCr - (IR == 1 && (r == 1 || YREG) ? 1 : 0); ++k) {
+                            if constexpr (UNP)
+                                xin[r][k] = lds_at<P>(ga[r][k] + aoff);
+                            else
+                                xin[r][k] = lds_at<P>(((LDPC_PP_EXP == 5 || LDPC_PP_EXP == 7) ? ab + 8u * (uint32_t)(lane + 64 * (k + 8 * r))
+                                                                                              : PP_ADDR8(DCX, colw[r], k, ab, N + 3, CHK_PP_GATHER)) + aoff);
+                        }
                     });
                     if constexpr (LDPC_PP_GATHER_FIRST && LDPC_PP_PREFETCH) {
                         constexpr int NG = DC0 + (R > 1 ? DC1 : 0);
@@ -651,21 +739,42 @@
                 if (LDPC_PP_BITDELAY > 0) __builtin_amdgcn_s_sleep(LDPC_PP_BITDELAY);
                 if (bits && LDPC_PP_EXP != 1) {
 #pragma unroll
-                    for (int q = 0; q < (CPT + 1) / 2; ++q) asm volatile("" : "+v"(vdst2[q]));
-                    P sum[CPT];
-#pragma unroll
-                    for (int i = 0; i < CPT; ++i) sum[i] = yq[Y][i];
-                    int k = 0;
+                    for (int q = 0; q < (CPL + 1) / 2; ++q) asm volatile("" : "+v"(vdst2[q]));
+                    P sum[CPL];
+#pragma unroll
+                    for (int i = 0; i < CPL; ++i) sum[i] = yq[Y][i];
                     const int ln = (int)__builtin_amdgcn_mbcnt_hi(~0u, __builtin_amdgcn_mbcnt_lo(~0u, 0u));
-                    vn_phases<F, C, CPT, CPT>(s.c2v[Y] + ln, vgb, vgd, k, sum, LDPC_CHK_LIM(EA - ln), CHK_PP_BIT_READ);
-#pragma unroll
-                    for (int i = 0; i < CPT; ++i) s.app[Y][LDPC_CHK(vdst(i), N + 3, CHK_PP_APP_WRITE)] = sum[i];
+                    if constexpr (W12) {
+                        constexpr int K0 = LDPC_PP_W12_K0, K1 = LDPC_PP_W12_K1;
+                        const P *cv = s.c2v[Y] + ln;
+                        [[maybe_unused]] const int lim = LDPC_CHK_LIM(EA - ln);
+                        P rd[CPL][K0 > K1 ? K0 : K1];
+#pragma unroll
+                        for (int i = 0; i < CPL; ++i)
+#pragma unroll
+                            for (int k = 0; k < (i == 0 ? K0 : K1); ++k) rd[i][k] = lds_at<P>(ra[i][k] + Y * kPPC2vDist);
+#pragma unroll
+                        for (int k = 0; k < (K0 > K1 ? K0 : K1); ++k)
+#pragma unroll
+                            for (int i = 0; i < CPL; ++i)
+                                if (k < (i == 0 ? K0 : K1)) padd<false>(sum[i], rd[i][k]);
+#pragma unroll
+                        for (int i = 0; i < CPL; ++i)
+                            for (int k = (i == 0 ? K0 : K1); k < vgd[i]; ++k)
+                                padd<false>(sum[i], cv[LDPC_CHK(vgb[i] + k * 64, lim, CHK_PP_BIT_READ)]);
+                    } else {
+                        int k = 0;
+                        vn_phases<F, C, CPL, CPL>(s.c2v[Y] + ln, vgb, vgd, k, sum, LDPC_CHK_LIM(EA - ln), CHK_PP_BIT_READ);
+                    }
+#pragma unroll
+                    for (int i = 0; i < CPL; ++i) s.app[Y][LDPC_CHK(vdst(i), N + 3, CHK_PP_APP_WRITE)] = sum[i];
                     if (TF && last) decide(Y, sum, wdec);
                 }
             }
             if constexpr (R > 0) {
                 if (rows && LDPC_PP_EXP != 2) {
-                    const uint32_t ab = s.app_base[X], cb = s.c2v_base[X];
+                    [[maybe_unused]] const uint32_t ab = s.app_base[X], cb = s.c2v_base[FIXL ? 0 : X];
+                    constexpr uint32_t coff = FIXL ? X * kPPC2vDist : 0u;
                     if constexpr (IR != 0) {
                         if constexpr (YREG) xin[0][L0] = yreg[X];
                         const P sum = inreg_sum(Xc, xin[0][L0]);
@@ -688,10 +797,12 @@
                         bool ok = true;
                         auto store = [&](int k, const P &m) {
                             if (IR == 1 && k == DCr - 1) return;
-                            if constexpr (LDPC_PP_EXP != 4)
-                                lds_put<P>((LDPC_PP_EXP == 6 || LDPC_PP_EXP == 7)
-                                               ? cb + 8u * (uint32_t)(lane + 64 * ((k + 8 * r + 16 * (tid >> 6)) % 112))
-                                               : PP_ADDR8(DCX, posw[r], k, cb, EA, CHK_PP_SCATTER),
+                            if constexpr (UNP)
+                                lds_put<P>(sa[r][k] + coff, m);
+                            else if constexpr (LDPC_PP_EXP != 4)
+                                lds_put<P>(((LDPC_PP_EXP == 6 || LDPC_PP_EXP == 7)
+                                                ? cb + 8u * (uint32_t)(lane + 64 * ((k + 8 * r + 16 * (tid >> 6)) % 112))
+                                                : PP_ADDR8(DCX, posw[r], k, cb, EA, CHK_PP_SCATTER)) + coff,
                                            m);
                         };
                         if constexpr (LDPC_PP_EXP == 3) {
@@ -761,7 +872,7 @@
 
         if (LDPC_PP_TAILEXP & 2) {
             int sums[6 * C] = {};
-            pp_account<C, HB, IR != 0>(a, s.red, grp, sums, redo, acc);
+            pp_account<C, HB, IR != 0, SPLITCH || LDPC_PP_CHAN_ALL, W12 ? 4 : 3>(a, s.red, grp, sums, redo, acc);
             continue;
         }
         const bool fused = TF && a.T > 0;
@@ -769,9 +880,9 @@
             if (!fused) {
 #pragma unroll
                 for (int X = 0; X < 2; ++X) {
-                    P post[CPT];
-#pragma unroll
-                    for (int i = 0; i < CPT; ++i) post[i] = s.app[X][LDPC_CHK(vdst(i) <= N ? vdst(i) : 0, N + 3, CHK_PP_APP_WRITE)];
+                    P post[CPL];
+#pragma unroll
+                    for (int i = 0; i < CPL; ++i) post[i] = s.app[X][LDPC_CHK(vdst(i) <= N ? vdst(i) : 0, N + 3, CHK_PP_APP_WRITE)];
                     decide(X, post, wdec);
                 }
             }
@@ -779,7 +890,7 @@
         if constexpr (IR != 0) {
             inreg_final(std::integral_constant<int, 0>());
             inreg_final(std::integral_constant<int, 1>());
-            const int v = u16_at<DCX>(colw[0], L0);
+            const int v = inreg_col();
             if (has && v < N) {
 #pragma unroll
                 for (int q = 0; q < 2 * C; ++q) {
@@ -807,7 +918,7 @@
             }
         }
         PP_STAMP_ACC(5);
-        pp_account<C, HB, IR != 0>(a, s.red, grp, sums, redo, acc);
+        pp_account<C, HB, IR != 0, SPLITCH || LDPC_PP_CHAN_ALL, W12 ? 4 : 3>(a, s.red, grp, sums, redo, acc);
     }
     PP_STAMP_OUT()
 }
@@ -820,15 +931,16 @@
 #define LDPC_PP_ENTRY_NOPS 0
 #endif
 
-template <typename F, int SRC, int CPT, int VAR, bool FDIV, bool SPLIT, bool INREG>
+template <typename F, int SRC, int CPT, int VAR, bool FDIV, bool SPLIT, bool INREG, int W = 16>
 __device__ __forceinline__ void pp_kernel(const DecodeArgs &a, const DevGraph &g, const RowSched &rs, unsigned *redo)
 {
     static_assert(!INREG || SPLIT, "in-register bits come with the degree-aware row slots");
+    static_assert(W == 16 || INREG, "the 12-wave block runs the in-register schedule");
     using P = Pack<F, PPCw<F>::C>;
     extern __shared__ __attribute__((aligned(16))) unsigned char smem[];
 #pragma unroll
     for (int i = 0; i < LDPC_PP_ENTRY_NOPS; ++i) asm volatile("s_nop 0");
-    const PPSlots<P> s = pp_slots<P>(smem, g.N, rs.e_pad + 64);
+    const PPSlots<P> s = pp_slots<P, W == 12>(smem, g.N, rs.e_pad + 64);
     unsigned long long *acc = reinterpret_cast<unsigned long long *>(s.red + kPPRedAcc);
     if (threadIdx.x == 0) {
         s.red[0] = s.red[1] = 0;
@@ -850,13 +962,13 @@
     if constexpr (INREG) {
         const bool pure = low && __builtin_amdgcn_readfirstlane((int)rs.pair[kPPRole + (low ? wave : 0)]) != 0;
         if (!low)
-            pp_role<F, SRC, 8, 8, CPT, VAR, FDIV, 0, true>(a, g, rs, s, redo, acc);
+            pp_role<F, SRC, 8, 8, CPT, VAR, FDIV, 0, true, 0, W>(a, g, rs, s, redo, acc);
         else if (wave >= kPPRole / 128) {
-            if (pure) pp_role<F, SRC, 7, 7, CPT, VAR, FDIV, 2, false, 1>(a, g, rs, s, redo, acc);
-            else pp_role<F, SRC, 7, 7, CPT, VAR, FDIV, 2, false, 2>(a, g, rs, s, redo, acc);
+            if (pure) pp_role<F, SRC, 7, 7, CPT, VAR, FDIV, 2, false, 1, W>(a, g, rs, s, redo, acc);
+            else pp_role<F, SRC, 7, 7, CPT, VAR, FDIV, 2, false, 2, W>(a, g, rs, s, redo, acc);
         } else {
-            if (pure) pp_role<F, SRC, 7, 8, CPT, VAR, FDIV, 2, false, 1>(a, g, rs, s, redo, acc);
-            else pp_role<F, SRC, 7, 8, CPT, VAR, FDIV, 2, false, 2>(a, g, rs, s, redo, acc);
+            if (pure) pp_role<F, SRC, 7, 8, CPT, VAR, FDIV, 2, false, 1, W>(a, g, rs, s, redo, acc);
+            else pp_role<F, SRC, 7, 8, CPT, VAR, FDIV, 2, false, 2, W>(a, g, rs, s, redo, acc);
         }
     } else if (!low)
         pp_role<F, SRC, 8, 8, CPT, VAR, FDIV, 0, true>(a, g, rs, s, redo, acc);
@@ -885,6 +997,12 @@
     pp_kernel<F, SRC, CPT, VAR, FDIV, true, true>(a, g, rs, redo);
 }
 
+template <typename F, int SRC, int CPT, int VAR, bool FDIV>
+__global__ __launch_bounds__(kPPRole + kPPRole / 2) void k_rows_ppw(DecodeArgs a, DevGraph g, RowSched rs, unsigned *redo)
+{
+    pp_kernel<F, SRC, CPT, VAR, FDIV, true, true, 12>(a, g, rs, redo);
+}
+
 static int rows_pp_lds_bytes(const DevGraph &g, const RowSched &rs)
 {
     return (int)(2 * (size_t)pp_slot_words(g.N, rs.e_pad + 64) * 8 + kPPRedInts * sizeof(int));
@@ -896,21 +1014,43 @@
            g.N <= 4 * kPPRole && g.N + 3 <= 0xffff && rows_pp_lds_bytes(g, rs) <= 160 * 1024;
 }
 
+static size_t rows_ppw_lds_bytes(const RowSched &rs)
+{
+    return 2 * (size_t)kPPAppStride + 8 + kPPC2vDist + (size_t)(rs.e_pad + 64) * 8 + kPPRedInts * sizeof(int);
+}
+
+bool pp_w12_layout(int N, int e_pad, int *lds_bytes)
+{
+    RowSched rs{};
+    rs.e_pad = e_pad;
+    const size_t bytes = rows_ppw_lds_bytes(rs);
+    if (lds_bytes) *lds_bytes = (int)std::min<size_t>(bytes, 0x7fffffff);
+    return N >= 0 && e_pad >= 0 && ((size_t)N + 3) * 8 <= kPPAppStride && ((size_t)e_pad + 64) * 8 <= kPPC2vStride &&
+           bytes <= kMaxLds;
+}
+
+static bool rows_ppw_supported(const DevGraph &g, const RowSched &rs)
+{
+    return rs.cpt == 3 && pp_w12_layout(g.N, rs.e_pad, nullptr);
+}
+
 template <typename F, int SRC, int VAR, bool FDIV>
-static const void *pp_fn_t(const RowSched &rs)
-{
-    if constexpr (sizeof(F) == 8)
+static const void *pp_fn_t(const RowSched &rs, bool w12)
+{
+    if constexpr (sizeof(F) == 8) {
+        if (rs.pair && w12) return (const void *)k_rows_ppw<F, SRC, 3, VAR, FDIV>;
         if (rs.pair)
             return rs.cpt == 3 ? (const void *)k_rows_ppi<F, SRC, 3, VAR, FDIV> : (const void *)k_rows_ppi<F, SRC, 4, VAR, FDIV>;
+    }
     return rs.dc_low == 7 ? (const void *)k_rows_pp<F, SRC, 4, VAR, FDIV, true>
                           : (const void *)k_rows_pp<F, SRC, 4, VAR, FDIV, false>;
 }
 
-static const void *pp_fn(const RowSched &rs, const DecodeArgs &a, bool f64)
+static const void *pp_fn(const RowSched &rs, const DecodeArgs &a, bool f64, bool w12)
 {
     const bool given = a.src == SRC_GIVEN;
 #define LDPC_PP_SRC(FT, VARV, FD) \
-    return given ? pp_fn_t<FT, SRC_GIVEN, VARV, FD>(rs) : pp_fn_t<FT, SRC_PHILOX, VARV, FD>(rs);
+    return given ? pp_fn_t<FT, SRC_GIVEN, VARV, FD>(rs, w12) : pp_fn_t<FT, SRC_PHILOX, VARV, FD>(rs, w12);
     if (!f64) {
         if (a.variant == V_MS) { LDPC_PP_SRC(float, V_MS, false) }
         if (a.variant == V_NMS && a.nms_fast) { LDPC_PP_SRC(float, V_NMS, false) }
@@ -925,10 +1065,11 @@
 
 bool plan_rows_pp(const PlanInput &in, LaunchPlan &p)
 {
-    const RowSched *rs = in.rs_pp && opt(LDPC_OPT_PP_SLOTS) != 1 ? in.rs_pp : in.rs;
+    const int slots = opt(LDPC_OPT_PP_SLOTS);
+    const RowSched *rs = in.rs_pp && slots != 1 ? in.rs_pp : in.rs;
     if (!rows_pp_supported(in.g, *rs)) return false;
     const RowSched *ri = nullptr;
-    if (in.f64 && LDPC_PP_NOB2 && LDPC_PP_PREFETCH && rs == in.rs_pp && in.rs_ppi && opt(LDPC_OPT_PP_SLOTS) == 0 &&
+    if (in.f64 && LDPC_PP_NOB2 && LDPC_PP_PREFETCH && rs == in.rs_pp && in.rs_ppi && (slots == 0 || slots == 3) &&
         rs->dc_low == 7 && in.rs_ppi->pair && in.rs_ppi->e_pad == rs->e_pad && rows_pp_supported(in.g, *in.rs_ppi))
         ri = in.rs_ppi;
     p.kernel = Kernel::rows_pp;
@@ -936,9 +1077,11 @@
     p.redo = true;
     p.rs = rs;
     p.rs_inreg = ri;
-    p.fn = pp_fn(ri ? *ri : *rs, in.a, in.f64);
-    p.threads = 2 * kPPRole;
+    const bool w12 = ri && slots == 0 && rows_ppw_supported(in.g, *ri);
+    p.fn = pp_fn(ri ? *ri : *rs, in.a, in.f64, w12);
+    p.threads = w12 ? kPPRole + kPPRole / 2 : 2 * kPPRole;
     p.lds_bytes = rows_pp_lds_bytes(in.g, *rs);
+    p.pad_lds_bytes = w12 ? (int)rows_ppw_lds_bytes(*ri) - p.lds_bytes : 0;
     p.blocks_per_cu = 1;
     const int CW = 2 * (in.f64 ? PPCw<double>::C : PPCw<float>::C);
     p.grid = std::min(in.num_cus, (in.a.batch + CW - 1) / CW);
diff --git a/ldpcsimulation_amd/native.py b/ldpcsimulation_amd/native.py
--- a/ldpcsimulation_amd/native.py
+++ b/ldpcsimulation_amd/native.py
@@ -22,7 +22,8 @@
            "ems_swizzle": 21, "ddbmp_kernel": 22}
 EMS_OPTIONS = ("ems_threads", "ems_swizzle")
 OPTION_VALUES = {"rows64": {"pp": 0, "fast": 1, "rows": 2}, "rows32": {"pp": 0, "fast": 1, "rows": 2},
-                 "pp_slots": {"split": 0, "plain": 1, "split_lds": 2}, "kernel": {"auto": 0, "lds": 1, "flood": 2, "global": 3},
+                 "pp_slots": {"split": 0, "plain": 1, "split_lds": 2, "split_w16": 3},
+                 "kernel": {"auto": 0, "lds": 1, "flood": 2, "global": 3},
                  "flood_mode": {"phase": 0, "persistent": 1}, "flood_msg": {"packed": 0, "c2v": 1},
                  "bp_kernel": {"rows": 0, "generic": 1}, "gdbf_kernel": {"rows": 0, "generic": 1},
                  "ddbmp_kernel": {"rows": 0, "generic": 1},
@@ -351,6 +352,8 @@
     "ldpc_ctx_pp_row_slots": ([_vp, _vp, _vp, _vp, C.c_int, C.POINTER(C.c_int)], _i32),
     "ldpc_ctx_row_sched_info": ([_vp, C.POINTER(_Cfg), _vp], _i32),
     "ldpc_ctx_pp_inreg_info": ([_vp, C.POINTER(_Cfg), _vp], _i32),
+    "ldpc_ctx_pp_block_info": ([_vp, C.POINTER(_Cfg), _vp], _i32),
+    "ldpc_pp_block_layout": ([_i32, _i32, _vp], _i32),
     "ldpc_ctx_set_option": ([_vp, _i32, _i32], _i32),
     "ldpc_ctx_get_option": ([_vp, _i32, _pi32], _i32),
     "ldpc_nb_ctx_set_option": ([_vp, _i32, _i32], _i32),
@@ -405,9 +408,9 @@
 _lib = None
 
 
-_ADDED_IN_ABI = {"ldpc_ctx_pp_inreg_info", "ldpc_ctx_redo_list", "ldpc_ctx_pp_row_slots", "ldpc_fxms_decode_batch",
-                 "ldpc_fxms_sim_launch", "ldpc_fxms_sim_batch", "ldpc_fxms_sim_trace", "ldpc_fxms_kernel_info",
-                 "ldpc_fxlms_decode_batch", "ldpc_fxlms_sim_launch", "ldpc_fxlms_sim_batch", "ldpc_fxlms_sim_trace",
+_ADDED_IN_ABI = {"ldpc_ctx_pp_inreg_info", "ldpc_ctx_pp_block_info", "ldpc_pp_block_layout", "ldpc_ctx_redo_list",
+                 "ldpc_ctx_pp_row_slots", "ldpc_fxms_decode_batch", "ldpc_fxms_sim_launch", "ldpc_fxms_sim_batch",
+                 "ldpc_fxms_sim_trace", "ldpc_fxms_kernel_info", "ldpc_fxlms_decode_batch", "ldpc_fxlms_sim_launch", "ldpc_fxlms_sim_batch", "ldpc_fxlms_sim_trace",
                  "ldpc_fxlms_kernel_info"}
 
 
@@ -437,6 +440,12 @@
 def _check(rc: int):
     if rc != LDPC_OK:
         raise LdpcError(rc, lib().ldpc_last_error().decode(errors="replace"))
+
+
+def pp_block_layout(n_bits: int, e_pad: int) -> dict:
+    info = np.zeros(2, dtype=np.int32)
+    _check(lib().ldpc_pp_block_layout(int(n_bits), int(e_pad), info.ctypes.data))
+    return {"fits": bool(info[0]), "launch_lds_bytes": int(info[1])}
 
 
 def device_count() -> int:
@@ -659,6 +668,11 @@
         keys = ("inreg_bits", "lds_check_edges", "bit_slot_edges", "slots_per_thread")
         return {k: int(v) for k, v in zip(keys, info)}
 
+    def pp_block_info(self, cfg: DecoderConfig) -> dict:
+        info = np.zeros(2, dtype=np.int32)
+        _check(lib().ldpc_ctx_pp_block_info(self._h, C.byref(cfg._c()), info.ctypes.data))
+        return {"threads": int(info[0]), "launch_lds_bytes": int(info[1])}
+
     def pp_row_slots(self, cfg: DecoderConfig):
         cols = np.zeros((2048, 8), dtype=np.uint16)
         deg = np.zeros(2048, dtype=np.uint8)
```
